# neeharperi/FutureDet

Hardware: AMD Instinct MI355X
Metric: sweeps/sec end-to-end (300k pts, 10-sweep voxel) (higher is better)
Workload: dtype f32

## Files before the change

### futuredet_amd/backbones.py

```python
import numpy as np
import torch
from torch import nn

from . import hip_ops, sparse as spconv
from .nn_utils import build_norm_layer
from .registry import BACKBONES
from .sparse import SparseConv3d, SubMConv3d


def conv3x3(in_planes, out_planes, stride=1, indice_key=None, bias=True):
    return spconv.SubMConv3d(in_planes, out_planes, kernel_size=3, stride=stride, padding=1, bias=bias,
                             indice_key=indice_key)


class SparseBasicBlock(spconv.SparseModule):
    expansion = 1

    def __init__(self, inplanes, planes, stride=1, norm_cfg=None, downsample=None, indice_key=None):
        super().__init__()
        if norm_cfg is None:
            norm_cfg = dict(type="BN1d", eps=1e-3, momentum=0.01)
        bias = norm_cfg is not None
        self.conv1 = conv3x3(inplanes, planes, stride, indice_key=indice_key, bias=bias)
        self.bn1 = build_norm_layer(norm_cfg, planes)[1]
        self.relu = nn.ReLU()
        self.conv2 = conv3x3(planes, planes, indice_key=indice_key, bias=bias)
        self.bn2 = build_norm_layer(norm_cfg, planes)[1]
        self.downsample = downsample
        self.stride = stride

    def forward(self, x):
        identity = x
        out = self.conv1(x)
        out.features = self.relu(self.bn1(out.features))
        out = self.conv2(out)
        out.features = self.bn2(out.features)
        if self.downsample is not None:
            identity = self.downsample(x)
        out.features = self.relu(out.features + identity.features)
        return out

    def forward_fused_bn(self, x, bn_act):
        out = self.conv1(x)
        out.features = bn_act(out.features, self.bn1, self.relu)
        out = self.conv2(out)
        identity = x if self.downsample is None else self.downsample(x)
        out.features = bn_act(out.features, self.bn2, self.relu, identity.features)
        return out


@BACKBONES.register_module
class SpMiddleResNetFHD(nn.Module):
    def __init__(self, num_input_features=128, norm_cfg=None, name="SpMiddleResNetFHD", **kwargs):
        super().__init__()
        self.name = name
        if norm_cfg is None:
            norm_cfg = dict(type="BN1d", eps=1e-3, momentum=0.01)
        S = spconv.SparseSequential
        self.conv_input = S(SubMConv3d(num_input_features, 16, 3, bias=False, indice_key="res0"),
                            build_norm_layer(norm_cfg, 16)[1], nn.ReLU(inplace=True))
        self.conv1 = S(SparseBasicBlock(16, 16, norm_cfg=norm_cfg, indice_key="res0"),
                       SparseBasicBlock(16, 16, norm_cfg=norm_cfg, indice_key="res0"))
        self.conv2 = S(SparseConv3d(16, 32, 3, 2, padding=1, bias=False), build_norm_layer(norm_cfg, 32)[1],
                       nn.ReLU(inplace=True), SparseBasicBlock(32, 32, norm_cfg=norm_cfg, indice_key="res1"),
                       SparseBasicBlock(32, 32, norm_cfg=norm_cfg, indice_key="res1"))
        self.conv3 = S(SparseConv3d(32, 64, 3, 2, padding=1, bias=False), build_norm_layer(norm_cfg, 64)[1],
                       nn.ReLU(inplace=True), SparseBasicBlock(64, 64, norm_cfg=norm_cfg, indice_key="res2"),
                       SparseBasicBlock(64, 64, norm_cfg=norm_cfg, indice_key="res2"))
        self.conv4 = S(SparseConv3d(64, 128, 3, 2, padding=[0, 1, 1], bias=False), build_norm_layer(norm_cfg, 128)[1],
                       nn.ReLU(inplace=True), SparseBasicBlock(128, 128, norm_cfg=norm_cfg, indice_key="res3"),
                       SparseBasicBlock(128, 128, norm_cfg=norm_cfg, indice_key="res3"))
        self.extra_conv = S(SparseConv3d(128, 128, (3, 1, 1), (2, 1, 1), bias=False), build_norm_layer(norm_cfg, 128)[1],
                            nn.ReLU())
        self.compute_dtype = torch.float32
        self.dense_channels_last = True
        self.dense_dtype = None
        self.profile_hook = None
        self.fused_bn = False
        self.train_dtype = torch.float32

    def _bn_act(self, features, bn, relu, residual=None):
        if self.fused_bn and spconv.batch_norm_fusable(features, bn):
            return spconv.batch_norm_act(features, bn, residual=residual, relu=True)
        if features.dtype == torch.bfloat16:
            out = bn(features.float())
            if residual is not None:
                out = out + residual.float()
            return spconv.relu_to_bf16(out)
        out = bn(features)
        if residual is not None:
            out = out + residual
        return relu(out)

    def _run_stage(self, seq, x):
        mods = list(seq._modules.values())
        i = 0
        while i < len(mods):
            m = mods[i]
            if isinstance(m, SparseBasicBlock):
                x = m.forward_fused_bn(x, self._bn_act)
            elif isinstance(m, spconv.SparseModule):
                x = m(x)
            elif x.features.shape[0] != 0:
                if isinstance(m, nn.BatchNorm1d) and i + 1 < len(mods) and isinstance(mods[i + 1], nn.ReLU):
                    x.features = self._bn_act(x.features, m, mods[i + 1])
                    i += 1
                else:
                    x.features = m(x.features)
            i += 1
        return x

    def forward_generic(self, voxel_features, coors, batch_size, input_shape):
        sparse_shape = np.array(input_shape[::-1]) + [1, 0, 0]
        ret = spconv.SparseConvTensor(voxel_features, coors.int(), sparse_shape, batch_size)
        stages = (self.conv_input, self.conv1, self.conv2, self.conv3, self.conv4, self.extra_conv)
        mixed = self.train_dtype == torch.bfloat16 and self.training and torch.is_grad_enabled()
        if mixed:
            ret.features = ret.features.to(torch.bfloat16)
        if mixed or (self.fused_bn and self.training and torch.is_grad_enabled()):
            run = [lambda x, seq=seq: self._run_stage(seq, x) for seq in stages]
        else:
            run = stages
        x = run[0](ret)
        x_conv1 = run[1](x)
        x_conv2 = run[2](x_conv1)
        x_conv3 = run[3](x_conv2)
        x_conv4 = run[4](x_conv3)
        ret = run[5](x_conv4).dense()
        if mixed:
            ret = ret.float()
        N, C, D, H, W = ret.shape
        ret = ret.view(N, C * D, H, W)
        return ret, {"conv1": x_conv1, "conv2": x_conv2, "conv3": x_conv3, "conv4": x_conv4}

    def _stages(self):
        return [(self.conv_input[0], self.conv_input[1], [self.conv1[0], self.conv1[1]], True),
                (self.conv2[0], self.conv2[1], [self.conv2[3], self.conv2[4]], False),
                (self.conv3[0], self.conv3[1], [self.conv3[3], self.conv3[4]], False),
                (self.conv4[0], self.conv4[1], [self.conv4[3], self.conv4[4]], False),
                (self.extra_conv[0], self.extra_conv[1], [], False)]

    def build_indexes(self, mark_fn, batch_size, input_shape, device, voxels=None, static=False, expected=None, row_caps=None):
        D, H, W = [int(v) for v in (np.array(input_shape[::-1]) + [1, 0, 0])]
        if voxels is not None:
            geoms = [self._stages()[lvl][0].geometry() for lvl in range(1, 5)]
            return hip_ops.build_pyramid(voxels[0], voxels[1], voxels[2], batch_size, (D, H, W), geoms, device, static=static,
                                         expected=expected, row_caps=row_caps)
        assert not static, "static indexes are built from the voxelizer's device output (voxels=...)"
        counts = torch.zeros((5,), dtype=torch.int32, device=device)
        idx = [hip_ops.SparseIndex(batch_size, D, H, W, device)]
        mark_fn(idx[0])
        idx[0].scan(counts[0:1])
        for lvl in range(1, 5):
            conv = self._stages()[lvl][0]
            ks, st, pd = conv.geometry()
            nxt = idx[-1].downsample(ks, st, pd)
            nxt.scan(counts[lvl:lvl + 1])
            idx.append(nxt)
        host = counts.cpu()
        for i, ix in enumerate(idx):
            ix.finalize(int(host[i]))
        return idx

    def run_fused(self, idx, feats0, dense_out=None, fork=False):
        dt = self.compute_dtype
        stages = self._stages()
        rb_cache = {}

        from_index = dt == torch.float32

        def rulebook(src, dst, conv):
            ks, st, pd = conv.geometry()
            key = (id(src), id(dst), tuple(ks), tuple(st), tuple(pd))
            if key not in rb_cache:
                layer = (spconv.pad_channels(conv.in_channels), spconv.pad_channels(conv.out_channels)) if from_index else None
                rb_cache[key] = src.rulebook(dst, ks, st, pd, fp32_layer=layer)
            return rb_cache[key]

        def run(conv, bn, x, src, dst, relu, residual=None):
            wpk, bias, cin_p, cout_p = conv.packed_weight(dt, bn)
            assert x.shape[1] == cin_p, (x.shape, cin_p)
            nbr = rulebook(src, dst, conv)
            fn = lambda: hip_ops.spconv_apply(x, wpk, bias, nbr, dst.n, cout_p, residual=residual, relu=relu)
            if self.profile_hook is not None:
                s = 4 if dt == torch.float32 else 2
                K = nbr.shape[0]
                table = lambda: nbr.table() if isinstance(nbr, hip_ops.IndexRulebook) else nbr
                pairs = lambda: int((table()[:, : dst.n] >= 0).sum().item())
                return self.profile_hook("spconv_%dx%d_K%d" % (cin_p, cout_p, K),
                                         dict(s=s, K=K, cin=cin_p, cout=cout_p, n_in=src.n, n_out=dst.n, pairs=pairs), fn)
            return fn()

        def index_plans():
            groups = ([], [])
            for lvl, (conv, bn, blocks, is_subm_in) in enumerate(stages):
                if lvl == 0:
                    continue
                src_l, dst_l = (idx[lvl] if is_subm_in else idx[lvl - 1]), idx[lvl]
                for s_l, cv in [(src_l, conv)] + [(dst_l, b.conv1) for b in blocks[:1]]:
                    nbr = rulebook(s_l, dst_l, cv)
                    if isinstance(nbr, hip_ops.IndexRulebook):
                        ci, co = spconv.pad_channels(cv.in_channels), spconv.pad_channels(cv.out_channels)
                        groups[int(ci == co and bool(hip_ops._lib.load().fd_spconv_wants_balanced_ranges(ci, co, 0)))].append((nbr, ci, co))
            made = []
            for group in groups:
                splits = [(rb,) + tuple(hip_ops.row_split(rb, rb.n_out, ci, co)) for rb, ci, co in group]
                made += [r for _, r, _ in splits if r is not None]
                made += hip_ops.plans_from_index(splits)
            return made

        main, side = None, None
        if fork and feats0.is_cuda:
            main = torch.cuda.current_stream(feats0.device)
            pool = self.__dict__.setdefault("_side_streams", {})
            side = pool.get(main.cuda_stream)
            if side is None:
                side = pool[main.cuda_stream] = torch.cuda.Stream(device=feats0.device)
            side.wait_stream(main)
            with torch.cuda.stream(side):
                made = []
                for lvl, (conv, bn, blocks, is_subm_in) in enumerate(stages):
                    if lvl == 0:
                        continue
                    src_l, dst_l = (idx[lvl] if is_subm_in else idx[lvl - 1]), idx[lvl]
                    nbr = rulebook(src_l, dst_l, conv)
                    if not isinstance(nbr, hip_ops.IndexRulebook):
                        made.append(nbr)
                    for blk in blocks:
                        nbr = rulebook(dst_l, dst_l, blk.conv1)
                        if isinstance(nbr, hip_ops.IndexRulebook):
                            continue
                        made.append(nbr)
                        cp = spconv.pad_channels(blk.conv1.out_channels)
                        if dt == torch.float32 and nbr.shape[0] == 27 and \
                                hip_ops._lib.load().fd_spconv_wants_balanced_ranges(cp, cp, 0):
                            r = hip_ops.ranges_for(nbr, cp, cp)
                            if r[0] is not None:
                                made.append(r[0])
                        if dt == torch.float32 and nbr.shape[0] == 27 and dst_l.n > 0 and \
                                hip_ops._lib.load().fd_spconv_plan_wanted(cp, cp, 0):
                            made.append(hip_ops.plan_for(nbr, dst_l.n, *hip_ops.row_split(nbr, dst_l.n, cp, cp))[0])
                made += index_plans()
                for t in made:
                    t.record_stream(main)
        elif from_index:
            index_plans()
        x = feats0
        levels = {}
        for lvl, (conv, bn, blocks, is_subm_in) in enumerate(stages):
            src = idx[lvl] if is_subm_in else idx[lvl - 1]
            dst = idx[lvl]
            if lvl == 1 and side is not None:
                main.wait_stream(side)
            x = run(conv, bn, x, src, dst, relu=True)
            for blk in blocks:
                y = run(blk.conv1, blk.bn1, x, dst, dst, relu=True)
                x = run(blk.conv2, blk.bn2, y, dst, dst, relu=True, residual=x)
            levels[lvl] = (x, dst)
        bev = hip_ops.densify(x, idx[4], out_dtype=self.dense_dtype or dt, channels_last=self.dense_channels_last, out=dense_out)
        return bev, levels

    def forward_static_train(self, feats0, idx):
        if not self.fused_bn:
            raise ValueError("SpMiddleResNetFHD.forward_static_train needs fused_bn = True: torch's BatchNorm1d cannot take its row count "
                             "from the device (set backbone.fused_bn = True)")
        if not (self.training and torch.is_grad_enabled()):
            raise RuntimeError("SpMiddleResNetFHD.forward_static_train is the training path: call .train() and enable gradients")
        if self.train_dtype not in (torch.float32, torch.bfloat16):
            raise ValueError("SpMiddleResNetFHD: train_dtype must be torch.float32 or torch.bfloat16 (got %s)" % (self.train_dtype,))
        B = idx[0].B
        feats = feats0.to(self.train_dtype)
        rulebooks = {}

        def conv(m, x, src, dst):
            ks, st, pd = m.geometry()
            key = (id(src), id(dst), tuple(ks), tuple(st), tuple(pd))
            if key not in rulebooks:
                rulebooks[key] = src.rulebook(dst, ks, st, pd)
            return m._forward_autograd(x, dst, rulebooks[key])

        def bn_act(x, bn, dst, residual=None):
            if dst.n < 2 or not spconv.batch_norm_fusable(x.features, bn):
                raise hip_ops.FutureDetHipError("forward_static_train: BatchNorm over %s %s rows cannot run on the fused kernels"
                                                % (tuple(x.features.shape), x.features.dtype))
            x.features = spconv.batch_norm_act(x.features, bn, residual=residual, relu=True, n_dev=dst.n_dev if dst.static else None)
            return x

        x = spconv.SparseConvTensor(feats, None, idx[0].spatial_shape, B, _index=idx[0])
        for lvl, (head, bn, blocks, is_subm_in) in enumerate(self._stages()):
            src, dst = (idx[lvl] if is_subm_in else idx[lvl - 1]), idx[lvl]
            x = bn_act(conv(head, x, src, dst), bn, dst)
            for blk in blocks:
                y = bn_act(conv(blk.conv1, x, dst, dst), blk.bn1, dst)
                x = bn_act(conv(blk.conv2, y, dst, dst), blk.bn2, dst, residual=x.features)
        ret = x.dense()
        if ret.dtype != torch.float32:
            ret = ret.float()
        N, C, D, H, W = ret.shape
        return ret.view(N, C * D, H, W)

    def forward(self, voxel_features, coors, batch_size, input_shape):
        if self.training:
            if self.train_dtype not in (torch.float32, torch.bfloat16):
                raise ValueError("SpMiddleResNetFHD: train_dtype must be torch.float32 or torch.bfloat16 (got %s)" % (self.train_dtype,))
            if self.train_dtype == torch.float32 and self.compute_dtype != torch.float32 and torch.is_grad_enabled():
                raise NotImplementedError("SpMiddleResNetFHD: with train_dtype = torch.float32 training runs the fp32 sparse convolution only; "
                                          "compute_dtype = %s selects the inference path (set train_dtype = torch.bfloat16 for mixed-precision "
                                          "training, or compute_dtype = torch.float32)" % self.compute_dtype)
            return self.forward_generic(voxel_features, coors, batch_size, input_shape)
        coors = coors.int().contiguous()
        dev = voxel_features.device
        idx = self.build_indexes(lambda i0: i0.mark(coors), batch_size, input_shape, dev)
        row_of = idx[0].lookup(coors)
        feats0 = hip_ops.rows_permute(voxel_features.float().contiguous(), row_of,
                                      spconv.pad_channels(voxel_features.shape[1]), self.compute_dtype, n_rows=idx[0].n)
        bev, levels = self.run_fused(idx, feats0)
        multi = {}
        for name, lvl, c in (("conv1", 0, 16), ("conv2", 1, 32), ("conv3", 2, 64), ("conv4", 3, 128)):
            f, ix = levels[lvl]
            multi[name] = spconv.SparseConvTensor(f[:, :c], None, ix.spatial_shape, batch_size, _index=ix)
        return bev, multi


@BACKBONES.register_module
class PointPillarsScatter(nn.Module):

    def __init__(self, num_input_features=64, norm_cfg=None, name="PointPillarsScatter", **kwargs):
        super().__init__()
        self.name = "PointPillarsScatter"
        self.nchannels = num_input_features
        self.dense_channels_last = True

    def forward(self, voxel_features, coords, batch_size, input_shape, n_dev=None):
        self.nx = int(input_shape[0])
        self.ny = int(input_shape[1])
        coords = coords.int().contiguous()
        if n_dev is None and torch.is_grad_enabled() and voxel_features.requires_grad:
            return _ScatterFn.apply(voxel_features, coords, batch_size, self.ny, self.nx, self.dense_channels_last)
        return hip_ops.pillar_scatter(voxel_features, coords, n_dev, batch_size, self.ny, self.nx,
                                      channels_last=self.dense_channels_last)


    def forward_static(self, voxel_features, coords, counts, batch_size, input_shape):
        self.nx = int(input_shape[0])
        self.ny = int(input_shape[1])
        return _ScatterSegFn.apply(voxel_features, coords.int().contiguous(), counts, batch_size, self.ny, self.nx, self.dense_channels_last)


class _ScatterSegFn(torch.autograd.Function):

    @staticmethod
    def forward(ctx, feats, coords, counts, batch_size, ny, nx, channels_last):
        B = counts.shape[0]
        cap = feats.shape[0] // B
        ctx.coords, ctx.counts, ctx.cap = coords, counts, cap
        canvas = None
        for b in range(B):
            sl = slice(b * cap, (b + 1) * cap)
            canvas = hip_ops.pillar_scatter(feats[sl], coords[sl], counts[b:b + 1], batch_size, ny, nx, channels_last=channels_last,
                                            out=canvas, zero_first=(b == 0))
        return canvas

    @staticmethod
    def backward(ctx, dcanvas):
        coords, counts, cap = ctx.coords, ctx.counts, ctx.cap
        dcanvas = dcanvas.float()
        d = torch.cat([hip_ops.pillar_scatter_backward(dcanvas, coords[b * cap:(b + 1) * cap], n_dev=counts[b:b + 1])
                       for b in range(counts.shape[0])])
        ctx.coords = ctx.counts = None
        return d, None, None, None, None, None, None


class _ScatterFn(torch.autograd.Function):

    @staticmethod
    def forward(ctx, feats, coords, batch_size, ny, nx, channels_last):
        ctx.coords = coords
        return hip_ops.pillar_scatter(feats, coords, None, batch_size, ny, nx, channels_last=channels_last)

    @staticmethod
    def backward(ctx, dcanvas):
        d = hip_ops.pillar_scatter_backward(dcanvas.float(), ctx.coords)
        ctx.coords = None
        return d, None, None, None, None, None
```

### futuredet_amd/csrc/fd_common.h

```cpp
#pragma once
#include <hip/hip_runtime.h>
#include <stdint.h>
#include <stdio.h>

#include <atomic>

#include "../../include/futuredet_hip.h"

namespace fd {

void set_error(const char *fmt, ...);

struct SpconvCall {
    const void *in;
    int64_t n_in;
    const void *wpacked;
    const float *bias;
    const void *residual;
    int relu;
    const int *nbr;
    int64_t nbr_stride;
    const int *ranges;
    int n_ranges;
    int K, n_out;
    const int *n_out_dev;
    int64_t n_expected;
    int cin, cout, dtype;
    void *out;
    hipStream_t stream;
    const int *plan;
    int64_t plan_stride;
};

constexpr int kSpconvMaxTaps = 27;

struct WeightSection {
    size_t offset, bytes;
};
struct SpconvWeightLayout {
    WeightSection base, c32, pair, win;
    size_t total;
};
inline SpconvWeightLayout spconv_weight_layout(int K, int cin, int cout, int dtype) {
    const size_t elem = dtype == 0 ? 4 : 2, main_bytes = (size_t)K * cin * cout * elem;
    SpconvWeightLayout l{};
    size_t end = 0;
    auto section = [&](bool present, size_t bytes) {
        const WeightSection s{end, present ? bytes : 0};
        end += s.bytes;
        return s;
    };
    l.base = section(true, main_bytes);
    l.c32 = section(dtype == 0 && cin == 32 && cout == 32, main_bytes);
    l.pair = section(dtype == 1 && cin == 16, (size_t)((K + 1) / 2) * 32 * cout * elem);
    l.win = section(dtype == 1 && ((cin == 64 && cout == 64) || (cin == 128 && cout == 128)), main_bytes);
    l.total = end;
    return l;
}
inline SpconvWeightLayout spconv_weight_layout(const SpconvCall &c) { return spconv_weight_layout(c.K, c.cin, c.cout, c.dtype); }

int spconv_f32_res16_dispatch(const SpconvCall &c);
int spconv_f32_c32_dispatch(const SpconvCall &c);
int spconv_f32_compact_dispatch(const SpconvCall &c);
int spconv_bf16_win_dispatch(const SpconvCall &c);
int spconv_bf16_ws_dispatch(const SpconvCall &c);

int wino_pc_launch(const float *x, const void *wp, const float *bias, float *y, int B, int H, int W, int cin, int cout, int relu, int cout_total,
                   int co_off, int wide_items, hipStream_t stream);

__device__ __forceinline__ int device_count(int capacity, const int *count_dev) {
    if (!count_dev) return capacity;
    const int n = *count_dev;
    return n < capacity ? (n > 0 ? n : 0) : capacity;
}

inline int check_launch(const char *what) {
    hipError_t e = hipGetLastError();
    if (e != hipSuccess) {
        set_error("%s: %s", what, hipGetErrorString(e));
        return FD_ELAUNCH;
    }
    return FD_OK;
}

#define FD_REQUIRE(cond, ...)           \
    do {                                \
        if (!(cond)) {                  \
            fd::set_error(__VA_ARGS__); \
            return FD_EINVAL;           \
        }                               \
    } while (0)

inline hipStream_t as_stream(fd_stream_t s) { return reinterpret_cast<hipStream_t>(s); }

int fill_words(void *p, uint32_t value, size_t n_words, hipStream_t stream);
int fill_words3(void *p0, uint32_t v0, size_t n0, void *p1, uint32_t v1, size_t n1, void *p2, uint32_t v2, size_t n2, hipStream_t stream);

constexpr int kMaxDevices = 64;
int current_device();
int device_cu_count();
bool ensure_dynamic_lds(const void *kernel, size_t bytes, std::atomic<uint64_t> &done);
#define FD_TUNE_KNOBS(X)                                                                                                       \
    X(kTuneSpconvRG, "spconv_rg") X(kTuneSpconvV1, "spconv_v1") X(kTuneConvNT, "conv_nt") X(kTuneV2RangesPerCU, "v2_ranges_per_cu") \
    X(kTuneSpconvC32, "spconv_c32") X(kTuneBf16GP, "bf16_gp") X(kTuneBf16RG, "bf16_rg") X(kTuneBf16Depth, "bf16_depth")        \
    X(kTuneBf16NW, "bf16_nw") X(kTuneBf16Win, "bf16_win") X(kTuneF32ResRG, "f32_res_rg") X(kTuneConvStrip, "conv_strip")       \
    X(kTuneF32ResNW, "f32_res_nw") X(kTuneSpconvPlan, "spconv_plan")
#define FD_TUNE_ENUM(key, name) key,
enum TuneKey { FD_TUNE_KNOBS(FD_TUNE_ENUM) kTuneCount };
#undef FD_TUNE_ENUM
int tuning(TuneKey key);

inline size_t align_up(size_t v, size_t a) { return (v + a - 1) / a * a; }

struct IndexGeom {
    int B, D, H, W, Ht, Wt;
    __host__ __device__ int64_t num_cols() const { return (int64_t)B * Ht * Wt * 64; }
};
__host__ __device__ inline IndexGeom make_geom(int B, int D, int H, int W) {
    IndexGeom g;
    g.B = B; g.D = D; g.H = H; g.W = W;
    g.Ht = (H + 7) >> 3; g.Wt = (W + 7) >> 3;
    return g;
}
__host__ __device__ inline int64_t col_of(const IndexGeom &g, int b, int y, int x) {
    return ((((int64_t)b * g.Ht + (y >> 3)) * g.Wt + (x >> 3)) << 6) + ((y & 7) << 3) + (x & 7);
}
__device__ inline void col_to_byx(const IndexGeom &g, int64_t col, int &b, int &y, int &x) {
    int in = (int)(col & 63);
    int64_t t = col >> 6;
    int tx = (int)(t % g.Wt);
    t /= g.Wt;
    int ty = (int)(t % g.Ht);
    b = (int)(t / g.Ht);
    y = ty * 8 + (in >> 3);
    x = tx * 8 + (in & 7);
}

__device__ inline unsigned xcd_swizzle(unsigned bid, unsigned nblocks) {
    const unsigned nx = 8;
    unsigned per = nblocks / nx, rem = nblocks % nx;
    unsigned xcd = bid % nx, loc = bid / nx;
    unsigned start = xcd * per + (xcd < rem ? xcd : rem);
    return start + loc;
}

}
```

### futuredet_amd/csrc/fd_spconv.hip

```cpp
#include "fd_spconv_pack.h"

namespace {

typedef float f32x4 __attribute__((ext_vector_type(4)));
typedef short s16x4 __attribute__((ext_vector_type(4)));
typedef __bf16 bf16x8 __attribute__((ext_vector_type(8)));

__device__ inline unsigned short f2bf(float v) {
    unsigned u = __float_as_uint(v);
    u += 0x7fffu + ((u >> 16) & 1u);
    return (unsigned short)(u >> 16);
}
__device__ inline float bf2f(unsigned short h) { return __uint_as_float(((unsigned)h) << 16); }


template <int CIN, int COUT, int RG>
__global__ void __launch_bounds__(256) spconv_f32(const float *__restrict__ in, const float4 *__restrict__ wp,
                                                  const float *__restrict__ bias, const float *__restrict__ residual, int relu,
                                                  const int *__restrict__ nbr, int64_t nbr_stride, int K, int n_out,
                                                  const int *__restrict__ n_out_dev, float *__restrict__ out) {
    constexpr int ROWS_B = 64 * RG;
    constexpr int NB = COUT / 16, NC = CIN / 16;
    __shared__ int s_nbr[fd::kSpconvMaxTaps * ROWS_B];
    const int tile = blockIdx.x;
    const int row0 = tile * ROWS_B;
    n_out = fd::device_count(n_out, n_out_dev);
    if (row0 >= n_out) return;
    for (int t = threadIdx.x; t < K * ROWS_B; t += 256) {
        int k = t / ROWS_B, r = t - k * ROWS_B;
        int64_t o = (int64_t)row0 + r;
        s_nbr[t] = (o < n_out) ? nbr[(int64_t)k * nbr_stride + o] : -1;
    }
    __syncthreads();
    const int lane = threadIdx.x & 63, wave = __builtin_amdgcn_readfirstlane(threadIdx.x >> 6);
    const int lrow = lane & 15, lq = lane >> 4;
    const int wrow = wave * 16 * RG;
    if (row0 + wrow >= n_out) return;

    f32x4 acc[RG][NB];
#pragma unroll
    for (int g = 0; g < RG; ++g)
#pragma unroll
        for (int nb = 0; nb < NB; ++nb) acc[g][nb] = (f32x4){0.f, 0.f, 0.f, 0.f};

    for (int k = 0; k < K; ++k) {
        int idx[RG];
        bool any[RG];
        bool any_all = false;
#pragma unroll
        for (int g = 0; g < RG; ++g) {
            idx[g] = s_nbr[k * ROWS_B + wrow + g * 16 + lrow];
            any[g] = __ballot(idx[g] >= 0) != 0ull;
            any_all = any_all || any[g];
        }
        if (!any_all) continue;
        const float4 *wk = wp + (int64_t)k * NC * NB * 64 + lane;
#pragma unroll
        for (int c = 0; c < NC; ++c) {
            float4 a[RG];
#pragma unroll
            for (int g = 0; g < RG; ++g) {
                a[g] = make_float4(0.f, 0.f, 0.f, 0.f);
                if (idx[g] >= 0) a[g] = *reinterpret_cast<const float4 *>(in + (int64_t)idx[g] * CIN + c * 16 + lq * 4);
            }
#pragma unroll
            for (int nb = 0; nb < NB; ++nb) {
                const float4 b = wk[(c * NB + nb) * 64];
#pragma unroll
                for (int g = 0; g < RG; ++g) {
                    if (any[g]) {
                        acc[g][nb] = __builtin_amdgcn_mfma_f32_16x16x4f32(a[g].x, b.x, acc[g][nb], 0, 0, 0);
                        acc[g][nb] = __builtin_amdgcn_mfma_f32_16x16x4f32(a[g].y, b.y, acc[g][nb], 0, 0, 0);
                        acc[g][nb] = __builtin_amdgcn_mfma_f32_16x16x4f32(a[g].z, b.z, acc[g][nb], 0, 0, 0);
                        acc[g][nb] = __builtin_amdgcn_mfma_f32_16x16x4f32(a[g].w, b.w, acc[g][nb], 0, 0, 0);
                    }
                }
            }
        }
    }
#pragma unroll
    for (int g = 0; g < RG; ++g) {
#pragma unroll
        for (int nb = 0; nb < NB; ++nb) {
            const int col = nb * 16 + lrow;
            const float bv = bias ? bias[col] : 0.0f;
#pragma unroll
            for (int r = 0; r < 4; ++r) {
                const int row = row0 + wrow + g * 16 + lq * 4 + r;
                if (row < n_out) {
                    float v = acc[g][nb][r] + bv;
                    if (residual) v += residual[(int64_t)row * COUT + col];
                    if (relu) v = fmaxf(v, 0.0f);
                    out[(int64_t)row * COUT + col] = v;
                }
            }
        }
    }
}

template <int CIN, int COUT, int RG>
__global__ void __launch_bounds__(256) spconv_bf16(const unsigned short *__restrict__ in, const void *__restrict__ wp_,
                                                   const float *__restrict__ bias, const unsigned short *__restrict__ residual,
                                                   int relu, const int *__restrict__ nbr, int64_t nbr_stride, int K, int n_out,
                                                   const int *__restrict__ n_out_dev, unsigned short *__restrict__ out) {
    constexpr int ROWS_B = 64 * RG;
    constexpr int NB = COUT / 16;
    constexpr bool WIDE = CIN >= 32;
    constexpr int NC = WIDE ? CIN / 32 : 1;
    __shared__ int s_nbr[fd::kSpconvMaxTaps * ROWS_B];
    const int tile = blockIdx.x;
    const int row0 = tile * ROWS_B;
    n_out = fd::device_count(n_out, n_out_dev);
    if (row0 >= n_out) return;
    for (int t = threadIdx.x; t < K * ROWS_B; t += 256) {
        int k = t / ROWS_B, r = t - k * ROWS_B;
        int64_t o = (int64_t)row0 + r;
        s_nbr[t] = (o < n_out) ? nbr[(int64_t)k * nbr_stride + o] : -1;
    }
    __syncthreads();
    const int lane = threadIdx.x & 63, wave = __builtin_amdgcn_readfirstlane(threadIdx.x >> 6);
    const int lrow = lane & 15, lq = lane >> 4;
    const int wrow = wave * 16 * RG;
    if (row0 + wrow >= n_out) return;

    f32x4 acc[RG][NB];
#pragma unroll
    for (int g = 0; g < RG; ++g)
#pragma unroll
        for (int nb = 0; nb < NB; ++nb) acc[g][nb] = (f32x4){0.f, 0.f, 0.f, 0.f};

    for (int k = 0; k < K; ++k) {
        int idx[RG];
        bool any[RG];
        bool any_all = false;
#pragma unroll
        for (int g = 0; g < RG; ++g) {
            idx[g] = s_nbr[k * ROWS_B + wrow + g * 16 + lrow];
            any[g] = __ballot(idx[g] >= 0) != 0ull;
            any_all = any_all || any[g];
        }
        if (!any_all) continue;
        if constexpr (WIDE) {
            const bf16x8 *wk = reinterpret_cast<const bf16x8 *>(wp_) + (int64_t)k * NC * NB * 64 + lane;
#pragma unroll
            for (int c = 0; c < NC; ++c) {
                bf16x8 a[RG];
#pragma unroll
                for (int g = 0; g < RG; ++g) {
                    uint4 raw = make_uint4(0u, 0u, 0u, 0u);
                    if (idx[g] >= 0) raw = *reinterpret_cast<const uint4 *>(in + (int64_t)idx[g] * CIN + c * 32 + lq * 8);
                    a[g] = __builtin_bit_cast(bf16x8, raw);
                }
#pragma unroll
                for (int nb = 0; nb < NB; ++nb) {
                    const bf16x8 b = wk[(c * NB + nb) * 64];
#pragma unroll
                    for (int g = 0; g < RG; ++g)
                        if (any[g]) acc[g][nb] = __builtin_amdgcn_mfma_f32_16x16x32_bf16(a[g], b, acc[g][nb], 0, 0, 0);
                }
            }
        } else {
            const s16x4 *wk = reinterpret_cast<const s16x4 *>(wp_) + (int64_t)k * NB * 64 + lane;
            s16x4 a[RG];
#pragma unroll
            for (int g = 0; g < RG; ++g) {
                uint2 raw = make_uint2(0u, 0u);
                if (idx[g] >= 0) raw = *reinterpret_cast<const uint2 *>(in + (int64_t)idx[g] * CIN + lq * 4);
                a[g] = __builtin_bit_cast(s16x4, raw);
            }
#pragma unroll
            for (int nb = 0; nb < NB; ++nb) {
                const s16x4 b = wk[nb * 64];
#pragma unroll
                for (int g = 0; g < RG; ++g)
                    if (any[g]) acc[g][nb] = __builtin_amdgcn_mfma_f32_16x16x16bf16_1k(a[g], b, acc[g][nb], 0, 0, 0);
            }
        }
    }
#pragma unroll
    for (int g = 0; g < RG; ++g) {
#pragma unroll
        for (int nb = 0; nb < NB; ++nb) {
            const int col = nb * 16 + lrow;
            const float bv = bias ? bias[col] : 0.0f;
#pragma unroll
            for (int r = 0; r < 4; ++r) {
                const int row = row0 + wrow + g * 16 + lq * 4 + r;
                if (row < n_out) {
                    float v = acc[g][nb][r] + bv;
                    if (residual) v += bf2f(residual[(int64_t)row * COUT + col]);
                    if (relu) v = fmaxf(v, 0.0f);
                    out[(int64_t)row * COUT + col] = f2bf(v);
                }
            }
        }
    }
}

template <int CIN, int COUT, int RG>
void launch(const fd::SpconvCall &a) {
    const int rows_b = 64 * RG;
    dim3 grid((unsigned)((a.n_out + rows_b - 1) / rows_b));
    const void *wp = (const char *)a.wpacked + fd::spconv_weight_layout(a).base.offset;
    if (a.dtype == 0)
        hipLaunchKernelGGL((spconv_f32<CIN, COUT, RG>), grid, dim3(256), 0, a.stream, (const float *)a.in, (const float4 *)wp, a.bias,
                           (const float *)a.residual, a.relu, a.nbr, a.nbr_stride, a.K, a.n_out, a.n_out_dev, (float *)a.out);
    else
        hipLaunchKernelGGL((spconv_bf16<CIN, COUT, RG>), grid, dim3(256), 0, a.stream, (const unsigned short *)a.in, wp, a.bias,
                           (const unsigned short *)a.residual, a.relu, a.nbr, a.nbr_stride, a.K, a.n_out, a.n_out_dev, (unsigned short *)a.out);
}

template <int CIN, int COUT>
void launch_rg(const fd::SpconvCall &a, int rg) {
    if (rg >= 4) launch<CIN, COUT, 4>(a);
    else if (rg == 2) launch<CIN, COUT, 2>(a);
    else launch<CIN, COUT, 1>(a);
}

int pick_rg(int64_t n_out, int cin, int cout) {
    const int forced = fd::tuning(fd::kTuneSpconvRG);
    if (forced > 0) return forced;
    const int64_t waves2 = (n_out + 31) / 32;
    int rg = (cin * cout >= 128 * 128) ? 1 : 2;
    if (rg == 2 && waves2 < 256 * 4 * 2) rg = 1;
    return rg;
}

}

extern "C" size_t fd_spconv_packed_weight_bytes(int K, int cin, int cout, int dtype) {
    if (K <= 0 || cin <= 0 || cout <= 0) return 0;
    return fd::spconv_weight_layout(K, cin, cout, dtype).total;
}

extern "C" int fd_spconv_pack_weight(const float *w, int K, int cin, int cout, int dtype, void *dst) {
    if (const int rc = fd::spconv_pack_check("fd_spconv_pack_weight", w, dst, K, cin, cout, dtype, 0)) return rc;
    fd::spconv_pack_weight_host(w, K, cin, cout, dtype, dst);
    return FD_OK;
}

namespace {
int spconv_apply(const void *in_feats, int64_t n_in, const void *wpacked, const float *bias, const void *residual, int relu, const int32_t *nbr,
                 int64_t nbr_stride, const int32_t *ranges, int n_ranges, int K, int64_t n_out, const int32_t *n_out_dev, int64_t n_expected, int cin,
                 int cout, int dtype, void *out_feats, fd_stream_t stream, const int32_t *plan, int64_t plan_stride) {
    FD_REQUIRE(K >= 1 && K <= fd::kSpconvMaxTaps, "fd_spconv_apply: K must be in [1,27]");
    FD_REQUIRE(dtype == 0 || dtype == 1, "fd_spconv_apply: dtype must be 0 (f32) or 1 (bf16)");
    FD_REQUIRE(n_out >= 0 && n_out <= nbr_stride && n_out < (1ll << 31), "fd_spconv_apply: n_out out of range");
    FD_REQUIRE(n_ranges >= 0 && (ranges == nullptr || n_ranges >= 1), "fd_spconv_apply: ranges needs n_ranges >= 1");
    if (n_expected <= 0 || n_expected > n_out) n_expected = n_out;
    if (n_out == 0) return FD_OK;
    FD_REQUIRE(in_feats && wpacked && (nbr || plan) && out_feats, "fd_spconv_apply: null argument");
    const fd::SpconvCall c{in_feats, n_in, wpacked, bias, residual, relu, nbr, nbr_stride, ranges, n_ranges, K, (int)n_out, n_out_dev, n_expected,
                           cin, cout, dtype, out_feats, fd::as_stream(stream), plan, plan_stride};
    if (dtype == 0 && !fd::tuning(fd::kTuneSpconvV1) && cin == 16 && fd::tuning(fd::kTuneF32ResRG) >= 0) {
        if (fd::spconv_f32_res16_dispatch(c)) return fd::check_launch("fd_spconv_apply(f32 resident)");
    }
    if (dtype == 0 && !fd::tuning(fd::kTuneSpconvV1) && fd::tuning(fd::kTuneSpconvC32) >= 0) {
        if (fd::spconv_f32_c32_dispatch(c)) return fd::check_launch("fd_spconv_apply(c32)");
    }
    if (dtype == 0 && !fd::tuning(fd::kTuneSpconvV1)) {
        if (fd::spconv_f32_compact_dispatch(c)) return fd::check_launch("fd_spconv_apply(compact)");
    }
    if (dtype == 1 && fd::tuning(fd::kTuneBf16GP) >= 0) {
        const bool subm_like = K == 27 && n_in == n_out;
        if (fd::tuning(fd::kTuneBf16Win) >= 0 && subm_like && fd::spconv_bf16_win_dispatch(c)) return fd::check_launch("fd_spconv_apply(bf16 window)");
        if (fd::spconv_bf16_ws_dispatch(c)) return fd::check_launch("fd_spconv_apply(bf16 ws)");
    }
    if (!nbr) {
        fd::set_error("fd_spconv_apply_plan: no kernel runs %d -> %d on %lld input rows from a chunk plan alone: pass the rulebook table", cin, cout,
                      (long long)n_in);
        return FD_EINVAL;
    }
    const int rg = pick_rg(n_expected, cin, cout);
    const int key = cin * 1000 + cout;
    switch (key) {
        case 16016: launch_rg<16, 16>(c, rg); break;
        case 16032: launch_rg<16, 32>(c, rg); break;
        case 32032: launch_rg<32, 32>(c, rg); break;
        case 32064: launch_rg<32, 64>(c, rg); break;
        case 64064: launch_rg<64, 64>(c, rg); break;
        case 64128: launch_rg<64, 128>(c, rg); break;
        case 128128: launch_rg<128, 128>(c, rg); break;
        default:
            fd::set_error("fd_spconv_apply: unsupported channels %d -> %d", cin, cout);
            return FD_EINVAL;
    }
    return fd::check_launch("fd_spconv_apply");
}
}

extern "C" int fd_spconv_apply(const void *in_feats, int64_t n_in, const void *wpacked, const float *bias, const void *residual, int relu,
                               const int32_t *nbr, int64_t nbr_stride, const int32_t *ranges, int n_ranges, int K, int64_t n_out,
                               const int32_t *n_out_dev, int64_t n_expected, int cin, int cout, int dtype, void *out_feats, fd_stream_t stream) {
    return spconv_apply(in_feats, n_in, wpacked, bias, residual, relu, nbr, nbr_stride, ranges, n_ranges, K, n_out, n_out_dev, n_expected, cin, cout,
                        dtype, out_feats, stream, nullptr, 0);
}

extern "C" int fd_spconv_apply_plan(const void *in_feats, int64_t n_in, const void *wpacked, const float *bias, const void *residual, int relu,
                                    const int32_t *nbr, int64_t nbr_stride, const int32_t *ranges, int n_ranges, int K, int64_t n_out,
                                    const int32_t *n_out_dev, int64_t n_expected, int cin, int cout, int dtype, void *out_feats,
                                    const int32_t *plan, int64_t plan_stride, fd_stream_t stream) {
    FD_REQUIRE(nbr || plan, "fd_spconv_apply_plan: nbr == NULL needs a chunk plan (fd_spconv_plan_from_index)");
    if (plan) {
        FD_REQUIRE(K == fd::kSpconvMaxTaps && dtype == 0, "fd_spconv_apply_plan: a chunk plan belongs to an fp32 layer of K = 27 taps");
        FD_REQUIRE(nbr == nullptr || cin == cout, "fd_spconv_apply_plan: next to a rulebook table a chunk plan belongs to an fp32 SubM layer (K = 27)");
        FD_REQUIRE(plan_stride >= fd_spconv_plan_stride(n_out), "fd_spconv_apply_plan: plan_stride below fd_spconv_plan_stride(n_out)");
        if (!nbr) {
            FD_REQUIRE(fd_spconv_index_plan_wanted(cin, cout, dtype),
                       "fd_spconv_apply_plan: nbr == NULL, but no kernel runs this layer shape from a chunk plan alone (fd_spconv_index_plan_wanted)");
        } else if (!fd_spconv_plan_wanted(cin, cout, dtype)) {
            plan = nullptr;
        }
    }
    return spconv_apply(in_feats, n_in, wpacked, bias, residual, relu, nbr, nbr_stride, ranges, n_ranges, K, n_out, n_out_dev, n_expected, cin, cout,
                        dtype, out_feats, stream, plan, plan_stride);
}
```

### futuredet_amd/csrc/fd_spconv_c32.hip

```cpp
#include "fd_spconv_chunk.h"

namespace {

namespace sk = fd::skeleton;
typedef float f32x16 __attribute__((ext_vector_type(16)));
typedef unsigned u32x4 __attribute__((ext_vector_type(4)));
constexpr int TM = 128, COUT = 32, TS = 4, WR = 1;
constexpr sk::Layout L = sk::layout(TM, COUT, TS, 32);
static_assert(((sk::kMaxTaps + TS - 1) / TS) * (TM / WR / 32) <= L.item_slot, "item list slot");

template <int CIN, int DEPTH, bool PLAN>
__global__ void __launch_bounds__(256) spconv_f32_c32(const float *__restrict__ in, const float4 *__restrict__ wp, const float *__restrict__ bias,
                                                      const float *__restrict__ residual, int relu, const int *__restrict__ nbr, int64_t nbr_stride,
                                                      int K, int n_out, const int *__restrict__ n_out_dev, float *__restrict__ out, unsigned in_bytes,
                                                      const int *__restrict__ ranges, int rows_per_range) {
    constexpr int NCH = CIN / 8;
    constexpr int kPad = sk::pad_entry(TM);
    extern __shared__ __attribute__((aligned(16))) unsigned char smem[];
    int *s_list = reinterpret_cast<int *>(smem + L.list);
    unsigned short *s_items = reinterpret_cast<unsigned short *>(smem + L.items);
    unsigned char *s_cnt = smem + L.cnt;
    int *s_pad = reinterpret_cast<int *>(smem + L.pad);
    float *s_acc = reinterpret_cast<float *>(smem + L.acc);

    const int tid = threadIdx.x, lane = tid & 63, wave = __builtin_amdgcn_readfirstlane(tid >> 6);
    int r_begin, r_end, n_chunks, chunk_rows;
    sk::resolve_range(n_out, n_out_dev, ranges, rows_per_range, r_begin, r_end);
    if (r_begin >= r_end) return;
    sk::cut_chunks<TM>(r_begin, r_end, n_chunks, chunk_rows);
    int pre[sk::kSliceRegs<TM>];
    const int k_fetch = PLAN ? sk::kPlanRows : K;
    sk::fetch_slice<TM>(pre, nbr, nbr_stride, k_fetch, r_begin);

    const int ln = lane & 31, lh = lane >> 5;
    const int ts = wave, wr = 0;
    unsigned char *acc_bytes = reinterpret_cast<unsigned char *>(s_acc + ts * L.acc_copy);
    const __amdgpu_buffer_rsrc_t rsrc = __builtin_amdgcn_make_buffer_rsrc(const_cast<float *>(in), 0, (int)in_bytes, 0x00020000);
    unsigned short *items = s_items + wave * L.item_slot;

    for (int chunk = 0; chunk < n_chunks; ++chunk) {
        int row0, n_rows;
        if (!sk::chunk_span(r_begin, r_end, chunk_rows, chunk, row0, n_rows)) break;
        if constexpr (PLAN) {
            sk::stage_plan_chunk<TM, COUT, TS, 32>(pre, s_list, s_cnt, s_pad, s_acc, bias, residual, row0, n_rows);
        } else {
            sk::stage_chunk<TM, COUT, TS, 32>(pre, s_list, s_pad, s_acc, bias, residual, K, row0, n_rows);
            __syncthreads();
            sk::compact_taps<TM, WR>(s_list, s_cnt, K);
        }
        __syncthreads();
        if (chunk + 1 < n_chunks) sk::fetch_slice<TM>(pre, nbr, nbr_stride, k_fetch, row0 + chunk_rows);
        const int n_items = sk::build_items<TS, 32>(s_cnt, items, K, ts, wr);

        int k_r[DEPTH], row_r[DEPTH];
        u32x4 a_r[DEPTH][NCH];
        auto stage_a0 = [&](int it) -> int { return sk::stage_a0(items, n_items, it); };
        auto stage_a1 = [&](int it, int code_v, int &kk, int &e) { sk::stage_a1<TM, WR, 32>(s_list, s_pad, n_items, wr, ln, it, code_v, kk, e); };
        auto gather_offset = [&](int e) -> unsigned { return sk::entry_row_bytes<CIN>(e) + (unsigned)(lh * 16); };
        auto gather_step = [&](unsigned voff, int c) { return __builtin_amdgcn_raw_buffer_load_b128(rsrc, voff + c * 32, 0, 0); };
        float4 b[NCH];
        auto load_b = [&](int k) {
            const float4 *wk = wp + (int64_t)k * NCH * 64 + lane;
#pragma unroll
            for (int c = 0; c < NCH; ++c) b[c] = wk[c * 64];
        };
        int k_s, e_s, code_s;
#pragma unroll
        for (int d = 0; d < DEPTH - 1; ++d) {
            stage_a1(d, stage_a0(d), k_s, e_s);
            const unsigned vo = gather_offset(e_s);
#pragma unroll
            for (int c = 0; c < NCH; ++c) a_r[d][c] = gather_step(vo, c);
            k_r[d] = k_s;
            row_r[d] = e_s;
        }
        k_r[DEPTH - 1] = -1;
        row_r[DEPTH - 1] = kPad;
        stage_a1(DEPTH - 1, stage_a0(DEPTH - 1), k_s, e_s);
        code_s = stage_a0(DEPTH);
        if (n_items > 0) load_b(k_r[0]);

        for (int i0 = 0; i0 < n_items; i0 += DEPTH) {
#pragma unroll
            for (int d = 0; d < DEPTH; ++d) {
                const unsigned arow = sk::entry_local_row(row_r[d]);
                unsigned aoff[4];
#pragma unroll
                for (int q = 0; q < 4; ++q) aoff[q] = sk::acc_slot_bytes<COUT>(arow, (unsigned)(2 * q + lh));
                f32x16 acc;
#pragma unroll
                for (int q = 0; q < 4; ++q) {
                    const float4 v = *reinterpret_cast<const float4 *>(acc_bytes + aoff[q]);
                    acc[4 * q + 0] = v.x; acc[4 * q + 1] = v.y; acc[4 * q + 2] = v.z; acc[4 * q + 3] = v.w;
                }
                const int dn = (d + DEPTH - 1) % DEPTH;
                {
                    const int it = i0 + d + DEPTH - 1;
                    const unsigned vo = gather_offset(e_s);
                    k_r[dn] = k_s;
                    row_r[dn] = e_s;
#pragma unroll
                    for (int c = 0; c < NCH; ++c) a_r[dn][c] = gather_step(vo, c);
                    stage_a1(it + 1, code_s, k_s, e_s);
                    code_s = stage_a0(it + 2);
                }
                const int knext = k_r[(d + 1) % DEPTH];
                const bool reload = knext >= 0 && knext != k_r[d];
                __builtin_amdgcn_sched_barrier(0);
#pragma unroll
                for (int c = 0; c < NCH; ++c) {
                    const float4 av = __builtin_bit_cast(float4, a_r[d][c]);
                    acc = __builtin_amdgcn_mfma_f32_32x32x2f32(b[c].x, av.x, acc, 0, 0, 0);
                    acc = __builtin_amdgcn_mfma_f32_32x32x2f32(b[c].y, av.y, acc, 0, 0, 0);
                    acc = __builtin_amdgcn_mfma_f32_32x32x2f32(b[c].z, av.z, acc, 0, 0, 0);
                    acc = __builtin_amdgcn_mfma_f32_32x32x2f32(b[c].w, av.w, acc, 0, 0, 0);
                    if (reload) b[c] = (wp + (int64_t)knext * NCH * 64 + lane)[c * 64];
                }
#pragma unroll
                for (int q = 0; q < 4; ++q)
                    *reinterpret_cast<float4 *>(acc_bytes + aoff[q]) = make_float4(acc[4 * q + 0], acc[4 * q + 1], acc[4 * q + 2], acc[4 * q + 3]);
                __builtin_amdgcn_sched_barrier(0);
            }
        }
        __syncthreads();
        sk::epilogue<TM, COUT, TS>(s_acc, bias, residual, relu, out, row0, n_rows);
        __syncthreads();
    }
}

template <int CIN, int DEPTH, bool PLAN>
int launch_c32(const fd::SpconvCall &c) {
    const unsigned in_bytes = (unsigned)(c.n_in * CIN * 4);
    int n_ranges = c.n_ranges, rows_per = 0;
    if (!c.ranges) sk::equal_rows_split(c.n_out, TM, c.n_out_dev != nullptr, n_ranges, rows_per);
    static std::atomic<uint64_t> lds_set{0};
    if (!fd::ensure_dynamic_lds(reinterpret_cast<const void *>(spconv_f32_c32<CIN, DEPTH, PLAN>), (size_t)L.bytes, lds_set)) return 0;
    const void *wp = (const char *)c.wpacked + fd::spconv_weight_layout(c).c32.offset;
    hipLaunchKernelGGL((spconv_f32_c32<CIN, DEPTH, PLAN>), dim3((unsigned)n_ranges), dim3(256), (size_t)L.bytes, c.stream, (const float *)c.in, (const float4 *)wp,
                       c.bias, (const float *)c.residual, c.relu, PLAN ? c.plan : c.nbr, PLAN ? c.plan_stride : c.nbr_stride, c.K, c.n_out, c.n_out_dev, (float *)c.out, in_bytes, c.ranges, rows_per);
    return 1;
}

}

namespace fd {
int spconv_f32_c32_dispatch(const SpconvCall &c) {
    if (c.cout != 32 || c.cin != 32) return 0;
    if (!sk::entries_fit(c.n_in, c.cin)) return 0;
    return c.plan ? launch_c32<32, 3, true>(c) : launch_c32<32, 3, false>(c);
}
}
```

### futuredet_amd/csrc/fd_spconv_chunk.h

```cpp
#pragma once
#include "fd_common.h"

namespace fd {
namespace skeleton {

constexpr int kMaxTaps = 27;

constexpr int pad_entry(int tm) { return (int)(0xffffff00u | (unsigned)tm); }
__device__ __forceinline__ int pack_entry(int in_row, int local_row) { return (in_row << 8) | local_row; }
__device__ __forceinline__ unsigned entry_local_row(int e) { return (unsigned)e & 255u; }
template <int CIN>
__device__ __forceinline__ unsigned entry_row_bytes(int e) {
    static_assert(CIN == 16 || CIN == 32 || CIN == 64 || CIN == 128, "shift per CIN");
    const unsigned hi = (unsigned)e & 0xffffff00u;
    return CIN >= 64 ? hi << (CIN == 128 ? 1 : 0) : hi >> (CIN == 32 ? 1 : 2);
}
inline bool entries_fit(int64_t n_in_bound, int cin) { return n_in_bound < (1ll << 23) && n_in_bound * cin * 4 < (1ll << 31); }

struct Layout {
    int list;
    int items;
    int item_slot;
    int cnt;
    int pad;
    int acc;
    int acc_copy;
    int bytes;
};
constexpr int acc_copy_floats(int tm, int cout) { return (tm + 1) * cout; }
constexpr Layout layout(int tm, int cout, int ts, int item) {
    Layout l{};
    l.list = 0;
    l.items = l.list + (int)sizeof(int) * kMaxTaps * tm;
    l.item_slot = item == 16 ? kMaxTaps * (tm / 16) : 32;
    l.cnt = l.items + (int)sizeof(unsigned short) * 4 * l.item_slot;
    l.pad = l.cnt + 112;
    l.acc = l.pad + (int)sizeof(int) * item;
    l.acc_copy = acc_copy_floats(tm, cout);
    l.bytes = l.acc + (int)sizeof(float) * ts * l.acc_copy;
    return l;
}

template <int COUT>
__device__ __forceinline__ unsigned acc_swizzle(unsigned row) {
    static_assert(COUT == 16 || COUT == 32 || COUT == 64 || COUT == 128, "whole bank rows");
    constexpr int kSwzShift = COUT >= 64 ? 0 : COUT == 32 ? 1 : 2;
    constexpr unsigned kSwzMask = COUT >= 64 ? 15u : COUT == 32 ? 7u : 3u;
    return (row >> kSwzShift) & kSwzMask;
}
template <int COUT>
__device__ __forceinline__ int acc_slot(int row, int col) {
    return row * (COUT / 4) + (col ^ (int)acc_swizzle<COUT>((unsigned)row));
}
template <int COUT>
__device__ __forceinline__ unsigned acc_slot_bytes(unsigned row, unsigned col) {
    return row * (COUT * 4) + ((col ^ acc_swizzle<COUT>(row)) << 4);
}

__device__ __forceinline__ void resolve_range_of(int block, int n_blocks, int n_out, const int *n_out_dev, const int *ranges, int rows_per_range,
                                                 int &r_begin, int &r_end) {
    if (n_out_dev) n_out = fd::device_count(n_out, n_out_dev);
    if (ranges) {
        r_begin = ranges[block];
        r_end = ranges[block + 1];
    } else {
        if (n_out_dev) rows_per_range = (((n_out + n_blocks - 1) / n_blocks) + 15) & ~15;
        const int64_t b = (int64_t)block * rows_per_range;
        r_begin = (int)(b < n_out ? b : n_out);
        r_end = (int)(b + rows_per_range < n_out ? b + rows_per_range : n_out);
    }
    if (r_end > n_out) r_end = n_out;
}
__device__ __forceinline__ void resolve_range(int n_out, const int *n_out_dev, const int *ranges, int rows_per_range,
                                              int &r_begin, int &r_end) {
    resolve_range_of((int)blockIdx.x, (int)gridDim.x, n_out, n_out_dev, ranges, rows_per_range, r_begin, r_end);
}
template <int TM>
__device__ __forceinline__ void cut_chunks(int r_begin, int r_end, int &n_chunks, int &chunk_rows) {
    n_chunks = (r_end - r_begin + TM - 1) / TM;
    chunk_rows = (((r_end - r_begin + n_chunks - 1) / n_chunks) + 15) & ~15;
}
__device__ __forceinline__ bool chunk_span(int r_begin, int r_end, int chunk_rows, int chunk, int &row0, int &n_rows) {
    row0 = r_begin + chunk * chunk_rows;
    n_rows = (r_end - row0) < chunk_rows ? (r_end - row0) : chunk_rows;
    return n_rows > 0;
}
inline void equal_rows_split(int n_out, int tm, bool device_count, int &n_ranges, int &rows_per) {
    if (n_ranges <= 0) n_ranges = (n_out + tm - 1) / tm;
    rows_per = (((n_out + n_ranges - 1) / n_ranges) + 15) & ~15;
    if (!device_count) n_ranges = (n_out + rows_per - 1) / rows_per;
}

template <int TM>
constexpr int kSliceRegs = (kMaxTaps * TM + 255) / 256;

template <int TM>
__device__ __forceinline__ void fetch_slice(int (&pre)[kSliceRegs<TM>], const int *nbr, int64_t nbr_stride, int K, int row0) {
    const int tid = threadIdx.x;
#pragma unroll
    for (int i = 0; i < kSliceRegs<TM>; ++i) {
        const int t = tid + i * 256;
        int k = t / TM;
        const int r = t - k * TM;
        k = k < K ? k : K - 1;
        int64_t o = (int64_t)row0 + r;
        o = o < nbr_stride ? o : nbr_stride - 1;
        pre[i] = nbr[(int64_t)k * nbr_stride + o];
    }
}

template <int COUT>
constexpr bool kInitAcc = COUT <= 64;

template <int TM, int COUT, int TS>
__device__ __forceinline__ void init_acc(float *s_acc, const float *bias, const float *residual, int row0, int n_rows) {
    const int tid = threadIdx.x;
    if constexpr (kInitAcc<COUT>) {
        constexpr int C4i = COUT / 4, NINIT = TM * C4i / 256;
        static_assert(TM * C4i % 256 == 0, "whole passes");
        float4 iv[NINIT];
#pragma unroll
        for (int i = 0; i < NINIT; ++i) {
            const int t = tid + i * 256, c4 = t % C4i;
            iv[i] = bias ? reinterpret_cast<const float4 *>(bias)[c4] : make_float4(0.f, 0.f, 0.f, 0.f);
        }
        if (residual) {
            float4 rv[NINIT];
#pragma unroll
            for (int i = 0; i < NINIT; ++i) {
                const int t = tid + i * 256, r = t / C4i, c4 = t - r * C4i;
                const int rr = r < n_rows ? r : n_rows - 1;
                rv[i] = reinterpret_cast<const float4 *>(residual + (int64_t)(row0 + rr) * COUT)[c4];
            }
#pragma unroll
            for (int i = 0; i < NINIT; ++i) { iv[i].x += rv[i].x; iv[i].y += rv[i].y; iv[i].z += rv[i].z; iv[i].w += rv[i].w; }
        }
#pragma unroll
        for (int i = 0; i < NINIT; ++i) {
            const int t = tid + i * 256, r = t / C4i, c4 = t - r * C4i;
            reinterpret_cast<float4 *>(s_acc)[acc_slot<COUT>(r, c4)] = r < n_rows ? iv[i] : make_float4(0.f, 0.f, 0.f, 0.f);
        }
        for (int t = TM * C4i + tid; t < TS * acc_copy_floats(TM, COUT) / 4; t += 256) reinterpret_cast<float4 *>(s_acc)[t] = make_float4(0.f, 0.f, 0.f, 0.f);
    } else {
        for (int t = tid; t < TS * acc_copy_floats(TM, COUT) / 4; t += 256) reinterpret_cast<float4 *>(s_acc)[t] = make_float4(0.f, 0.f, 0.f, 0.f);
    }
}

template <int TM, int COUT, int TS, int ITEM>
__device__ __forceinline__ void stage_chunk(const int (&pre)[kSliceRegs<TM>], int *s_list, int *s_pad, float *s_acc, const float *bias,
                                            const float *residual, int K, int row0, int n_rows) {
    const int tid = threadIdx.x;
    static_assert(256 % TM == 0, "a thread stages the same local row in every pass");
    const bool in_chunk = tid % TM < n_rows;
#pragma unroll
    for (int i = 0; i < kSliceRegs<TM>; ++i) {
        const int t = tid + i * 256;
        if (t < K * TM) s_list[t] = in_chunk ? pre[i] : -1;
    }
    init_acc<TM, COUT, TS>(s_acc, bias, residual, row0, n_rows);
    if (tid < ITEM) s_pad[tid] = pad_entry(TM);
}

constexpr int kPlanRows = kMaxTaps + 1;
constexpr int kPlanTM = 128;
constexpr int kPlanCountWords = (kMaxTaps + 3) / 4;
inline int64_t plan_stride_for(int64_t n_out) { return (n_out + 8 + 63) / 64 * 64; }

template <int TM, int COUT, int TS, int ITEM>
__device__ __forceinline__ void stage_plan_chunk(const int (&pre)[kSliceRegs<TM>], int *s_list, unsigned char *s_cnt, int *s_pad, float *s_acc,
                                                 const float *bias, const float *residual, int row0, int n_rows) {
    const int tid = threadIdx.x;
    static_assert(TM == kPlanTM && 256 % TM == 0, "the plan is cut for 128-row chunks");
    static_assert(kSliceRegs<TM> * 256 >= kMaxTaps * TM + kPlanCountWords, "the count words ride in the slice's last register");
    const bool in_chunk = tid % TM < n_rows;
#pragma unroll
    for (int i = 0; i < kSliceRegs<TM>; ++i) {
        const int t = tid + i * 256;
        if (t < kMaxTaps * TM) {
            s_list[t] = in_chunk ? pre[i] : pad_entry(TM);
        } else if (t < kMaxTaps * TM + kPlanCountWords) {
            const int k0 = (t - kMaxTaps * TM) * 4;
#pragma unroll
            for (int q = 0; q < 4; ++q)
                if (k0 + q < kMaxTaps) s_cnt[(k0 + q) * 4] = (unsigned char)((unsigned)pre[i] >> (8 * q));
        }
    }
    init_acc<TM, COUT, TS>(s_acc, bias, residual, row0, n_rows);
    if (tid < ITEM) s_pad[tid] = pad_entry(TM);
}

template <int TM, int WR>
__device__ __forceinline__ void compact_taps(int *s_list, unsigned char *s_cnt, int K) {
    const int lane = threadIdx.x & 63, wave = __builtin_amdgcn_readfirstlane(threadIdx.x >> 6);
    constexpr int RW = TM / WR, NH = (RW + 63) / 64;
    for (int k = wave; k < K; k += 4) {
#pragma unroll
        for (int wr = 0; wr < WR; ++wr) {
            const int base = k * TM + wr * RW;
            int count = 0;
            int v[NH];
#pragma unroll
            for (int h = 0; h < NH; ++h) {
                const int r = h * 64 + lane;
                v[h] = (r < RW) ? s_list[base + r] : -1;
            }
#pragma unroll
            for (int h = 0; h < NH; ++h) {
                const int r = h * 64 + lane;
                if (r < RW) s_list[base + r] = pad_entry(TM);
            }
#pragma unroll
            for (int h = 0; h < NH; ++h) {
                const int r = h * 64 + lane;
                const unsigned long long m = __ballot(v[h] >= 0);
                const int pos = count + __popcll(m & ((1ull << lane) - 1ull));
                if (v[h] >= 0) s_list[base + pos] = pack_entry(v[h], wr * RW + r);
                count += __popcll(m);
            }
            if (lane == 0) s_cnt[k * 4 + wr] = (unsigned char)count;
        }
    }
}

template <int TS, int ITEM>
__device__ __forceinline__ int build_items(const unsigned char *s_cnt, unsigned short *items, int K, int ts, int wr) {
    const int lane = threadIdx.x & 63;
    const int ng = (lane < K && (lane % TS) == ts) ? ((int)s_cnt[lane * 4 + wr] + ITEM - 1) / ITEM : 0;
    int inc = ng;
#pragma unroll
    for (int off = 1; off < 64; off <<= 1) {
        const int u = __shfl_up(inc, off);
        if (lane >= off) inc += u;
    }
    const int n_items = __builtin_amdgcn_readfirstlane(__shfl(inc, 63));
    for (int g = 0; g < ng; ++g) items[inc - ng + g] = (unsigned short)((lane << 3) | g);
    __builtin_amdgcn_fence(__ATOMIC_RELEASE, "workgroup");
    __builtin_amdgcn_wave_barrier();
    __builtin_amdgcn_fence(__ATOMIC_ACQUIRE, "workgroup");
    return n_items;
}

__device__ __forceinline__ int stage_a0(const unsigned short *items, int n_items, int it) { return (int)items[it < n_items ? it : 0]; }
template <int TM, int WR, int ITEM>
__device__ __forceinline__ void stage_a1(const int *s_list, const int *s_pad, int n_items, int wr, int lp, int it, int code_v, int &kk, int &e) {
    const bool v = it < n_items;
    const int code = __builtin_amdgcn_readfirstlane(code_v);
    const int ks = v ? (code >> 3) : 0;
    kk = v ? ks : -1;
    const int *lst = v ? s_list + ks * TM + wr * (TM / WR) + (code & 7) * ITEM : s_pad;
    e = lst[lp];
}

template <int TM, int COUT, int TS>
__device__ __forceinline__ void epilogue(float *s_acc, const float *bias, const float *residual, int relu,
                                         float *out, int row0, int n_rows) {
    const int tid = threadIdx.x;
    constexpr int C4 = COUT / 4;
    for (int t = tid; t < n_rows * C4; t += 256) {
        const int r = t / C4, c4 = t - r * C4;
        const int row = row0 + r;
        const int slot = acc_slot<COUT>(r, c4);
        float4 v = reinterpret_cast<const float4 *>(s_acc)[slot];
#pragma unroll
        for (int q = 1; q < TS; ++q) {
            const float4 v2 = reinterpret_cast<const float4 *>(s_acc + q * acc_copy_floats(TM, COUT))[slot];
            v.x += v2.x; v.y += v2.y; v.z += v2.z; v.w += v2.w;
        }
        if constexpr (!kInitAcc<COUT>) {
            if (bias) {
                const float4 bv = reinterpret_cast<const float4 *>(bias)[c4];
                v.x += bv.x; v.y += bv.y; v.z += bv.z; v.w += bv.w;
            }
            if (residual) {
                const float4 rv = reinterpret_cast<const float4 *>(residual + (int64_t)row * COUT)[c4];
                v.x += rv.x; v.y += rv.y; v.z += rv.z; v.w += rv.w;
            }
        }
        if (relu) { v.x = fmaxf(v.x, 0.f); v.y = fmaxf(v.y, 0.f); v.z = fmaxf(v.z, 0.f); v.w = fmaxf(v.w, 0.f); }
        reinterpret_cast<float4 *>(out + (int64_t)row * COUT)[c4] = v;
    }
}

}
}
```

### futuredet_amd/csrc/fd_spconv_v2.hip

```cpp
#include "fd_spconv_chunk.h"

namespace {

namespace sk = fd::skeleton;
typedef float f32x4 __attribute__((ext_vector_type(4)));
typedef unsigned u32x4 __attribute__((ext_vector_type(4)));
typedef int i32x4 __attribute__((ext_vector_type(4)));

#ifdef FD_V2_TRACE
__device__ unsigned long long *g_trace;
#define FD_T(i)                                                                                  \
    do {                                                                                         \
        if (threadIdx.x == 0 && g_trace) g_trace[(size_t)blockIdx.x * 16 + (i)] = __builtin_readcyclecounter(); \
    } while (0)
#define FD_TV(i, v)                                                                    \
    do {                                                                               \
        if (threadIdx.x == 0 && g_trace) g_trace[(size_t)blockIdx.x * 16 + (i)] = (v); \
    } while (0)
#else
#define FD_T(i)
#define FD_TV(i, v)
#endif


constexpr int tap_splits(int cout) { return (cout == 32 || cout == 64) ? 2 : 1; }

template <int CIN, int COUT, int TM, int DEPTH, bool PLAN>
__global__ void __launch_bounds__(256) spconv_f32_compact(const float *__restrict__ in, const float4 *__restrict__ wp,
                                                          const float *__restrict__ bias, const float *__restrict__ residual, int relu,
                                                          const int *__restrict__ nbr, int64_t nbr_stride, int K, int n_out,
                                                          const int *__restrict__ n_out_dev, float *__restrict__ out, unsigned in_bytes,
                                                          const int *__restrict__ ranges, int rows_per_range) {
    constexpr int NB = COUT / 16, NC = CIN / 16;
    constexpr int WC = NB == 8 ? 4 : (NB >= 2 ? 2 : 1);
    constexpr int NBW = NB / WC;
    constexpr int TS = tap_splits(COUT);
    constexpr int WR = 4 / (WC * TS);
    constexpr int NACC = NBW;
    static_assert((TM == 128 || TM == 64) && TM / WR >= 16, "local row uses 8 bits (0..TM, TM = scratch row)");
    static_assert(!PLAN || (TM == sk::kPlanTM && WR == 1), "the chunk plan holds the lists of 128-row chunks with one row set");
    constexpr int kPad = sk::pad_entry(TM);
    constexpr sk::Layout L = sk::layout(TM, COUT, TS, 16);
    extern __shared__ __attribute__((aligned(16))) unsigned char smem[];
    int *s_list = reinterpret_cast<int *>(smem + L.list);
    unsigned short *s_items = reinterpret_cast<unsigned short *>(smem + L.items);
    unsigned char *s_cnt = smem + L.cnt;
    int *s_pad = reinterpret_cast<int *>(smem + L.pad);
    float *s_acc = reinterpret_cast<float *>(smem + L.acc);

    const int tid = threadIdx.x, lane = tid & 63, wave = __builtin_amdgcn_readfirstlane(tid >> 6);
    int r_begin, r_end, n_chunks, chunk_rows;
    sk::resolve_range(n_out, n_out_dev, ranges, rows_per_range, r_begin, r_end);
    if (r_begin >= r_end) return;
    FD_T(0);
    sk::cut_chunks<TM>(r_begin, r_end, n_chunks, chunk_rows);
    int pre[sk::kSliceRegs<TM>];
    const int k_fetch = PLAN ? sk::kPlanRows : K;
    sk::fetch_slice<TM>(pre, nbr, nbr_stride, k_fetch, r_begin);

    const int lrow = lane & 15, lq = lane >> 4;
    const int wc = wave % WC, wr = TS == 1 ? wave / WC : 0, ts = TS == 1 ? 0 : wave / WC;
    const int cb = wc * NBW * 16;
    unsigned char *acc_bytes = reinterpret_cast<unsigned char *>(s_acc + ts * L.acc_copy);
    const unsigned slot0 = (unsigned)(cb >> 2) + (unsigned)lq;
    const __amdgpu_buffer_rsrc_t rsrc = __builtin_amdgcn_make_buffer_rsrc(const_cast<float *>(in), 0, (int)in_bytes, 0x00020000);
    unsigned short *items = s_items + wave * L.item_slot;

    for (int chunk = 0; chunk < n_chunks; ++chunk) {
    int row0, n_rows;
    if (!sk::chunk_span(r_begin, r_end, chunk_rows, chunk, row0, n_rows)) break;
    if constexpr (PLAN) {
        sk::stage_plan_chunk<TM, COUT, TS, 16>(pre, s_list, s_cnt, s_pad, s_acc, bias, residual, row0, n_rows);
    } else {
        sk::stage_chunk<TM, COUT, TS, 16>(pre, s_list, s_pad, s_acc, bias, residual, K, row0, n_rows);
        __syncthreads();
        if (chunk == 0) FD_T(1);
        sk::compact_taps<TM, WR>(s_list, s_cnt, K);
    }
    __syncthreads();
    if (chunk == 0) FD_T(2);
    if (chunk + 1 < n_chunks) sk::fetch_slice<TM>(pre, nbr, nbr_stride, k_fetch, row0 + chunk_rows);
    const int n_items = sk::build_items<TS, 16>(s_cnt, items, K, ts, wr);

    int k_r[DEPTH];
    int row_r[DEPTH];
    u32x4 a_r[DEPTH][NC];
    auto stage_a0 = [&](int it) -> int { return sk::stage_a0(items, n_items, it); };
    auto stage_a1 = [&](int it, int code_v, int &kk, int &e) { sk::stage_a1<TM, WR, 16>(s_list, s_pad, n_items, wr, lrow, it, code_v, kk, e); };
    auto gather_offset = [&](int e) -> unsigned { return sk::entry_row_bytes<CIN>(e) + (unsigned)(lq * 16); };
    auto gather_chunk = [&](unsigned voff, int c) { return __builtin_amdgcn_raw_buffer_load_b128(rsrc, voff + c * 64, 0, 0); };
    auto load_b = [&](int k, float4(&dst)[NC][NBW]) {
        const float4 *wk = wp + ((int64_t)k * NC * NB + wc * NBW) * 64 + lane;
#pragma unroll
        for (int c = 0; c < NC; ++c)
#pragma unroll
            for (int nw = 0; nw < NBW; ++nw) dst[c][nw] = wk[(c * NB + nw) * 64];
    };
    float4 b[NC][NBW];
    static_assert(DEPTH >= 2, "the slot freed by the previous item is refilled during the current item's MFMAs");
    int k_s, e_s, code_s;
#pragma unroll
    for (int d = 0; d < DEPTH - 1; ++d) {
        stage_a1(d, stage_a0(d), k_s, e_s);
        const unsigned vo = gather_offset(e_s);
#pragma unroll
        for (int c = 0; c < NC; ++c) a_r[d][c] = gather_chunk(vo, c);
        k_r[d] = k_s;
        row_r[d] = e_s;
    }
    k_r[DEPTH - 1] = -1;
    row_r[DEPTH - 1] = kPad;
    stage_a1(DEPTH - 1, stage_a0(DEPTH - 1), k_s, e_s);
    code_s = stage_a0(DEPTH);
    if (n_items > 0) load_b(k_r[0], b);
    if (chunk == 0) { FD_T(3); FD_TV(8, (unsigned long long)n_items); FD_TV(9, (unsigned long long)n_chunks); FD_TV(10, (unsigned long long)n_rows);
                      FD_TV(11, (unsigned long long)__builtin_amdgcn_s_getreg(4 | (31 << 11))); FD_TV(12, (unsigned long long)__builtin_amdgcn_s_getreg(20 | (31 << 11))); }
    FD_TV(13, (unsigned long long)(g_trace ? g_trace[(size_t)blockIdx.x * 16 + 13] : 0) + (unsigned long long)n_items);

    auto mfma_chunk = [&](const u32x4 &a4, const float4(&bc)[NBW], f32x4(&acc)[NACC]) {
        const float4 av = __builtin_bit_cast(float4, a4);
#pragma unroll
        for (int nw = 0; nw < NBW; ++nw) acc[nw] = __builtin_amdgcn_mfma_f32_16x16x4f32(bc[nw].x, av.x, acc[nw], 0, 0, 0);
#pragma unroll
        for (int nw = 0; nw < NBW; ++nw) acc[nw] = __builtin_amdgcn_mfma_f32_16x16x4f32(bc[nw].y, av.y, acc[nw], 0, 0, 0);
#pragma unroll
        for (int nw = 0; nw < NBW; ++nw) acc[nw] = __builtin_amdgcn_mfma_f32_16x16x4f32(bc[nw].z, av.z, acc[nw], 0, 0, 0);
#pragma unroll
        for (int nw = 0; nw < NBW; ++nw) acc[nw] = __builtin_amdgcn_mfma_f32_16x16x4f32(bc[nw].w, av.w, acc[nw], 0, 0, 0);
    };

    for (int i0 = 0; i0 < n_items; i0 += DEPTH) {
#pragma unroll
        for (int d = 0; d < DEPTH; ++d) {
            const unsigned arow = sk::entry_local_row(row_r[d]);
            unsigned aoff[NBW];
#pragma unroll
            for (int nw = 0; nw < NBW; ++nw) aoff[nw] = sk::acc_slot_bytes<COUT>(arow, slot0 + 4u * nw);
            f32x4 acc[NACC];
#pragma unroll
            for (int nw = 0; nw < NBW; ++nw) acc[nw] = *reinterpret_cast<const f32x4 *>(acc_bytes + aoff[nw]);
            const int dn = (d + DEPTH - 1) % DEPTH;
            unsigned vo;
            {
                const int it = i0 + d + DEPTH - 1;
                vo = gather_offset(e_s);
                k_r[dn] = k_s;
                row_r[dn] = e_s;
                stage_a1(it + 1, code_s, k_s, e_s);
                code_s = stage_a0(it + 2);
            }
            const int knext = k_r[(d + 1) % DEPTH];
            const bool reload = knext >= 0 && knext != k_r[d];
            constexpr bool kSpread = NC * 4 * NBW >= 16;
            if constexpr (!kSpread) {
#pragma unroll
                for (int c = 0; c < NC; ++c) a_r[dn][c] = gather_chunk(vo, c);
            }
            __builtin_amdgcn_sched_barrier(0);
            if (reload) {
                const float4 *wk = wp + ((int64_t)knext * NC * NB + wc * NBW) * 64 + lane;
#pragma unroll
                for (int c = 0; c < NC; ++c) {
                    mfma_chunk(a_r[d][c], b[c], acc);
                    if constexpr (kSpread) a_r[dn][c] = gather_chunk(vo, c);
#pragma unroll
                    for (int nw = 0; nw < NBW; ++nw) b[c][nw] = wk[(c * NB + nw) * 64];
                    __builtin_amdgcn_sched_group_barrier(0x008, 4 * NBW, 0);
                    __builtin_amdgcn_sched_group_barrier(0x020, (kSpread ? 1 : 0) + NBW, 0);
                }
            } else {
#pragma unroll
                for (int c = 0; c < NC; ++c) {
                    mfma_chunk(a_r[d][c], b[c], acc);
                    if constexpr (kSpread) {
                        a_r[dn][c] = gather_chunk(vo, c);
                        __builtin_amdgcn_sched_group_barrier(0x008, 4 * NBW, 0);
                        __builtin_amdgcn_sched_group_barrier(0x020, 1, 0);
                    }
                }
            }
#pragma unroll
            for (int nw = 0; nw < NBW; ++nw) *reinterpret_cast<f32x4 *>(acc_bytes + aoff[nw]) = acc[nw];
            __builtin_amdgcn_sched_barrier(0);
        }
    }
    if (chunk == 0) FD_T(4);
    __syncthreads();
    if (chunk == 0) FD_T(5);
    sk::epilogue<TM, COUT, TS>(s_acc, bias, residual, relu, out, row0, n_rows);
    __syncthreads();
    if (chunk == 0) FD_T(6);
    }
    FD_T(7);
}

inline size_t lds_request(int cin, int cout, int tm) {
    const size_t lds = (size_t)sk::layout(tm, cout, tap_splits(cout), 16).bytes;
    return (cin == 64 && cout == 64 && tm == 128 && lds < 56 * 1024) ? (size_t)56 * 1024 : lds;
}

template <int CIN, int COUT, int TM, int DEPTH, bool PLAN = false>
int launch_compact(const fd::SpconvCall &c) {
    if constexpr (!PLAN && ((CIN == COUT && COUT >= 32) || COUT == 2 * CIN) && TM == sk::kPlanTM) {
        if (c.plan) return launch_compact<CIN, COUT, TM, DEPTH, true>(c);
    }
    const size_t lds_req = lds_request(CIN, COUT, TM);
    static std::atomic<uint64_t> lds_set{0};
    auto kern = spconv_f32_compact<CIN, COUT, TM, DEPTH, PLAN>;
    if (!fd::ensure_dynamic_lds(reinterpret_cast<const void *>(kern), lds_req, lds_set)) return 0;
    const unsigned in_bytes = (unsigned)(c.n_in * CIN * 4);
    int n_ranges = c.n_ranges, rows_per = 0;
    if (!c.ranges) sk::equal_rows_split(c.n_out, TM, c.n_out_dev != nullptr, n_ranges, rows_per);
    const void *wp = (const char *)c.wpacked + fd::spconv_weight_layout(c).base.offset;
    hipLaunchKernelGGL(kern, dim3((unsigned)n_ranges), dim3(256), lds_req, c.stream, (const float *)c.in, (const float4 *)wp, c.bias,
                       (const float *)c.residual, c.relu, PLAN ? c.plan : c.nbr, PLAN ? c.plan_stride : c.nbr_stride, c.K, c.n_out, c.n_out_dev,
                       (float *)c.out, in_bytes, c.ranges, rows_per);
    return 1;
}

constexpr int kWorkRows = 8;
constexpr int kRowCost = 24;
__global__ void __launch_bounds__(256) block_work_kernel(const int *__restrict__ nbr, int64_t nbr_stride, int K, int n_out,
                                                         const int *__restrict__ n_out_dev, unsigned row_cost, unsigned *__restrict__ work) {
    n_out = fd::device_count(n_out, n_out_dev);
    const int n_blocks = (n_out + kWorkRows - 1) / kWorkRows;
    const int lane = threadIdx.x & 63;
    const int64_t wave = (int64_t)blockIdx.x * 4 + (threadIdx.x >> 6);
    const int64_t o = wave * 64 + lane;
    if (wave * 8 >= n_blocks) return;
    unsigned w = row_cost;
    for (int k = 0; k < K; ++k) {
        const bool v = o < n_out && nbr[(int64_t)k * nbr_stride + o] >= 0;
        const unsigned long long m = __ballot(v);
        const unsigned byte = (unsigned)(m >> (8 * (lane & 7))) & 0xffu;
        w += (unsigned)__popc(byte) * 2u + (byte ? 1u : 0u);
    }
    if (lane < 8 && wave * 8 + lane < n_blocks) work[wave * 8 + lane] = w;
}

__global__ void __launch_bounds__(1024) range_split_kernel(const unsigned *__restrict__ work, int n_out, const int *__restrict__ n_out_dev,
                                                           int n_ranges, int *__restrict__ ranges) {
    n_out = fd::device_count(n_out, n_out_dev);
    const int n_blocks = (n_out + kWorkRows - 1) / kWorkRows;
    __shared__ unsigned long long s_seg[16];
    __shared__ unsigned long long s_total;
    const int tid = threadIdx.x, lane = tid & 63, wave = tid >> 6;
    if (n_blocks == 0) {
        for (int j = tid; j <= n_ranges; j += 1024) ranges[j] = 0;
        return;
    }
    const int seg = (((n_blocks + 15) / 16) + 63) & ~63;
    const int b_lo = wave * seg, b_hi = min(n_blocks, b_lo + seg);
    constexpr int kU = 16;
    unsigned long long sum = 0;
    for (int c0 = b_lo; c0 < b_hi; c0 += 64 * kU) {
        unsigned wv[kU];
#pragma unroll
        for (int u = 0; u < kU; ++u) {
            const int bb = c0 + 64 * u + lane;
            wv[u] = work[bb < b_hi ? bb : b_hi - 1];
        }
#pragma unroll
        for (int u = 0; u < kU; ++u) sum += (c0 + 64 * u + lane < b_hi) ? wv[u] : 0u;
    }
#pragma unroll
    for (int o = 32; o > 0; o >>= 1) sum += __shfl_xor(sum, o);
    if (lane == 0) s_seg[wave] = sum;
    __syncthreads();
    if (tid == 0) {
        unsigned long long run = 0;
        for (int w = 0; w < 16; ++w) { const unsigned long long v = s_seg[w]; s_seg[w] = run; run += v; }
        s_total = run;
    }
    __syncthreads();
    const unsigned long long total = s_total > 0 ? s_total : 1ull;
    const double scale = (double)n_ranges / (2.0 * (double)total);
    auto range_of = [&](unsigned long long ex, unsigned w) -> int {
        const int r = (int)((double)(2ull * ex + w) * scale);
        return r < n_ranges ? r : n_ranges - 1;
    };
    unsigned long long run = s_seg[wave];
    int prev = -1;
    if (b_lo > 0 && b_lo < n_blocks) {
        const unsigned wp = work[b_lo - 1];
        prev = range_of(run - wp, wp);
    }
    constexpr int kB = 8;
    __shared__ unsigned s_buf[16][64 * (kB + 1)];
    unsigned *buf = s_buf[wave];
    for (int c0 = b_lo; c0 < b_hi; c0 += 64 * kB) {
#pragma unroll
        for (int u = 0; u < kB; ++u) {
            const int e = 64 * u + lane, bb = c0 + e;
            buf[(e / kB) * (kB + 1) + e % kB] = bb < b_hi ? work[bb] : 0u;
        }
        __builtin_amdgcn_fence(__ATOMIC_RELEASE, "workgroup");
        __builtin_amdgcn_wave_barrier();
        __builtin_amdgcn_fence(__ATOMIC_ACQUIRE, "workgroup");
        unsigned w[kB];
        unsigned tot = 0;
#pragma unroll
        for (int i = 0; i < kB; ++i) {
            w[i] = buf[lane * (kB + 1) + i];
            tot += w[i];
        }
        unsigned inc = tot;
#pragma unroll
        for (int o = 1; o < 64; o <<= 1) {
            const unsigned u = __shfl_up(inc, o);
            if (lane >= o) inc += u;
        }
        unsigned long long ex = run + (inc - tot);
        const int first = c0 + lane * kB;
        int last_rg = prev;
        {
            unsigned long long e2 = ex;
#pragma unroll
            for (int i = 0; i < kB; ++i) {
                if (first + i < b_hi) last_rg = range_of(e2, w[i]);
                e2 += w[i];
            }
        }
        int before = __shfl_up(last_rg, 1);
        if (lane == 0) before = prev;
        if (first >= b_hi) last_rg = before;
#pragma unroll
        for (int i = 0; i < kB; ++i) {
            const int bb = first + i;
            if (bb < b_hi) {
                const int rg = range_of(ex, w[i]);
                for (int j = before + 1; j <= rg; ++j) ranges[j] = bb * kWorkRows;
                before = rg;
                if (bb == n_blocks - 1)
                    for (int j = rg + 1; j <= n_ranges; ++j) ranges[j] = n_out;
            }
            ex += w[i];
        }
        const int n_valid = min(64 * kB, b_hi - c0);
        prev = __shfl(last_rg, (n_valid - 1) / kB);
        run += __shfl(inc, 63);
        __builtin_amdgcn_wave_barrier();
    }
}

constexpr int kPlanSplit = 4;
__global__ void __launch_bounds__(256) chunk_plan_kernel(const int *__restrict__ nbr, int64_t nbr_stride, int n_out, const int *__restrict__ n_out_dev,
                                                         const int *__restrict__ ranges, int rows_per_range, int *__restrict__ plan, int64_t plan_stride) {
    constexpr int TM = sk::kPlanTM, K = sk::kMaxTaps, NT = (K + 3) / 4, NH = TM / 64;
    constexpr int kPad = sk::pad_entry(TM);
    const int lane = threadIdx.x & 63, wave = __builtin_amdgcn_readfirstlane(threadIdx.x >> 6);
    int r_begin, r_end, n_chunks, chunk_rows;
    sk::resolve_range(n_out, n_out_dev, ranges, rows_per_range, r_begin, r_end);
    if (r_begin < 0 || r_begin >= r_end) return;
    sk::cut_chunks<TM>(r_begin, r_end, n_chunks, chunk_rows);
    for (int chunk = blockIdx.y; chunk < n_chunks; chunk += kPlanSplit) {
        int row0, n_rows;
        if (!sk::chunk_span(r_begin, r_end, chunk_rows, chunk, row0, n_rows)) break;
        int v[NT][NH];
#pragma unroll
        for (int j = 0; j < NT; ++j) {
            const int k = wave + 4 * j < K ? wave + 4 * j : K - 1;
#pragma unroll
            for (int h = 0; h < NH; ++h) {
                const int r = h * 64 + lane;
                const int rr = r < n_rows ? r : n_rows - 1;
                v[j][h] = nbr[(int64_t)k * nbr_stride + row0 + rr];
                if (r >= n_rows) v[j][h] = -1;
            }
        }
#pragma unroll
        for (int j = 0; j < NT; ++j) {
            const int k = wave + 4 * j;
            if (k >= K) break;
            int *list = plan + (int64_t)k * plan_stride + row0;
            int count = 0;
#pragma unroll
            for (int h = 0; h < NH; ++h) {
                const unsigned long long m = __ballot(v[j][h] >= 0);
                const int pos = count + __popcll(m & ((1ull << lane) - 1ull));
                if (v[j][h] >= 0) list[pos] = sk::pack_entry(v[j][h], h * 64 + lane);
                count += __popcll(m);
            }
#pragma unroll
            for (int h = 0; h < NH; ++h) {
                const int p = h * 64 + lane;
                if (p >= count && p < n_rows) list[p] = kPad;
            }
            if (lane == 0) reinterpret_cast<unsigned char *>(plan + (int64_t)K * plan_stride + row0)[k] = (unsigned char)count;
        }
    }
}

struct PlanSource {
    const unsigned long long *words;
    const int *prefix;
    const int *out_coords;
    const int *n_out_dev;
    const int *ranges;
    int *plan;
    int64_t plan_stride;
    fd::IndexGeom gi;
    int n_out, n_ranges, rows_per_range;
    int s[3], p[3];
};
constexpr int kMaxPlanSources = 8;
struct PlanSources {
    PlanSource t[kMaxPlanSources];
};

__device__ __forceinline__ int tap_row(unsigned long long w, int base, int iz, int D) {
    return (iz >= 0 && iz < D && ((w >> iz) & 1ull)) ? base + __popcll(w & ((1ull << iz) - 1ull)) : -1;
}

__global__ void __launch_bounds__(256) index_plan_kernel(const PlanSources S) {
    constexpr int TM = sk::kPlanTM, K = sk::kMaxTaps, NH = TM / 64, NCOL = 3;
    constexpr int kPad = sk::pad_entry(TM);
    const PlanSource &t = S.t[blockIdx.z];
    if ((int)blockIdx.x >= t.n_ranges) return;
    const int lane = threadIdx.x & 63, wave = __builtin_amdgcn_readfirstlane(threadIdx.x >> 6);
    int r_begin, r_end, n_chunks, chunk_rows;
    sk::resolve_range_of((int)blockIdx.x, t.n_ranges, t.n_out, t.n_out_dev, t.ranges, t.rows_per_range, r_begin, r_end);
    if (r_begin < 0 || r_begin >= r_end) return;
    sk::cut_chunks<TM>(r_begin, r_end, n_chunks, chunk_rows);
    const fd::IndexGeom gi = t.gi;
    for (int chunk = blockIdx.y; chunk < n_chunks; chunk += kPlanSplit) {
        int row0, n_rows;
        if (!sk::chunk_span(r_begin, r_end, chunk_rows, chunk, row0, n_rows)) break;
        int4 c[NH];
#pragma unroll
        for (int h = 0; h < NH; ++h) {
            const int r = h * 64 + lane;
            c[h] = reinterpret_cast<const int4 *>(t.out_coords)[row0 + (r < n_rows ? r : n_rows - 1)];
        }
        unsigned long long w[NCOL][NH];
        int base[NCOL][NH];
#pragma unroll
        for (int j = 0; j < NCOL; ++j) {
            const int c9 = wave + 4 * j, ky = c9 / 3, kx = c9 - 3 * ky;
#pragma unroll
            for (int h = 0; h < NH; ++h) {
                const int iy = c[h].z * t.s[1] - t.p[1] + ky;
                const int ix = c[h].w * t.s[2] - t.p[2] + kx;
                const bool ok = c9 < 9 && h * 64 + lane < n_rows && iy >= 0 && iy < gi.H && ix >= 0 && ix < gi.W;
                const int64_t col = ok ? fd::col_of(gi, c[h].x, iy, ix) : 0;
                const unsigned long long wv = t.words[col];
                base[j][h] = t.prefix[col];
                w[j][h] = ok ? wv : 0ull;
            }
        }
#pragma unroll
        for (int j = 0; j < NCOL; ++j) {
            const int c9 = wave + 4 * j;
            if (c9 >= 9) break;
            for (int kz = 0; kz < 3; ++kz) {
                const int k = kz * 9 + c9;
                int *list = t.plan + (int64_t)k * t.plan_stride + row0;
                int v[NH];
#pragma unroll
                for (int h = 0; h < NH; ++h) v[h] = tap_row(w[j][h], base[j][h], c[h].y * t.s[0] - t.p[0] + kz, gi.D);
                int count = 0;
#pragma unroll
                for (int h = 0; h < NH; ++h) {
                    const unsigned long long m = __ballot(v[h] >= 0);
                    const int pos = count + __popcll(m & ((1ull << lane) - 1ull));
                    if (v[h] >= 0) list[pos] = sk::pack_entry(v[h], h * 64 + lane);
                    count += __popcll(m);
                }
#pragma unroll
                for (int h = 0; h < NH; ++h) {
                    const int p = h * 64 + lane;
                    if (p >= count && p < n_rows) list[p] = kPad;
                }
                if (lane == 0) reinterpret_cast<unsigned char *>(t.plan + (int64_t)K * t.plan_stride + row0)[k] = (unsigned char)count;
            }
        }
    }
}

__global__ void __launch_bounds__(256) index_work_kernel(const unsigned long long *__restrict__ words, fd::IndexGeom g, const int *__restrict__ coords,
                                                         int n_out, const int *__restrict__ n_out_dev, unsigned row_cost, unsigned *__restrict__ work) {
    n_out = fd::device_count(n_out, n_out_dev);
    const int n_blocks = (n_out + kWorkRows - 1) / kWorkRows;
    const int lane = threadIdx.x & 63;
    const int64_t wave = (int64_t)blockIdx.x * 4 + (threadIdx.x >> 6);
    const int64_t o = wave * 64 + lane;
    if (wave * 8 >= n_blocks) return;
    const bool in = o < n_out;
    const int4 c = reinterpret_cast<const int4 *>(coords)[in ? o : n_out - 1];
    unsigned long long wv[9];
#pragma unroll
    for (int c9 = 0; c9 < 9; ++c9) {
        const int iy = c.z - 1 + c9 / 3, ix = c.w - 1 + c9 % 3;
        const bool ok = in && iy >= 0 && iy < g.H && ix >= 0 && ix < g.W;
        const unsigned long long x = words[ok ? fd::col_of(g, c.x, iy, ix) : 0];
        wv[c9] = ok ? x : 0ull;
    }
    unsigned w = row_cost;
#pragma unroll
    for (int c9 = 0; c9 < 9; ++c9) {
        for (int kz = 0; kz < 3; ++kz) {
            const int iz = c.y - 1 + kz;
            const bool v = iz >= 0 && iz < g.D && ((wv[c9] >> iz) & 1ull);
            const unsigned long long m = __ballot(v);
            const unsigned byte = (unsigned)(m >> (8 * (lane & 7))) & 0xffu;
            w += (unsigned)__popc(byte) * 2u + (byte ? 1u : 0u);
        }
    }
    if (lane < 8 && wave * 8 + lane < n_blocks) work[wave * 8 + lane] = w;
}

}

extern "C" int64_t fd_spconv_plan_stride(int64_t n_out) { return n_out < 0 ? 0 : sk::plan_stride_for(n_out); }
extern "C" size_t fd_spconv_plan_bytes(int64_t n_out) { return n_out < 0 ? 0 : sizeof(int32_t) * (size_t)sk::kPlanRows * (size_t)sk::plan_stride_for(n_out); }

extern "C" int fd_spconv_plan_wanted(int cin, int cout, int dtype) {
    if (dtype != 0 || cin != cout || fd::tuning(fd::kTuneSpconvV1) || fd::tuning(fd::kTuneSpconvPlan) < 0) return 0;
    return cin == 32 || cin == 64 || cin == 128;
// ... 135 lines not shown
```

### futuredet_amd/hip_ops.py

```python
import ctypes
import threading

import numpy as np
import torch

from . import lib as _lib
from .lib import DecodeCfg, FutureDetHipError, MapView, check


_raw_stream = getattr(torch._C, "_cuda_getCurrentRawStream", None)


def _stream():
    if _raw_stream is not None:
        return ctypes.c_void_p(_raw_stream(torch.cuda.current_device()))
    return ctypes.c_void_p(torch.cuda.current_stream().cuda_stream)


def _dev(t, name, dtype=None):
    if not isinstance(t, torch.Tensor) or not t.is_cuda:
        raise FutureDetHipError("%s must be a tensor on the HIP device (got %s); this path has no CPU implementation"
                                % (name, "cpu tensor" if isinstance(t, torch.Tensor) else type(t)))
    if dtype is not None and t.dtype != dtype:
        raise FutureDetHipError("%s must be %s, got %s" % (name, dtype, t.dtype))
    if not t.is_contiguous():
        raise FutureDetHipError("%s must be contiguous" % name)
    return t


def _p(t):
    return ctypes.c_void_p(t.data_ptr()) if t is not None else None


class _Workspace(object):

    def __init__(self):
        self._bufs = {}
        self._scope = threading.local()

    def scope(self, token):
        ws = self

        class _Scope(object):
            def __enter__(self_):
                self_.prev = getattr(ws._scope, "token", None)
                ws._scope.token = token

            def __exit__(self_, *exc):
                ws._scope.token = self_.prev

        return _Scope()

    def release(self, token):
        for key in [k for k in self._bufs if k[2] == ("scope", token)]:
            del self._bufs[key]

    def get(self, tag, nbytes, device):
        token = getattr(self._scope, "token", None)
        key = (tag, device.index, ("scope", token) if token is not None else _stream().value)
        buf = self._bufs.get(key)
        if buf is None or buf.numel() < nbytes:
            buf = torch.empty(max(int(nbytes), 256), dtype=torch.uint8, device=device)
            self._bufs[key] = buf
        return buf


workspace = _Workspace()
_DT = {torch.float32: 0, torch.bfloat16: 1}


def set_tuning(name, value):
    check(_lib.load().fd_tuning_set(name.encode(), int(value)), "fd_tuning_set")


def voxelize(points, voxel_size, coors_range, max_points, max_voxels, batch_idx=0, want_voxels=True, want_mean=False,
             mean_stride=None, coor_cols=3, out=None, n_points_dev=None):
    L = _lib.load()
    points = _dev(points, "points", torch.float32)
    n, ndim = points.shape
    dev = points.device
    rng = (ctypes.c_float * 6)(*[float(np.float32(v)) for v in coors_range])
    vs = (ctypes.c_float * 3)(*[float(np.float32(v)) for v in voxel_size])
    out = dict(out or {})
    if want_voxels and "voxels" not in out:
        out["voxels"] = torch.empty((max_voxels, max_points, ndim), dtype=torch.float32, device=dev)
    if want_mean and "mean" not in out:
        out["mean"] = torch.empty((max_voxels, mean_stride or ndim), dtype=torch.float32, device=dev)
    if "coors" not in out:
        out["coors"] = torch.empty((max_voxels, coor_cols), dtype=torch.int32, device=dev)
    if "num_points" not in out:
        out["num_points"] = torch.empty((max_voxels,), dtype=torch.int32, device=dev)
    if "num_voxels" not in out:
        out["num_voxels"] = torch.zeros((1,), dtype=torch.int32, device=dev)
    mean = out.get("mean") if want_mean else None
    voxels = out.get("voxels") if want_voxels else None
    ws_bytes = L.fd_voxelize_workspace_bytes(n, max_voxels)
    ws = workspace.get("voxelize", ws_bytes, dev)
    check(L.fd_voxelize(_p(points), n, _p(n_points_dev), ndim, rng, vs, int(max_points), int(max_voxels), int(batch_idx), _p(voxels), _p(mean),
                        int(mean.shape[1]) if mean is not None else 0, _p(out["coors"]), int(out["coors"].shape[1]),
                        _p(out["num_points"]), _p(out["num_voxels"]), _p(ws), ws.numel(), _stream()), "fd_voxelize")
    return out


class SparseIndex(object):

    def __init__(self, B, D, H, W, device, words=None, prefix=None):
        L = _lib.load()
        self.B, self.D, self.H, self.W = int(B), int(D), int(H), int(W)
        self.ncols = L.fd_index_num_cols(self.B, self.H, self.W)
        self.words = torch.zeros((self.ncols,), dtype=torch.int64, device=device) if words is None else words
        self.prefix = torch.empty((self.ncols,), dtype=torch.int32, device=device) if prefix is None else prefix
        self.n_dev = None
        self.n = None
        self.coords = None
        self.device = device
        self.static = False
        self.n_expected = 0

    @property
    def spatial_shape(self):
        return [self.D, self.H, self.W]

    def mark(self, coords, n_dev=None, n_max=None):
        L = _lib.load()
        coords = _dev(coords, "coords", torch.int32)
        n_max = coords.shape[0] if n_max is None else n_max
        check(L.fd_index_mark(_p(coords), _p(n_dev), n_max, self.B, self.D, self.H, self.W, _p(self.words), _stream()),
              "fd_index_mark")

    def scan(self, n_dev):
        L = _lib.load()
        ws = workspace.get("index_scan", L.fd_index_workspace_bytes(self.ncols), self.device)
        self.n_dev = n_dev
        check(L.fd_index_scan(_p(self.words), self.ncols, _p(self.prefix), _p(n_dev), _p(ws), ws.numel(), _stream()),
              "fd_index_scan")

    def downsample(self, ksize, stride, pad):
        L = _lib.load()
        od = [(i + 2 * p - (k - 1) - 1) // s + 1 for i, k, s, p in zip(self.spatial_shape, ksize, stride, pad)]
        out = SparseIndex(self.B, od[0], od[1], od[2], self.device)
        check(L.fd_index_downsample(_p(self.words), self.B, self.D, self.H, self.W, (ctypes.c_int * 3)(*ksize),
                                    (ctypes.c_int * 3)(*stride), (ctypes.c_int * 3)(*pad), _p(out.words), _stream()),
              "fd_index_downsample")
        return out

    def finalize(self, n):
        L = _lib.load()
        self.n = int(n)
        self.coords = torch.empty((max(self.n, 1), 4), dtype=torch.int32, device=self.device)[: self.n]
        if self.n:
            check(L.fd_index_coords(_p(self.words), _p(self.prefix), self.B, self.D, self.H, self.W, _p(self.coords),
                                    _stream()), "fd_index_coords")

    def lookup(self, coords, n_dev=None):
        L = _lib.load()
        coords = _dev(coords, "coords", torch.int32)
        row_of = torch.empty((coords.shape[0],), dtype=torch.int32, device=self.device)
        check(L.fd_index_lookup(_p(self.words), _p(self.prefix), self.B, self.D, self.H, self.W, _p(coords), _p(n_dev),
                                coords.shape[0], _p(row_of), _stream()), "fd_index_lookup")
        return row_of

    def rulebook(self, out_index, ksize, stride, pad, fp32_layer=None):
        L = _lib.load()
        assert out_index.n is not None
        if fp32_layer is not None and index_plan_wanted(self, out_index, ksize, *fp32_layer):
            return IndexRulebook(self, out_index, stride, pad)
        K = int(ksize[0] * ksize[1] * ksize[2])
        nstride = max(64, (out_index.n + 63) // 64 * 64)
        nbr = torch.empty((K, nstride), dtype=torch.int32, device=self.device)
        static = getattr(out_index, "static", False)
        if out_index.n == 0:
            nbr.fill_(-1)
            return nbr
        check(L.fd_rulebook(_p(self.words), _p(self.prefix), self.B, self.D, self.H, self.W, _p(out_index.coords), out_index.n,
                            _p(out_index.n_dev), nstride, 0 if static else 1, (ctypes.c_int * 3)(*ksize), (ctypes.c_int * 3)(*stride),
                            (ctypes.c_int * 3)(*pad), _p(nbr), _stream()), "fd_rulebook")
        nbr.n_out = out_index.n
        nbr.n_dev = out_index.n_dev if static else None
        nbr.n_expected = out_index.n_expected if static else 0
        src_static = getattr(self, "static", False)
        nbr.n_in_dev = self.n_dev if src_static else None
        nbr.n_in_expected = self.n_expected if src_static else 0
        return nbr


def index_plan_wanted(src, dst, ksize, cin, cout):
    return (tuple(int(k) for k in ksize) == (3, 3, 3) and bool(dst.n) and bool(src.n) and src.n < (1 << 23) and src.n * cin * 4 < (1 << 31)
            and bool(_lib.load().fd_spconv_index_plan_wanted(int(cin), int(cout), 0)))


class IndexRulebook(object):

    def __init__(self, src, dst, stride, pad):
        static = getattr(dst, "static", False)
        self.src, self.dst, self.stride, self.pad = src, dst, tuple(int(v) for v in stride), tuple(int(v) for v in pad)
        self.shape = (27, max(64, (dst.n + 63) // 64 * 64))
        self.device = src.device
        self.n_out = dst.n
        self.n_dev = dst.n_dev if static else None
        self.n_expected = dst.n_expected if static else 0
        self.ranges, self.plans, self._table = None, {}, None

    def table(self):
        if self._table is None:
            self._table = self.src.rulebook(self.dst, (3, 3, 3), self.stride, self.pad)
        return self._table


def plans_from_index(requests):
    L = _lib.load()
    todo = [(rb, r, int(n), (r.data_ptr() if r is not None else 0, int(n), int(rb.n_out))) for rb, r, n in requests]
    todo = [t for t in todo if t[3] not in t[0].plans]
    out = []
    for at in range(0, len(todo), 8):
        part = todo[at:at + 8]
        srcs = (_lib.PlanSource * len(part))()
        for s, (rb, ranges, n_ranges, key) in zip(srcs, part):
            pstride = int(L.fd_spconv_plan_stride(rb.n_out))
            plan = torch.empty((28, pstride), dtype=torch.int32, device=rb.device)
            s.in_words, s.in_prefix, s.out_coords = rb.src.words.data_ptr(), rb.src.prefix.data_ptr(), rb.dst.coords.data_ptr()
            s.n_out_dev = rb.n_dev.data_ptr() if rb.n_dev is not None else None
            s.ranges = ranges.data_ptr() if ranges is not None else None
            s.plan, s.n_out, s.plan_stride = plan.data_ptr(), rb.n_out, pstride
            s.Din, s.Hin, s.Win, s.n_ranges = rb.src.D, rb.src.H, rb.src.W, n_ranges
            s.stride[:], s.pad[:] = list(rb.stride), list(rb.pad)
            rb.plans[key] = (plan, pstride, ranges)
            out.append(plan)
        check(L.fd_spconv_plan_from_index(part[0][0].src.B, len(part), srcs, _stream()), "fd_spconv_plan_from_index")
    return out


class _PyramidPlan(object):

    def __init__(self, B, shape0, geoms, device):
        L = _lib.load()
        self.B, self.geoms, self.device = int(B), geoms, device
        self.shapes = [tuple(int(v) for v in shape0)]
        for ks, st, pd in geoms:
            self.shapes.append(tuple((i + 2 * p - (k - 1) - 1) // s + 1 for i, k, s, p in zip(self.shapes[-1], ks, st, pd)))
        self.ncols = [L.fd_index_num_cols(self.B, sh[1], sh[2]) for sh in self.shapes]
        self.ws_bytes = L.fd_index_workspace_bytes(sum(self.ncols) + 2048 * len(self.ncols))

    def row_caps(self, cap0):
        caps = [min(int(cap0), self.B * int(np.prod(self.shapes[0])))]
        for (ks, st, pd), sh in zip(self.geoms, self.shapes[1:]):
            fan = int(np.prod([-(-k // s) for k, s in zip(ks, st)]))
            caps.append(min(caps[-1] * fan, self.B * int(np.prod(sh))))
        return caps


_pyramid_plans = {}


def build_pyramid(coors, nvox, n_max, B, shape0, geoms, device, static=False, expected=None, row_caps=None):
    L = _lib.load()
    key = (int(B), tuple(int(v) for v in shape0), tuple((tuple(k), tuple(s), tuple(p)) for k, s, p in geoms), str(device))
    plan = _pyramid_plans.get(key)
    if plan is None:
        plan = _pyramid_plans[key] = _PyramidPlan(B, shape0, geoms, device)
    shapes, ncols = plan.shapes, plan.ncols
    words_all = torch.empty((sum(ncols),), dtype=torch.int64, device=device)
    prefix_all = torch.empty((sum(ncols),), dtype=torch.int32, device=device)
    counts = torch.empty((len(shapes),), dtype=torch.int32, device=device)
    idx, off = [], 0
    levels = (_lib.IndexLevel * len(shapes))()
    wp, pp = words_all.data_ptr(), prefix_all.data_ptr()
    for l, (sh, nc) in enumerate(zip(shapes, ncols)):
        ix = SparseIndex.__new__(SparseIndex)
        ix.B, ix.D, ix.H, ix.W, ix.ncols, ix.device = plan.B, sh[0], sh[1], sh[2], nc, device
        ix.words, ix.prefix = words_all[off:off + nc], prefix_all[off:off + nc]
        ix.n_dev, ix.n, ix.coords = counts[l:l + 1], None, None
        ix.level_counts = counts
        ix.static, ix.n_expected = False, 0
        lv = levels[l]
        lv.D, lv.H, lv.W = sh
        if l:
            ks, st, pd = geoms[l - 1]
            lv.ksize[:], lv.stride[:], lv.pad[:] = list(ks), list(st), list(pd)
        lv.words, lv.prefix, lv.coords = wp + 8 * off, pp + 4 * off, None
        idx.append(ix)
        off += nc
    ws = workspace.get("index_scan", plan.ws_bytes, device)

    def size_coords(host):
        total = sum(host)
        coords_all = torch.empty((max(total, 1), 4), dtype=torch.int32, device=device)
        o = 0
        for l, ix in enumerate(idx):
            ix.n = int(host[l])
            ix.coords = coords_all[o:o + ix.n]
            levels[l].coords = (coords_all.data_ptr() + 16 * o) if ix.n else None
            levels[l].coords_rows = ix.n
            o += ix.n

    if static:
        host = plan.row_caps(int(B) * int(n_max))
        if row_caps is not None:
            host = [min(int(a), int(b)) for a, b in zip(host, row_caps)]
        for l, ix in enumerate(idx):
            ix.static = True
            ix.n_expected = int(expected[l]) if expected is not None else 0
        size_coords(host)
        fused = all(int(h) > 0 for h in host)
        check(L.fd_index_pyramid(_p(coors), _p(nvox), int(n_max), plan.B, len(shapes), levels, _p(counts), _p(ws), ws.numel(), _stream()),
              "fd_index_pyramid")
        if not fused:
            check(L.fd_index_pyramid_coords(plan.B, len(shapes), levels, _stream()), "fd_index_pyramid_coords")
        return idx
    check(L.fd_index_pyramid(_p(coors), _p(nvox), int(n_max), plan.B, len(shapes), levels, _p(counts), _p(ws), ws.numel(), _stream()),
          "fd_index_pyramid")
    size_coords(counts.tolist())
    check(L.fd_index_pyramid_coords(plan.B, len(shapes), levels, _stream()), "fd_index_pyramid_coords")
    return idx


def ranges_for(nbr, cin, cout):
    cached = getattr(nbr, "ranges", None)
    if cached is not None:
        return cached
    L = _lib.load()
    n_out = getattr(nbr, "n_out", None)
    if not n_out:
        return None, 0
    K, nstride = nbr.shape
    n = int(L.fd_spconv_num_ranges(getattr(nbr, "n_expected", 0) or n_out, cin, cout, 0))
    if n <= 0:
        return None, 0
    ranges = torch.empty((n + 1,), dtype=torch.int32, device=nbr.device)
    ws = workspace.get("spconv_ranges", L.fd_spconv_ranges_workspace_bytes(n_out), nbr.device)
    if isinstance(nbr, IndexRulebook):
        ix = nbr.dst
        check(L.fd_spconv_ranges_from_index(_p(ix.words), ix.B, ix.D, ix.H, ix.W, _p(ix.coords), n_out, _p(nbr.n_dev), n, _p(ranges), _p(ws),
                                            ws.numel(), _stream()), "fd_spconv_ranges_from_index")
    else:
        check(L.fd_spconv_ranges(_p(nbr), nstride, K, n_out, _p(getattr(nbr, "n_dev", None)), n, _p(ranges), _p(ws), ws.numel(), _stream()),
              "fd_spconv_ranges")
    nbr.ranges = (ranges, n)
    return nbr.ranges


def row_split(nbr, n_out, cin, cout, balanced=None):
    L = _lib.load()
    if balanced is None:
        balanced = nbr.shape[0] == 27 and cin == cout and bool(L.fd_spconv_wants_balanced_ranges(cin, cout, 0))
    if balanced == "tiles":
        return None, 0
    if balanced:
        return ranges_for(nbr, cin, cout)
    return None, int(L.fd_spconv_num_ranges(getattr(nbr, "n_expected", 0) or n_out, cin, cout, 0))


def plan_for(nbr, n_out, ranges, n_ranges):
    key = (ranges.data_ptr() if ranges is not None else 0, int(n_ranges), int(n_out))
    if isinstance(nbr, IndexRulebook):
        assert int(n_out) == nbr.n_out
        plans_from_index([(nbr, ranges, n_ranges)])
        return nbr.plans[key][:2]
    plans = getattr(nbr, "plans", None)
    if plans is None:
        plans = nbr.plans = {}
    if key not in plans:
        L = _lib.load()
        K, nstride = nbr.shape
        pstride = int(L.fd_spconv_plan_stride(n_out))
        plan = torch.empty((28, pstride), dtype=torch.int32, device=nbr.device)
        check(L.fd_spconv_plan_build(_p(nbr), nstride, K, n_out, _p(getattr(nbr, "n_dev", None)), _p(ranges), int(n_ranges), _p(plan), pstride,
                                     _stream()), "fd_spconv_plan_build")
        plans[key] = (plan, pstride, ranges)
    return plans[key][:2]


def rows_permute(src, row_of, c_dst, dtype=torch.float32, n_rows=None, n_dev=None):
    L = _lib.load()
    src = _dev(src, "src", torch.float32)
    row_of = _dev(row_of, "row_of", torch.int32)
    n_rows = src.shape[0] if n_rows is None else n_rows
    dst = torch.zeros((max(n_rows, 1), c_dst), dtype=dtype, device=src.device)[:n_rows]
    if src.shape[0]:
        check(L.fd_rows_permute(_p(src), src.shape[1], _p(row_of), _p(n_dev), src.shape[0], _p(dst), c_dst,
                                _DT[dtype], _stream()), "fd_rows_permute")
    return dst


def rows_place(index, coords, src, c_dst, dtype=torch.float32, n_dev=None, out=None):
    L = _lib.load()
    coords = _dev(coords, "coords", torch.int32)
    src = _dev(src, "src", torch.float32)
    if out is None:
        out = torch.zeros((max(index.n, 1), c_dst), dtype=dtype, device=src.device)[: index.n]
    _dev(out, "out", dtype)
    if coords.dim() != 2 or coords.shape[1] != 4:
        raise FutureDetHipError("rows_place: coords must be [n, 4] (b, z, y, x), got %s" % (tuple(coords.shape),))
    if src.dim() != 2 or src.shape[0] < coords.shape[0]:
        raise FutureDetHipError("rows_place: src must be [n, c_src] with a row per coordinate")
    if out.dim() != 2 or out.shape[1] != c_dst or index.n is None or out.shape[0] < index.n:
        raise FutureDetHipError("rows_place: out must be [rows >= index.n, %d] (finalised index), got %s" % (c_dst, tuple(out.shape)))
    check(L.fd_rows_place(_p(index.words), _p(index.prefix), index.B, index.D, index.H, index.W, _p(coords), _p(n_dev),
                          coords.shape[0], _p(src), src.shape[1], _p(out), c_dst, _DT[dtype], _stream()), "fd_rows_place")
    return out


def pack_spconv_weight(w_kio, dtype=torch.float32):
    L = _lib.load()
    dev = w_kio.device
    w = w_kio.detach().to("cpu", torch.float32).contiguous()
    K, cin, cout = w.shape
    nbytes = L.fd_spconv_packed_weight_bytes(K, cin, cout, _DT[dtype])
    host = torch.empty((nbytes,), dtype=torch.uint8)
    check(L.fd_spconv_pack_weight(ctypes.c_void_p(w.data_ptr()), K, cin, cout, _DT[dtype], ctypes.c_void_p(host.data_ptr())),
          "fd_spconv_pack_weight")
    return host.to(dev)


PACK_PLAIN, PACK_TRANSPOSED, PACK_FLIPPED_TRANSPOSED = 0, 1, 2
_PACK_DEVICE = {torch.float32: "fd_spconv_pack_weight_device", torch.bfloat16: "fd_spconv_pack_weight_device_bf16"}
_WGRAD = {torch.float32: ("fd_spconv_wgrad", "fd_spconv_wgrad_workspace_bytes", "spconv_wgrad"),
          torch.bfloat16: ("fd_spconv_wgrad_bf16", "fd_spconv_wgrad_bf16_workspace_bytes", "spconv_wgrad_bf16")}


def pack_spconv_weight_device(w_kio, mode=PACK_PLAIN, dtype=torch.float32):
    L = _lib.load()
    if dtype not in _DT:
        raise FutureDetHipError("pack_spconv_weight_device: dtype must be float32 or bfloat16 (got %s)" % (dtype,))
    w = _dev(w_kio.detach(), "w_kio", torch.float32)
    K, cin, cout = w.shape
    ci, co = (cout, cin) if mode else (cin, cout)
    out = torch.empty((L.fd_spconv_packed_weight_bytes(K, ci, co, _DT[dtype]),), dtype=torch.uint8, device=w.device)
    name = _PACK_DEVICE[dtype]
    check(getattr(L, name)(_p(w), K, cin, cout, int(mode), _p(out), _stream()), name)
    return out


def spconv_wgrad(feats, dy, nbr, n_out):
    L = _lib.load()
    if feats.dtype != dy.dtype or feats.dtype not in _DT:
        raise FutureDetHipError("spconv_wgrad: feats and dy must both be float32 or both bfloat16 (got %s and %s)" % (feats.dtype, dy.dtype))
    feats = _dev(feats, "feats")
    dy = _dev(dy, "dy")
    K, nstride = nbr.shape
    cin, cout = feats.shape[1], dy.shape[1]
    assert dy.shape[0] >= n_out
    dw = torch.empty((K, cin, cout), dtype=torch.float32, device=feats.device)
    name, ws_bytes, tag = _WGRAD[feats.dtype]
    ws = workspace.get(tag, getattr(L, ws_bytes)(K, n_out, cin, cout), feats.device)
    check(getattr(L, name)(_p(feats), feats.shape[0], _p(dy), _p(_dev(nbr, "nbr", torch.int32)), nstride, K, n_out,
                           _p(getattr(nbr, "n_dev", None)), cin, cout, _p(dw), _p(ws), ws.numel(), _stream()), name)
    return dw


def assign_targets(boxes, counts, classes, trajectory, cfg, out):
    L = _lib.load()
    boxes = _dev(boxes, "boxes", torch.float32)
    B = boxes.shape[0]
    assert tuple(boxes.shape) == (B, cfg.T, cfg.n_max, 12), (tuple(boxes.shape), cfg.T, cfg.n_max)
    assert tuple(counts.shape) == (B, cfg.T) and tuple(classes.shape) == (B, cfg.T, cfg.n_max)
    assert (trajectory is None) == (cfg.n_sets == 1)
    if trajectory is not None:
        assert tuple(trajectory.shape) == (B, cfg.T, cfg.n_max)
        trajectory = _dev(trajectory, "trajectory", torch.int32)
    U = cfg.n_tasks + (2 if cfg.n_sets == 3 else 0)
    ws = workspace.get("targets", L.fd_targets_workspace_bytes(B, cfg.T, U, cfg.max_objs), boxes.device)
    check(L.fd_assign_targets(_p(boxes), _p(_dev(counts, "counts", torch.int32)), _p(_dev(classes, "classes", torch.int32)), _p(trajectory), B,
                              ctypes.byref(cfg), _p(_dev(out["hm"], "hm", torch.float32)), _p(_dev(out["ind"], "ind", torch.int64)),
                              _p(_dev(out["mask"], "mask", torch.uint8)), _p(_dev(out["cat"], "cat", torch.int64)),
                              _p(_dev(out["anno_box"], "anno_box", torch.float32)), _p(_dev(out["gt_boxes_and_cls"], "gt_boxes_and_cls", torch.float32)),
                              _p(_dev(out["status"], "status", torch.int32)), _p(ws), ws.numel(), _stream()), "fd_assign_targets")
    return out


def rulebook_transpose(nbr, n_out, n_in):
    L = _lib.load()
    K, nstride = nbr.shape
    istride = max(64, (n_in + 63) // 64 * 64)
    inv = torch.empty((K, istride), dtype=torch.int32, device=nbr.device)
    check(L.fd_rulebook_transpose(_p(_dev(nbr, "nbr", torch.int32)), nstride, K, n_out, _p(getattr(nbr, "n_dev", None)), n_in, _p(inv),
                                  istride, _stream()), "fd_rulebook_transpose")
    return inv


def dense_gather(grad, index, c):
    L = _lib.load()
    if not (isinstance(grad, torch.Tensor) and grad.is_cuda and grad.dtype == torch.float32):
        raise FutureDetHipError("dense_gather: grad must be a float32 tensor on the HIP device")
    n = int(index.n)
    feats = torch.empty((max(n, 1), c), dtype=torch.float32, device=grad.device)[:n]
    sb, sc, sy, sx = grad.stride()
    check(L.fd_dense_gather(_p(grad), sb, sc, sy, sx, index.D, _p(index.coords), n, _p(index.n_dev if index.static else None), c,
                            _p(feats), _stream()), "fd_dense_gather")
    return feats


def spconv_apply(feats, wpacked, bias, nbr, n_out, cout, residual=None, relu=False, out=None, balanced=None, plan=None):
    L = _lib.load()
    feats = _dev(feats, "feats")
    dt = _DT[feats.dtype]
    cin = feats.shape[1]
    out_dtype, out_cols = feats.dtype, cout
    from_index = isinstance(nbr, IndexRulebook)
    if from_index and (plan is False or dt != 0 or n_out != nbr.n_out or not index_plan_wanted(nbr.src, nbr.dst, (3, 3, 3), cin, cout)):
        nbr, from_index = nbr.table(), False
    K, nstride = nbr.shape
    if out is None:
        out = torch.empty((max(n_out, 1), out_cols), dtype=out_dtype, device=feats.device)[:n_out]
    if residual is not None:
        _dev(residual, "residual", out_dtype)
    n_dev, n_expected = getattr(nbr, "n_dev", None), getattr(nbr, "n_expected", 0)
    ranges, n_ranges = row_split(nbr, n_out, cin, cout, balanced) if dt == 0 and n_out > 0 else (None, 0)
    if plan is None:
        plan = from_index or (dt == 0 and n_out > 0 and K == 27 and cin == cout and bool(L.fd_spconv_plan_wanted(cin, cout, 0)))
    if plan:
        plan_t, pstride = plan_for(nbr if from_index else _dev(nbr, "nbr", torch.int32), n_out, ranges, n_ranges)
        check(L.fd_spconv_apply_plan(_p(feats), feats.shape[0], _p(_dev(wpacked, "wpacked")), _p(bias), _p(residual), int(bool(relu)),
                                     None if from_index else _p(nbr), nstride, _p(ranges), n_ranges, K, n_out, _p(n_dev), int(n_expected or 0),
                                     cin, cout, dt, _p(out), _p(plan_t), pstride, _stream()),
              "fd_spconv_apply_plan")
        return out
    check(L.fd_spconv_apply(_p(feats), feats.shape[0], _p(_dev(wpacked, "wpacked")), _p(bias), _p(residual), int(bool(relu)),
                            _p(_dev(nbr, "nbr", torch.int32)), nstride, _p(ranges), n_ranges, K, n_out, _p(n_dev), int(n_expected or 0),
                            cin, cout, dt, _p(out), _stream()),
          "fd_spconv_apply")
    return out


def densify(feats, index, out_dtype=None, channels_last=False, out=None):
    L = _lib.load()
    feats = _dev(feats, "feats")
    C = feats.shape[1]
    shape = (index.B, C * index.D, index.H, index.W)
    if out is None:
        out_dtype = out_dtype or feats.dtype
        out = torch.empty(shape, dtype=out_dtype, device=feats.device,
                          memory_format=torch.channels_last if channels_last else torch.contiguous_format)
    else:
        assert tuple(out.shape) == shape and out.is_cuda
        out_dtype = out.dtype
    sb, sc, sy, sx = out.stride()
    check(L.fd_densify(_p(feats), C, _DT[feats.dtype], _p(index.words), _p(index.prefix), index.B, index.D, index.H,
                       index.W, _p(out), _DT[out_dtype], sb, sc, sy, sx, int(feats.shape[0]), _stream()), "fd_densify")
    return out


def pack_conv2d_weight(w_oihw):
    L = _lib.load()
    dev = w_oihw.device
    w = w_oihw.detach().to("cpu", torch.float32).contiguous()
    cout, cin, ks, _ = w.shape
    nbytes = L.fd_conv2d_packed_weight_bytes(cout, cin, ks)
    if nbytes == 0:
        raise FutureDetHipError("fd_conv2d: unsupported weight shape %s" % (tuple(w.shape),))
    host = torch.empty((nbytes,), dtype=torch.uint8)
    check(L.fd_conv2d_pack_weight(ctypes.c_void_p(w.data_ptr()), cout, cin, ks, ctypes.c_void_p(host.data_ptr())),
          "fd_conv2d_pack_weight")
    return host.to(dev)


def conv2d_nhwc_bf16(x, wpk, bias, cout, ks, stride=1, relu=True, out=None, co_off=0, osy=1, osx=1, ooy=0, oox=0):
    L = _lib.load()
    x = _dev(x, "x", torch.bfloat16)
    B, H, W, cin = x.shape
    pad = 1 if ks == 3 else 0
    Ho, Wo = (H + 2 * pad - ks) // stride + 1, (W + 2 * pad - ks) // stride + 1
    if out is None:
        out = torch.empty((B, Ho * osy, Wo * osx, cout), dtype=torch.bfloat16, device=x.device)
    _dev(out, "out", torch.bfloat16)
    check(L.fd_conv2d_nhwc_bf16(_p(x), B, H, W, cin, _p(wpk), _p(bias), cout, ks, stride, pad, int(bool(relu)), _p(out),
                                out.shape[3], co_off, osy, osx, ooy, oox, _stream()), "fd_conv2d_nhwc_bf16")
    return out


def pack_conv2d_weight_device(w, transposed=False):
    L = _lib.load()
    w = _dev(w.detach(), "w", torch.float32)
    if w.dim() != 4 or w.shape[2] != w.shape[3]:
        raise FutureDetHipError("pack_conv2d_weight_device: need a [Cout, Cin, k, k] weight (got %s)" % (tuple(w.shape),))
    cout, cin, ks, _ = w.shape
    if transposed and cout % 32:
        raise FutureDetHipError("pack_conv2d_weight_device: the transposed weights need Cout %% 32 == 0 (got %s)" % (tuple(w.shape),))
    nbytes = L.fd_conv2d_packed_weight_bytes(cin, cout, ks) if transposed else L.fd_conv2d_packed_weight_bytes(cout, cin, ks)
    if nbytes == 0:
        raise FutureDetHipError("fd_conv2d: unsupported weight shape %s" % (tuple(w.shape),))
    out = torch.empty((nbytes,), dtype=torch.uint8, device=w.device)
    check(L.fd_conv2d_pack_weight_dev(_p(w), cout, cin, ks, int(bool(transposed)), _p(out), _stream()), "fd_conv2d_pack_weight_dev")
    return out


def conv2d_wgrad_bf16_chunk():
    return int(_lib.load().fd_conv2d_wgrad_bf16_chunk())


def conv2d_wgrad_bf16(x_nhwc, dy_nhwc, ks):
    L = _lib.load()
    x = _dev(x_nhwc, "x_nhwc", torch.bfloat16)
    dy = _dev(dy_nhwc, "dy_nhwc", torch.bfloat16)
    if x.dim() != 4 or dy.dim() != 4 or x.shape[:3] != dy.shape[:3]:
        raise FutureDetHipError("conv2d_wgrad_bf16: x [B,H,W,Cin] and dy [B,H,W,Cout] must cover the same pixels (got %s and %s)"
                                % (tuple(x.shape), tuple(dy.shape)))
    B, H, W, cin = x.shape
    cout = dy.shape[3]
    nbytes = L.fd_conv2d_wgrad_bf16_workspace_bytes(B, H, W, cin, cout, ks)
    if nbytes == 0:
        raise FutureDetHipError("conv2d_wgrad_bf16: unsupported problem %s -> %d channels, ks %s" % (tuple(x.shape), cout, ks))
    ws = torch.empty((nbytes,), dtype=torch.uint8, device=x.device)
    dw = torch.empty((cout, cin, ks, ks), dtype=torch.float32, device=x.device)
    check(L.fd_conv2d_wgrad_bf16(_p(x), _p(dy), B, H, W, cin, cout, ks, _p(ws), ws.numel(), _p(dw), _stream()), "fd_conv2d_wgrad_bf16")
    return dw


def _map4(t, name):
    t = _dev(t, name, torch.bfloat16)
    if t.dim() != 4:
        raise FutureDetHipError("%s must be a [B, H, W, C] map (got %s)" % (name, tuple(t.shape)))
    return t


def _out_map(out, shape, like, name):
    if out is None:
        return torch.empty(shape, dtype=torch.bfloat16, device=like.device)
    _dev(out, name, torch.bfloat16)
    if tuple(out.shape) != tuple(shape):
        raise FutureDetHipError("%s must be %s (got %s)" % (name, tuple(shape), tuple(out.shape)))
    return out


def conv2d_s2_dgrad_bf16(dy_nhwc, wpk_t, H, W, cin, out=None):
    L = _lib.load()
    dy = _map4(dy_nhwc, "dy_nhwc")
    B, Ho, Wo, cout = dy.shape
    if H < 1 or W < 1 or (Ho, Wo) != ((H - 1) // 2 + 1, (W - 1) // 2 + 1):
        raise FutureDetHipError("conv2d_s2_dgrad_bf16: dy %s is not the stride-2 map of %d x %d" % (tuple(dy.shape), H, W))
    _dev(wpk_t, "wpk_t", torch.uint8)
    if wpk_t.numel() != L.fd_conv2d_packed_weight_bytes(cin, cout, 3) or wpk_t.numel() == 0:
        raise FutureDetHipError("conv2d_s2_dgrad_bf16: wpk_t is not the transposed pack of a [%d, %d, 3, 3] weight" % (cout, cin))
    out = _out_map(out, (B, H, W, cin), dy, "out")
    check(L.fd_conv2d_s2_dgrad_bf16(_p(dy), B, H, W, cin, cout, _p(wpk_t), _p(out), _stream()), "fd_conv2d_s2_dgrad_bf16")
    return out


def conv2d_wgrad_s2_bf16(x_nhwc, dy_nhwc):
    L = _lib.load()
    x, dy = _map4(x_nhwc, "x_nhwc"), _map4(dy_nhwc, "dy_nhwc")
    B, H, W, cin = x.shape
    cout = dy.shape[3]
    if tuple(dy.shape[:3]) != (B, (H - 1) // 2 + 1, (W - 1) // 2 + 1):
        raise FutureDetHipError("conv2d_wgrad_s2_bf16: dy %s is not the stride-2 map of x %s" % (tuple(dy.shape), tuple(x.shape)))
    nbytes = L.fd_conv2d_wgrad_s2_bf16_workspace_bytes(B, H, W, cin, cout)
    if nbytes == 0:
        raise FutureDetHipError("conv2d_wgrad_s2_bf16: unsupported problem %s -> %d channels" % (tuple(x.shape), cout))
    ws = torch.empty((nbytes,), dtype=torch.uint8, device=x.device)
    dw = torch.empty((cout, cin, 3, 3), dtype=torch.float32, device=x.device)
    check(L.fd_conv2d_wgrad_s2_bf16(_p(x), _p(dy), B, H, W, cin, cout, _p(ws), ws.numel(), _p(dw), _stream()), "fd_conv2d_wgrad_s2_bf16")
    return dw


PACK_UP2, PACK_DOWN2 = 0, 1


def pack_conv2d_weight_2x2_device(w, kind, fine_major=False):
    L = _lib.load()
    w = _dev(w.detach(), "w", torch.float32)
    if w.dim() != 4 or tuple(w.shape[2:]) != (2, 2) or kind not in (PACK_UP2, PACK_DOWN2):
        raise FutureDetHipError("pack_conv2d_weight_2x2_device: need a [Ccoarse, Cfine, 2, 2] weight and kind PACK_UP2 or PACK_DOWN2 (got %s, %r)"
                                % (tuple(w.shape), kind))
    cc, cf = (w.shape[1], w.shape[0]) if fine_major else (w.shape[0], w.shape[1])
    nbytes = L.fd_conv2d_packed_weight_2x2_bytes(cc, cf, kind)
    if nbytes == 0:
        raise FutureDetHipError("pack_conv2d_weight_2x2_device: unsupported weight shape %s for kind %d" % (tuple(w.shape), kind))
    out = torch.empty((nbytes,), dtype=torch.uint8, device=w.device)
    check(L.fd_conv2d_pack_weight_2x2_dev(_p(w), cc, cf, kind, int(bool(fine_major)), _p(out), _stream()), "fd_conv2d_pack_weight_2x2_dev")
    return out


def conv2d_up2_bf16(x_nhwc, wpk4, c_fine, out=None):
    x = _map4(x_nhwc, "x_nhwc")
    B, H, W, cc = x.shape
    _dev(wpk4, "wpk4", torch.uint8)
    per = _lib.load().fd_conv2d_packed_weight_bytes(c_fine, cc, 1)
    if per == 0 or wpk4.numel() != 4 * per:
        raise FutureDetHipError("conv2d_up2_bf16: wpk4 is not the PACK_UP2 pack of a [%d, %d, 2, 2] weight" % (cc, c_fine))
    out = _out_map(out, (B, 2 * H, 2 * W, c_fine), x, "out")
    for tap in range(4):
        conv2d_nhwc_bf16(x, wpk4[tap * per:(tap + 1) * per], None, c_fine, 1, stride=1, relu=False, out=out, osy=2, osx=2, ooy=tap >> 1, oox=tap & 1)
    return out


def conv2d_down2_bf16(x_nhwc, wpk, c_coarse, out=None):
    L = _lib.load()
    x = _map4(x_nhwc, "x_nhwc")
    B, H, W, cf = x.shape
    _dev(wpk, "wpk", torch.uint8)
    if wpk.numel() != L.fd_conv2d_packed_weight_2x2_bytes(c_coarse, cf, PACK_DOWN2) or wpk.numel() == 0:
        raise FutureDetHipError("conv2d_down2_bf16: wpk is not the PACK_DOWN2 pack of a [%d, %d, 2, 2] weight" % (c_coarse, cf))
    out = _out_map(out, (B, H // 2, W // 2, c_coarse), x, "out")
    check(L.fd_conv2d_down2_bf16(_p(x), B, H, W, cf, _p(wpk), c_coarse, _p(out), _stream()), "fd_conv2d_down2_bf16")
    return out


def conv2d_wgrad_2x2_bf16(coarse_nhwc, fine_nhwc, fine_major=False):
    L = _lib.load()
    co, fi = _map4(coarse_nhwc, "coarse_nhwc"), _map4(fine_nhwc, "fine_nhwc")
    B, H, W, cf = fi.shape
    cc = co.shape[3]
    if tuple(co.shape[:3]) != (B, H // 2, W // 2):
        raise FutureDetHipError("conv2d_wgrad_2x2_bf16: coarse %s is not the 2 x 2 / stride 2 map of fine %s" % (tuple(co.shape), tuple(fi.shape)))
    nbytes = L.fd_conv2d_wgrad_2x2_bf16_workspace_bytes(B, H, W, cc, cf)
    if nbytes == 0:
        raise FutureDetHipError("conv2d_wgrad_2x2_bf16: unsupported problem %s, %s" % (tuple(co.shape), tuple(fi.shape)))
    ws = torch.empty((nbytes,), dtype=torch.uint8, device=fi.device)
    dw = torch.empty((cf, cc, 2, 2) if fine_major else (cc, cf, 2, 2), dtype=torch.float32, device=fi.device)
    check(L.fd_conv2d_wgrad_2x2_bf16(_p(co), _p(fi), B, H, W, cc, cf, int(bool(fine_major)), _p(ws), ws.numel(), _p(dw), _stream()),
          "fd_conv2d_wgrad_2x2_bf16")
    return dw


def head_tail_max_groups():
    return int(_lib.load().fd_head_tail_bf16_max_groups())


def head_tail_wgrad_chunk():
    return int(_lib.load().fd_head_tail_wgrad_bf16_chunk())


def _head_tail_group(what, x, c0, w, bias, y):
    x = _dev(x, what + ": x", torch.bfloat16)
    w = _dev(w, what + ": weight", torch.float32)
    y = _dev(y, what + ": y", torch.float32)
    if bias is not None:
        bias = _dev(bias, what + ": bias", torch.float32)
    if x.dim() != 4 or w.dim() != 4 or tuple(w.shape[2:]) != (3, 3) or y.dim() != 4:
        raise FutureDetHipError("%s: needs x [B, H, W, C], a [k, cin, 3, 3] weight and y [B, k, H, W] (got %s, %s, %s)"
                                % (what, tuple(x.shape), tuple(w.shape), tuple(y.shape)))
    k, cin = int(w.shape[0]), int(w.shape[1])
    B, H, W, C = x.shape
    if tuple(y.shape) != (B, k, H, W) or (bias is not None and tuple(bias.shape) != (k,)):
        raise FutureDetHipError("%s: y must be [%d, %d, %d, %d] and the bias [%d] (got %s, %s)"
                                % (what, B, k, H, W, k, tuple(y.shape), None if bias is None else tuple(bias.shape)))
    if c0 < 0 or c0 % 8 or c0 + cin > C:
        raise FutureDetHipError("%s: channels %d .. %d are no 16-byte aligned slice of the %d channels of x" % (what, c0, c0 + cin - 1, C))
    rec = _lib.HeadTailGroup(x.data_ptr() + 2 * c0, w.data_ptr(), bias.data_ptr() if bias is not None else None, y.data_ptr(), C, cin, k)
    return rec, (B, H, W)


def _head_tail_launch(what, entry, records, with_workspace=False):
    L = _lib.load()
    shapes = set(s for _, s in records)
    if len(shapes) != 1:
        raise FutureDetHipError("%s: needs at least one group, all over the same B x H x W pixels (got %s)" % (what, sorted(shapes)))
    B, H, W = shapes.pop()
    step = head_tail_max_groups()
    for i in range(0, len(records), step):
        part = [r for r, _ in records[i:i + step]]
        arr = (_lib.HeadTailGroup * len(part))(*part)
        if with_workspace:
            nbytes = L.fd_head_tail_wgrad_bf16_workspace_bytes(B, H, W, sum(r.cin for r in part))
            if nbytes == 0:
                raise FutureDetHipError("%s: unsupported problem %d x %d x %d, cin %s" % (what, B, H, W, [r.cin for r in part]))
            ws = workspace.get("head_tail_wgrad", nbytes, torch.device("cuda", torch.cuda.current_device()))
            check(getattr(L, entry)(arr, len(part), B, H, W, _p(ws), ws.numel(), _stream()), entry)
        else:
            check(getattr(L, entry)(arr, len(part), B, H, W, _stream()), entry)


def head_tail_forward(groups):
    recs, ys = [], []
    for x, c0, w, bias in groups:
        x = _dev(x, "head_tail_forward: x", torch.bfloat16)
        w = _dev(w, "head_tail_forward: weight", torch.float32)
        if x.dim() != 4 or w.dim() != 4:
            raise FutureDetHipError("head_tail_forward: needs x [B, H, W, C] and a [k, cin, 3, 3] weight (got %s, %s)" % (tuple(x.shape), tuple(w.shape)))
        if bias is None:
            raise FutureDetHipError("head_tail_forward: every group needs a bias")
        y = torch.empty((x.shape[0], w.shape[0], x.shape[1], x.shape[2]), dtype=torch.float32, device=x.device)
        recs.append(_head_tail_group("head_tail_forward", x, c0, w, bias, y))
        ys.append(y)
    _head_tail_launch("head_tail_forward", "fd_head_tail_forward_bf16", recs)
    return ys


def head_tail_dgrad(groups):
    recs = [_head_tail_group("head_tail_dgrad", dx, c0, w, None, dy) for dx, c0, w, dy in groups]
    _head_tail_launch("head_tail_dgrad", "fd_head_tail_dgrad_bf16", recs)


def head_tail_wgrad(groups):
    recs, out = [], []
    for x, c0, cin, dy in groups:
        dy = _dev(dy, "head_tail_wgrad: dy", torch.float32)
        if dy.dim() != 4:
            raise FutureDetHipError("head_tail_wgrad: dy must be [B, k, H, W] (got %s)" % (tuple(dy.shape),))
        dw = torch.empty((dy.shape[1], cin, 3, 3), dtype=torch.float32, device=dy.device)
        db = torch.empty((dy.shape[1],), dtype=torch.float32, device=dy.device)
        recs.append(_head_tail_group("head_tail_wgrad", x, c0, dw, db, dy))
        out.append((dw, db))
    _head_tail_launch("head_tail_wgrad", "fd_head_tail_wgrad_bf16", recs, with_workspace=True)
    return out


def pack_conv2d_weight_f32(w_oihw):
    L = _lib.load()
    dev = w_oihw.device
    w = w_oihw.detach().to("cpu", torch.float32).contiguous()
    cout, cin, ks, _ = w.shape
    nbytes = L.fd_conv2d_f32_packed_weight_bytes(cout, cin, ks)
    if nbytes == 0:
        raise FutureDetHipError("fd_conv2d_f32: unsupported weight shape %s" % (tuple(w.shape),))
    host = torch.empty((nbytes,), dtype=torch.uint8)
    check(L.fd_conv2d_f32_pack_weight(ctypes.c_void_p(w.data_ptr()), cout, cin, ks, ctypes.c_void_p(host.data_ptr())),
          "fd_conv2d_f32_pack_weight")
    return host.to(dev)


def conv2d_nhwc_f32(x, wpk, bias, cout, ks, stride=1, relu=True, out=None, co_off=0, osy=1, osx=1, ooy=0, oox=0, tile=0):
    L = _lib.load()
# ... 1146 lines not shown
```

### futuredet_amd/lib.py

```python
import ctypes
import os

_HERE = os.path.dirname(os.path.abspath(__file__))
LIB_PATH = os.environ.get("FD_LIB_PATH") or os.path.join(_HERE, "libfuturedet_hip.so")
_lib = None

c_void_p = ctypes.c_void_p
c_int = ctypes.c_int
c_i64 = ctypes.c_int64
c_size_t = ctypes.c_size_t
c_float = ctypes.c_float


class MapView(ctypes.Structure):
    _fields_ = [("data", ctypes.c_void_p), ("group_stride", ctypes.c_int64), ("channel_stride", ctypes.c_int64), ("cell_stride", ctypes.c_int64),
                ("dtype", ctypes.c_int)]


ABI_VERSION = 8


class DecodeCfg(ctypes.Structure):
    _fields_ = [("H", c_int), ("W", c_int), ("out_size_factor", c_float), ("voxel_x", c_float), ("voxel_y", c_float),
                ("pc_x", c_float), ("pc_y", c_float), ("score_threshold", c_float), ("center_range", c_float * 6),
                ("nms_iou_threshold", c_float), ("nms_pre_max", c_int), ("nms_post_max", c_int), ("hm_channels", c_int),
                ("nms_kind", c_int), ("n_radius", c_int), ("circle_radius", c_float * 16)]


class IndexLevel(ctypes.Structure):
    _fields_ = [("D", ctypes.c_int32), ("H", ctypes.c_int32), ("W", ctypes.c_int32), ("ksize", ctypes.c_int32 * 3),
                ("stride", ctypes.c_int32 * 3), ("pad", ctypes.c_int32 * 3), ("words", c_void_p), ("prefix", c_void_p),
                ("coords", c_void_p), ("coords_rows", ctypes.c_int64)]


class PlanSource(ctypes.Structure):
    _fields_ = [("in_words", c_void_p), ("in_prefix", c_void_p), ("out_coords", c_void_p), ("n_out_dev", c_void_p), ("ranges", c_void_p),
                ("plan", c_void_p), ("n_out", ctypes.c_int64), ("plan_stride", ctypes.c_int64), ("Din", ctypes.c_int32), ("Hin", ctypes.c_int32),
                ("Win", ctypes.c_int32), ("n_ranges", ctypes.c_int32), ("stride", ctypes.c_int32 * 3), ("pad", ctypes.c_int32 * 3)]


class ForecastBuffers(ctypes.Structure):
    _fields_ = [(n, c_void_p) for n in ("center", "quat", "velocity", "size", "fwd_idx", "fwd_ok", "bwd_idx", "bwd_ok", "match_idx", "cv_centers",
                                        "status", "traj_kind", "traj_src", "traj_first", "traj_group", "n_traj")]


class TargetsCfg(ctypes.Structure):
    _fields_ = [("H", c_int), ("W", c_int), ("T", c_int), ("n_max", c_int), ("max_objs", c_int), ("n_sets", c_int), ("n_tasks", c_int),
                ("task_classes", c_int * 16), ("radius_mult", c_int), ("min_radius", c_int), ("out_size_factor", c_float), ("voxel_x", c_float),
                ("voxel_y", c_float), ("pc_x", c_float), ("pc_y", c_float), ("gaussian_overlap", ctypes.c_double)]


class OptimTable(ctypes.Structure):
    _fields_ = [(n, c_void_p) for n in ("params", "numel", "offset", "flags", "step", "coef", "chunks", "partials", "norm", "grad", "exp_avg",
                                        "exp_avg_sq")] + [("total", c_i64), ("n_tensors", ctypes.c_int32), ("n_chunks", ctypes.c_int32),
                                                          ("chunk", ctypes.c_int32)]


class LossCfg(ctypes.Structure):
    _fields_ = [(n, ctypes.c_int32) for n in ("B", "H", "W", "M", "n_tasks", "dense", "T", "D", "row_stride")] + [
        ("col", ctypes.c_int32 * 14), ("code_weights", ctypes.c_double * 14), ("code_weights_forecast", ctypes.c_double * 14),
        ("weight", ctypes.c_double)]


class LossTask(ctypes.Structure):
    _fields_ = [("hm", c_void_p), ("hm_target", c_void_p), ("ind", c_void_p), ("cat", c_void_p), ("mask", c_void_p * 7), ("maps", c_void_p * 7),
                ("anno_box", c_void_p * 7), ("C", ctypes.c_int32), ("sig", c_void_p), ("d_hm", c_void_p), ("d_maps", c_void_p * 7)]


class HeadTailGroup(ctypes.Structure):
    _fields_ = [("x", c_void_p), ("w", c_void_p), ("bias", c_void_p), ("y", c_void_p), ("x_stride", c_i64), ("cin", c_int), ("k", c_int)]


class DenseBnNhwcGroup(ctypes.Structure):
    _fields_ = [("gamma", c_void_p), ("beta", c_void_p), ("running_mean", c_void_p), ("running_var", c_void_p), ("num_batches_tracked", c_void_p),
                ("c", c_int), ("eps", c_float), ("momentum", ctypes.c_double)]


class AugmentRecord(ctypes.Structure):
    _fields_ = [("flip_a", ctypes.c_int32), ("flip_b", ctypes.c_int32), ("c", c_float), ("s", c_float), ("rot", c_float), ("scale", c_float),
                ("tx", ctypes.c_double), ("ty", ctypes.c_double), ("tz", ctypes.c_double)]


class AugmentMaskRecord(ctypes.Structure):
    _fields_ = [("flip_a", ctypes.c_int32), ("flip_b", ctypes.c_int32), ("m1", ctypes.c_double * 6), ("m2", ctypes.c_double * 6)]


SIGNATURES = {
    "fd_abi_version": (c_int, []),
    "fd_last_error": (ctypes.c_char_p, []),
    "fd_tuning_set": (c_int, [ctypes.c_char_p, c_int]),
    "fd_voxelize_workspace_bytes": (c_size_t, [c_i64, c_i64]),
    "fd_voxelize": (c_int, [c_void_p, c_i64, c_void_p, c_int, c_void_p, c_void_p, c_int, c_i64, c_int, c_void_p, c_void_p, c_int,
                            c_void_p, c_int, c_void_p, c_void_p, c_void_p, c_size_t, c_void_p]),
    "fd_index_num_cols": (c_i64, [c_int, c_int, c_int]),
    "fd_index_workspace_bytes": (c_size_t, [c_i64]),
    "fd_index_mark": (c_int, [c_void_p, c_void_p, c_i64, c_int, c_int, c_int, c_int, c_void_p, c_void_p]),
    "fd_index_downsample": (c_int, [c_void_p, c_int, c_int, c_int, c_int, c_void_p, c_void_p, c_void_p, c_void_p, c_void_p]),
    "fd_index_scan": (c_int, [c_void_p, c_i64, c_void_p, c_void_p, c_void_p, c_size_t, c_void_p]),
    "fd_index_coords": (c_int, [c_void_p, c_void_p, c_int, c_int, c_int, c_int, c_void_p, c_void_p]),
    "fd_index_lookup": (c_int, [c_void_p, c_void_p, c_int, c_int, c_int, c_int, c_void_p, c_void_p, c_i64, c_void_p, c_void_p]),
    "fd_rows_permute": (c_int, [c_void_p, c_int, c_void_p, c_void_p, c_i64, c_void_p, c_int, c_int, c_void_p]),
    "fd_rulebook": (c_int, [c_void_p, c_void_p, c_int, c_int, c_int, c_int, c_void_p, c_i64, c_void_p, c_i64, c_int, c_void_p, c_void_p,
                            c_void_p, c_void_p, c_void_p]),
    "fd_spconv_packed_weight_bytes": (c_size_t, [c_int, c_int, c_int, c_int]),
    "fd_spconv_pack_weight": (c_int, [c_void_p, c_int, c_int, c_int, c_int, c_void_p]),
    "fd_spconv_apply": (c_int, [c_void_p, c_i64, c_void_p, c_void_p, c_void_p, c_int, c_void_p, c_i64, c_void_p, c_int, c_int, c_i64,
                                c_void_p, c_i64, c_int, c_int, c_int, c_void_p, c_void_p]),
    "fd_spconv_num_ranges": (c_int, [c_i64, c_int, c_int, c_int]),
    "fd_spconv_wants_balanced_ranges": (c_int, [c_int, c_int, c_int]),
    "fd_spconv_ranges_workspace_bytes": (c_size_t, [c_i64]),
    "fd_spconv_ranges": (c_int, [c_void_p, c_i64, c_int, c_i64, c_void_p, c_int, c_void_p, c_void_p, c_size_t, c_void_p]),
    "fd_spconv_plan_stride": (c_i64, [c_i64]),
    "fd_spconv_plan_bytes": (c_size_t, [c_i64]),
    "fd_spconv_plan_wanted": (c_int, [c_int, c_int, c_int]),
    "fd_spconv_plan_build": (c_int, [c_void_p, c_i64, c_int, c_i64, c_void_p, c_void_p, c_int, c_void_p, c_i64, c_void_p]),
    "fd_spconv_apply_plan": (c_int, [c_void_p, c_i64, c_void_p, c_void_p, c_void_p, c_int, c_void_p, c_i64, c_void_p, c_int, c_int, c_i64,
                                     c_void_p, c_i64, c_int, c_int, c_int, c_void_p, c_void_p, c_i64, c_void_p]),
    "fd_spconv_index_plan_wanted": (c_int, [c_int, c_int, c_int]),
    "fd_spconv_plan_from_index": (c_int, [c_int, c_int, ctypes.POINTER(PlanSource), c_void_p]),
    "fd_spconv_ranges_from_index": (c_int, [c_void_p, c_int, c_int, c_int, c_int, c_void_p, c_i64, c_void_p, c_int, c_void_p, c_void_p, c_size_t,
                                            c_void_p]),
    "fd_densify": (c_int, [c_void_p, c_int, c_int, c_void_p, c_void_p, c_int, c_int, c_int, c_int, c_void_p, c_int, c_i64,
                           c_i64, c_i64, c_i64, c_i64, c_void_p]),
    "fd_conv2d_packed_weight_bytes": (c_size_t, [c_int, c_int, c_int]),
    "fd_conv2d_pack_weight": (c_int, [c_void_p, c_int, c_int, c_int, c_void_p]),
    "fd_conv2d_nhwc_bf16": (c_int, [c_void_p, c_int, c_int, c_int, c_int, c_void_p, c_void_p, c_int, c_int, c_int, c_int, c_int,
                                    c_void_p, c_int, c_int, c_int, c_int, c_int, c_int, c_void_p]),
    "fd_conv2d_f32_packed_weight_bytes": (c_size_t, [c_int, c_int, c_int]),
    "fd_conv2d_f32_pack_weight": (c_int, [c_void_p, c_int, c_int, c_int, c_void_p]),
    "fd_conv2d_f32_num_tiles": (c_int, []),
    "fd_conv2d_nhwc_f32": (c_int, [c_void_p, c_int, c_int, c_int, c_int, c_void_p, c_void_p, c_int, c_int, c_int, c_int, c_int,
                                   c_void_p, c_int, c_int, c_int, c_int, c_int, c_int, c_int, c_void_p]),
    "fd_conv2d_shuffle_nhwc_f32": (c_int, [c_void_p, c_int, c_int, c_int, c_int, c_void_p, c_void_p, c_int, c_int, c_int, c_void_p, c_int, c_int, c_int,
                                           c_void_p]),
    "fd_conv2d_grouped_nhwc_f32": (c_int, [c_void_p, c_int, c_int, c_int, c_int, c_int, c_void_p, c_void_p, c_void_p, c_int, c_void_p, c_int, c_int,
                                           c_int, c_void_p]),
    "fd_conv2d_wino_f32_num_tiles": (c_int, []),
    "fd_conv2d_wino_f32_packed_weight_bytes": (c_size_t, [c_int, c_int]),
    "fd_conv2d_wino_f32_pack_weight": (c_int, [c_void_p, c_int, c_int, c_void_p]),
    "fd_conv2d_wino_nhwc_f32": (c_int, [c_void_p, c_int, c_int, c_int, c_int, c_void_p, c_void_p, c_int, c_int, c_void_p, c_int, c_int, c_int,
                                        c_void_p]),
    "fd_decode_workspace_bytes": (c_size_t, [c_int, ctypes.POINTER(DecodeCfg)]),
    "fd_centerpoint_decode": (c_int, [c_void_p, c_i64, c_void_p, c_i64, c_void_p, c_i64, c_void_p, c_i64, c_void_p, c_i64,
                                      c_int, ctypes.POINTER(DecodeCfg), c_void_p, c_void_p, c_void_p, c_void_p, c_void_p,
                                      c_size_t, c_void_p]),
    "fd_centerpoint_decode_maps": (c_int, [ctypes.POINTER(MapView)] * 5 + [c_int, ctypes.POINTER(DecodeCfg), c_void_p, c_void_p, c_void_p, c_void_p,
                                           c_void_p, c_size_t, c_void_p]),
    "fd_centerpoint_decode_packed": (c_int, [ctypes.POINTER(MapView)] * 6 + [c_int, c_int, ctypes.POINTER(DecodeCfg), c_int, c_void_p, c_void_p, c_void_p,
                                             c_void_p, c_void_p, c_void_p, c_void_p, c_void_p, c_void_p, c_void_p, c_size_t, c_void_p]),
    "fd_assemble_detections": (c_int, [c_void_p, c_void_p, c_void_p, c_void_p, ctypes.POINTER(MapView), c_int, c_int, c_int, c_void_p, c_void_p,
                                       c_void_p, c_void_p, c_void_p, c_void_p]),
    "fd_nms_workspace_bytes": (c_size_t, [c_int]),
    "fd_rotated_nms": (c_int, [c_void_p, c_int, c_float, c_void_p, c_void_p, c_void_p, c_size_t, c_void_p]),
    "fd_boxes_iou_bev": (c_int, [c_void_p, c_int, c_void_p, c_int, c_void_p, c_void_p]),
    "fd_pillar_encode": (c_int, [c_void_p, c_void_p, c_void_p, c_void_p, c_i64, c_int, c_int, c_int, c_float, c_float, c_float,
                                 c_float, c_void_p, c_void_p, c_void_p, c_int, c_void_p, c_void_p, c_void_p, c_int, c_int,
                                 c_void_p, c_int, c_void_p]),
    "fd_pillar_scatter": (c_int, [c_void_p, c_int, c_int, c_int, c_void_p, c_void_p, c_i64, c_int, c_int, c_int, c_void_p, c_int,
                                  c_i64, c_i64, c_i64, c_i64, c_int, c_void_p]),
    "fd_forecast_chains": (c_int, [c_void_p, c_void_p, c_void_p, c_void_p, c_int, c_int, ctypes.c_double, c_void_p, c_void_p,
                                   c_void_p, c_void_p, c_void_p, c_void_p, c_void_p, c_void_p]),
    "fd_det_to_global_boxes": (c_int, [c_void_p, c_int, c_void_p, c_void_p, c_void_p, c_void_p, c_void_p, c_void_p, c_void_p, c_void_p, c_void_p]),
    "fd_forecast_groups": (c_int, [c_void_p, c_int, ctypes.c_double, c_void_p, c_void_p]),
    "fd_forecast_from_detections": (c_int, [c_void_p, c_void_p, c_int, c_int, c_int, c_int, c_void_p, c_void_p, ctypes.c_double, ctypes.c_double,
                                            ctypes.POINTER(ForecastBuffers), c_void_p]),
    "fd_nearest_rows": (c_int, [c_void_p, c_int, c_void_p, c_int, c_int, c_void_p, c_void_p]),
    "fd_index_pyramid": (c_int, [c_void_p, c_void_p, c_i64, c_int, c_int, ctypes.POINTER(IndexLevel), c_void_p, c_void_p, c_size_t,
                                 c_void_p]),
    "fd_index_pyramid_coords": (c_int, [c_int, c_int, ctypes.POINTER(IndexLevel), c_void_p]),
    "fd_rows_place": (c_int, [c_void_p, c_void_p, c_int, c_int, c_int, c_int, c_void_p, c_void_p, c_i64, c_void_p, c_int, c_void_p,
                              c_int, c_int, c_void_p]),
    "fd_sweep_assemble_workspace_bytes": (c_size_t, [c_i64]),
    "fd_sweep_assemble": (c_int, [c_void_p, c_int, c_int, c_i64, c_void_p, c_int, c_float, c_void_p, c_void_p, c_void_p,
                                  c_size_t, c_void_p]),
    "fd_deform_adapt_packed_weight_bytes": (c_size_t, [c_int]),
    "fd_deform_adapt_pack_weight": (c_int, [c_void_p, c_void_p, c_int, c_void_p]),
    "fd_deform_adapt_nhwc": (c_int, [c_void_p, c_int, c_int, c_int, c_int, c_int, c_void_p, c_void_p, c_void_p, c_void_p, c_void_p, c_void_p]),
    "fd_deform_adapt_backward_workspace_bytes": (c_size_t, [c_int, c_int, c_int]),
    "fd_deform_adapt_backward": (c_int, [c_void_p, c_void_p, c_void_p, c_void_p, c_void_p, c_void_p, c_int, c_int, c_int, c_int, c_void_p, c_void_p,
                                         c_void_p, c_void_p, c_size_t, c_void_p]),
    "fd_deform_adapt_pack_weight_device": (c_int, [c_void_p, c_void_p, c_void_p, c_void_p]),
    "fd_spconv_wgrad_workspace_bytes": (c_size_t, [c_int, c_i64, c_int, c_int]),
    "fd_spconv_wgrad": (c_int, [c_void_p, c_i64, c_void_p, c_void_p, c_i64, c_int, c_i64, c_void_p, c_int, c_int, c_void_p, c_void_p, c_size_t,
                                c_void_p]),
    "fd_rulebook_transpose": (c_int, [c_void_p, c_i64, c_int, c_i64, c_void_p, c_i64, c_void_p, c_i64, c_void_p]),
    "fd_spconv_pack_weight_device": (c_int, [c_void_p, c_int, c_int, c_int, c_int, c_void_p, c_void_p]),
    "fd_spconv_wgrad_bf16_workspace_bytes": (c_size_t, [c_int, c_i64, c_int, c_int]),
    "fd_spconv_wgrad_bf16": (c_int, [c_void_p, c_i64, c_void_p, c_void_p, c_i64, c_int, c_i64, c_void_p, c_int, c_int, c_void_p, c_void_p, c_size_t,
                                     c_void_p]),
    "fd_spconv_pack_weight_device_bf16": (c_int, [c_void_p, c_int, c_int, c_int, c_int, c_void_p, c_void_p]),
    "fd_conv2d_pack_weight_dev": (c_int, [c_void_p, c_int, c_int, c_int, c_int, c_void_p, c_void_p]),
    "fd_conv2d_wgrad_bf16_chunk": (c_int, []),
    "fd_conv2d_wgrad_bf16_workspace_bytes": (c_size_t, [c_int, c_int, c_int, c_int, c_int, c_int]),
    "fd_conv2d_wgrad_bf16": (c_int, [c_void_p, c_void_p, c_int, c_int, c_int, c_int, c_int, c_int, c_void_p, c_size_t, c_void_p, c_void_p]),
    "fd_conv2d_s2_dgrad_bf16": (c_int, [c_void_p, c_int, c_int, c_int, c_int, c_int, c_void_p, c_void_p, c_void_p]),
    "fd_conv2d_wgrad_s2_bf16_workspace_bytes": (c_size_t, [c_int, c_int, c_int, c_int, c_int]),
    "fd_conv2d_wgrad_s2_bf16": (c_int, [c_void_p, c_void_p, c_int, c_int, c_int, c_int, c_int, c_void_p, c_size_t, c_void_p, c_void_p]),
    "fd_conv2d_down2_bf16": (c_int, [c_void_p, c_int, c_int, c_int, c_int, c_void_p, c_int, c_void_p, c_void_p]),
    "fd_conv2d_packed_weight_2x2_bytes": (c_size_t, [c_int, c_int, c_int]),
    "fd_conv2d_pack_weight_2x2_dev": (c_int, [c_void_p, c_int, c_int, c_int, c_int, c_void_p, c_void_p]),
    "fd_conv2d_wgrad_2x2_bf16_workspace_bytes": (c_size_t, [c_int, c_int, c_int, c_int, c_int]),
    "fd_conv2d_wgrad_2x2_bf16": (c_int, [c_void_p, c_void_p, c_int, c_int, c_int, c_int, c_int, c_int, c_void_p, c_size_t, c_void_p, c_void_p]),
    "fd_head_tail_bf16_max_groups": (c_int, []),
    "fd_head_tail_wgrad_bf16_chunk": (c_int, []),
    "fd_head_tail_wgrad_bf16_workspace_bytes": (c_size_t, [c_int, c_int, c_int, c_int]),
    "fd_head_tail_forward_bf16": (c_int, [ctypes.POINTER(HeadTailGroup), c_int, c_int, c_int, c_int, c_void_p]),
    "fd_head_tail_dgrad_bf16": (c_int, [ctypes.POINTER(HeadTailGroup), c_int, c_int, c_int, c_int, c_void_p]),
    "fd_head_tail_wgrad_bf16": (c_int, [ctypes.POINTER(HeadTailGroup), c_int, c_int, c_int, c_int, c_void_p, c_size_t, c_void_p]),
    "fd_dense_gather": (c_int, [c_void_p, c_i64, c_i64, c_i64, c_i64, c_int, c_void_p, c_i64, c_void_p, c_int, c_void_p, c_void_p]),
    "fd_pillar_train_workspace_bytes": (c_size_t, [c_i64, c_int]),
    "fd_pillar_train_forward": (c_int, [c_void_p, c_void_p, c_void_p, c_i64, c_int, c_int, c_int, c_float, c_float, c_float, c_float,
                                        c_void_p, c_void_p, c_void_p, c_int, c_float, c_void_p, c_void_p, c_void_p, c_int, c_float,
                                        c_void_p, c_void_p, c_void_p, c_void_p, c_void_p, c_void_p, c_size_t, c_void_p]),
    "fd_pillar_train_backward": (c_int, [c_void_p, c_void_p, c_void_p, c_i64, c_int, c_int, c_int, c_float, c_float, c_float, c_float,
                                         c_void_p, c_void_p, c_void_p, c_int, c_void_p, c_void_p, c_void_p, c_int, c_void_p,
                                         c_void_p, c_void_p, c_void_p, c_void_p, c_void_p, c_void_p, c_void_p, c_size_t, c_void_p]),
    "fd_pillar_train_forward_dev": (c_int, [c_void_p, c_void_p, c_void_p, c_void_p, c_int, c_i64, c_int, c_int, c_int, c_float, c_float,
                                            c_float, c_float, c_void_p, c_void_p, c_void_p, c_int, c_float, c_void_p, c_void_p, c_void_p,
                                            c_int, c_float, c_void_p, c_void_p, c_void_p, c_void_p, c_void_p, c_void_p, c_size_t, c_void_p]),
    "fd_pillar_train_backward_dev": (c_int, [c_void_p, c_void_p, c_void_p, c_void_p, c_int, c_i64, c_int, c_int, c_int, c_float, c_float,
                                             c_float, c_float, c_void_p, c_void_p, c_void_p, c_int, c_void_p, c_void_p, c_void_p, c_int,
                                             c_void_p, c_void_p, c_void_p, c_void_p, c_void_p, c_void_p, c_void_p, c_void_p, c_size_t,
                                             c_void_p]),
    "fd_pillar_train_running_stats_dev": (c_int, [c_void_p, c_void_p, c_int, ctypes.c_double, c_void_p, c_int, c_i64, c_int, c_void_p,
                                                  c_void_p, c_void_p, c_void_p]),
    "fd_targets_workspace_bytes": (c_size_t, [c_int, c_int, c_int, c_int]),
    "fd_assign_targets": (c_int, [c_void_p, c_void_p, c_void_p, c_void_p, c_int, ctypes.POINTER(TargetsCfg), c_void_p, c_void_p, c_void_p, c_void_p,
                                  c_void_p, c_void_p, c_void_p, c_void_p, c_size_t, c_void_p]),
    "fd_optim_chunk": (c_int, []),
    "fd_optim_zero_grad": (c_int, [ctypes.POINTER(OptimTable), c_void_p]),
    "fd_optim_adam_step": (c_int, [ctypes.POINTER(OptimTable)] + [ctypes.c_double] * 6 + [c_void_p]),
    "fd_optim_adam_step_dev": (c_int, [ctypes.POINTER(OptimTable), c_void_p, c_int, c_void_p, c_void_p]),
    "fd_rows_colsum_chunk": (c_int, []),
    "fd_rows_colsum_workspace_bytes": (c_size_t, [c_i64, c_int]),
    "fd_rows_colsum": (c_int, [c_void_p, c_i64, c_void_p, c_int, c_int, c_void_p, c_void_p, c_size_t, c_void_p]),
    "fd_levels_overflow": (c_int, [c_void_p, c_void_p, c_int, c_void_p, c_void_p]),
    "fd_augment_points": (c_int, [c_void_p, c_i64, c_int, c_void_p, c_void_p, c_void_p, c_void_p]),
    "fd_augment_boxes": (c_int, [c_void_p, c_void_p, c_void_p, c_void_p, c_int, c_int, c_int, c_void_p]),
    "fd_gt_range_filter": (c_int, [c_void_p, c_void_p, c_void_p, c_void_p, c_float, c_float, c_float, c_float, c_void_p, c_void_p, c_void_p,
                                   c_void_p, c_void_p, c_int, c_int, c_int, c_void_p]),
    "fd_augment_mask": (c_int, [c_void_p, c_void_p, c_void_p, c_int, c_int, c_int, c_int, c_void_p]),
    "fd_augment_mask_check": (c_int, [c_void_p, c_int, c_int, c_int]),
    "fd_loss_chunk": (c_int, []),
    "fd_centerhead_loss_terms": (c_size_t, [ctypes.POINTER(LossCfg)]),
    "fd_centerhead_loss_workspace_bytes": (c_size_t, [ctypes.POINTER(LossCfg), c_int]),
    "fd_centerhead_loss_forward": (c_int, [ctypes.POINTER(LossCfg), ctypes.POINTER(LossTask), c_void_p, c_void_p, c_size_t, c_void_p]),
    "fd_centerhead_loss_backward": (c_int, [ctypes.POINTER(LossCfg), ctypes.POINTER(LossTask), c_void_p, c_void_p, c_void_p, c_size_t, c_void_p]),
    "fd_sparse_bn_chunk": (c_int, []),
    "fd_sparse_bn_workspace_bytes": (c_size_t, [c_i64, c_int]),
    "fd_sparse_bn_train_forward": (c_int, [c_void_p, c_void_p, c_void_p, c_void_p, c_i64, c_void_p, c_int, c_int, c_float, ctypes.c_double,
                                           c_void_p, c_void_p, c_void_p, c_void_p, c_void_p, c_void_p, c_size_t, c_void_p]),
    "fd_sparse_bn_train_backward": (c_int, [c_void_p, c_void_p, c_void_p, c_void_p, c_void_p, c_i64, c_void_p, c_int, c_int,
                                            c_void_p, c_void_p, c_void_p, c_void_p, c_void_p, c_size_t, c_void_p]),
    "fd_dense_bn_chunk": (c_int, []),
    "fd_dense_bn_workspace_bytes": (c_size_t, [c_i64, c_int, c_i64]),
    "fd_dense_bn_train_forward": (c_int, [c_void_p, c_void_p, c_void_p, c_i64, c_int, c_i64, c_int, c_float, ctypes.c_double,
                                          c_void_p, c_void_p, c_void_p, c_void_p, c_void_p, c_void_p, c_size_t, c_void_p]),
    "fd_dense_bn_train_backward": (c_int, [c_void_p, c_void_p, c_void_p, c_void_p, c_void_p, c_i64, c_int, c_i64, c_int,
                                           c_void_p, c_void_p, c_void_p, c_void_p, c_size_t, c_void_p]),
    "fd_dense_bn_nhwc_chunk": (c_int, []),
    "fd_dense_bn_nhwc_stat_groups": (c_int, []),
    "fd_dense_bn_nhwc_apply_blocks": (c_int, []),
    "fd_dense_bn_nhwc_workspace_bytes": (c_size_t, [c_i64, c_int]),
    "fd_dense_bn_nhwc_train_forward_bf16": (c_int, [c_void_p, ctypes.POINTER(DenseBnNhwcGroup), c_int, c_i64, c_int, c_int, c_void_p, c_void_p,
                                                    c_void_p, c_size_t, c_void_p]),
    "fd_dense_bn_nhwc_train_backward_bf16": (c_int, [c_void_p, c_void_p, c_void_p, c_void_p, ctypes.POINTER(DenseBnNhwcGroup), c_int, c_i64, c_int,
                                                     c_int, c_void_p, c_void_p, c_void_p, c_void_p, c_size_t, c_void_p]),
}
for _name in ("fd_sparse_bn_train_forward", "fd_sparse_bn_train_backward"):
    SIGNATURES[_name + "_bf16"] = SIGNATURES[_name]



class FutureDetHipError(RuntimeError):
    pass


def load():
    global _lib
    if _lib is None:
        if not os.path.isfile(LIB_PATH):
            raise FutureDetHipError(
                "libfuturedet_hip.so is not built (%s). Run `python -c 'import __graft_entry__ as g; g.build()'` "
                "or `python futuredet_amd/build.py`; there is no CPU fallback for this path." % LIB_PATH)
        L = ctypes.CDLL(LIB_PATH)
        for name, (res, args) in SIGNATURES.items():
            fn = getattr(L, name)
            fn.restype = res
            fn.argtypes = args
        if L.fd_abi_version() != ABI_VERSION:
            raise FutureDetHipError("%s reports ABI %d, these bindings are written for %d: rebuild it (python futuredet_amd/build.py --force)"
                                    % (LIB_PATH, L.fd_abi_version(), ABI_VERSION))
        _lib = L
    return _lib


def check(status, what):
    if status != 0:
        msg = load().fd_last_error()
        raise FutureDetHipError("%s failed (%d): %s" % (what, status, msg.decode() if msg else "?"))
```

### include/futuredet_hip.h

```cpp
#ifndef FUTUREDET_HIP_H
#define FUTUREDET_HIP_H

#include <stddef.h>
#include <stdint.h>

#ifdef __cplusplus
extern "C" {
#endif

#define FD_OK 0
#define FD_EINVAL (-1)
#define FD_EWORKSPACE (-2)
#define FD_ELAUNCH (-3)

typedef void *fd_stream_t;

int fd_abi_version(void);
const char *fd_last_error(void);
int fd_tuning_set(const char *name, int value);

size_t fd_voxelize_workspace_bytes(int64_t n_points, int64_t max_voxels);
int fd_voxelize(const float *points, int64_t n_points, const int32_t *n_points_dev, int ndim, const float *range6_host,
                const float *voxel_size3_host, int max_points, int64_t max_voxels, int batch_idx,
                float *out_voxels, float *out_mean, int mean_stride, int32_t *out_coors, int coor_cols,
                int32_t *out_num_points, int32_t *out_num_voxels, void *workspace, size_t workspace_bytes,
                fd_stream_t stream);

int64_t fd_index_num_cols(int B, int H, int W);
size_t fd_index_workspace_bytes(int64_t num_cols);
int fd_index_mark(const int32_t *coords , const int32_t *n_dev ,
                  int64_t n_max, int B, int D, int H, int W, uint64_t *words, fd_stream_t stream);
int fd_index_downsample(const uint64_t *in_words, int B, int D, int H, int W, const int *ksize3,
                        const int *stride3, const int *pad3, uint64_t *out_words, fd_stream_t stream);
int fd_index_scan(const uint64_t *words, int64_t num_cols, int32_t *prefix, int32_t *n_active_dev,
                  void *workspace, size_t workspace_bytes, fd_stream_t stream);
int fd_index_coords(const uint64_t *words, const int32_t *prefix, int B, int D, int H, int W,
                    int32_t *coords , fd_stream_t stream);
int fd_index_lookup(const uint64_t *words, const int32_t *prefix, int B, int D, int H, int W,
                    const int32_t *coords_in, const int32_t *n_dev, int64_t n_max, int32_t *row_of,
                    fd_stream_t stream);
int fd_rows_permute(const float *src, int c_src, const int32_t *row_of, const int32_t *n_dev, int64_t n_max,
                    void *dst, int c_dst, int dst_bf16, fd_stream_t stream);
int fd_rulebook(const uint64_t *in_words, const int32_t *in_prefix, int B, int Din, int Hin, int Win,
                const int32_t *out_coords, int64_t out_rows, const int32_t *n_out_dev, int64_t nbr_stride, int fill_tail, const int *ksize3,
                const int *stride3, const int *pad3, int32_t *nbr, fd_stream_t stream);

size_t fd_spconv_packed_weight_bytes(int K, int cin, int cout, int dtype);
int fd_spconv_pack_weight(const float *w_kio_host, int K, int cin, int cout, int dtype, void *wpacked_host);
int fd_spconv_apply(const void *in_feats, int64_t n_in, const void *wpacked, const float *bias, const void *residual,
                    int relu, const int32_t *nbr, int64_t nbr_stride, const int32_t *ranges ,
                    int n_ranges, int K, int64_t n_out, const int32_t *n_out_dev ,
                    int64_t n_expected ,
                    int cin, int cout, int dtype, void *out_feats, fd_stream_t stream);
int fd_spconv_num_ranges(int64_t n_out, int cin, int cout, int dtype);
int fd_spconv_wants_balanced_ranges(int cin, int cout, int dtype);
size_t fd_spconv_ranges_workspace_bytes(int64_t n_out);
int fd_spconv_ranges(const int32_t *nbr, int64_t nbr_stride, int K, int64_t n_out, const int32_t *n_out_dev, int n_ranges,
                     int32_t *ranges , void *workspace, size_t workspace_bytes, fd_stream_t stream);
int64_t fd_spconv_plan_stride(int64_t n_out);
size_t fd_spconv_plan_bytes(int64_t n_out);
int fd_spconv_plan_wanted(int cin, int cout, int dtype);
int fd_spconv_plan_build(const int32_t *nbr, int64_t nbr_stride, int K, int64_t n_out, const int32_t *n_out_dev, const int32_t *ranges,
                         int n_ranges, int32_t *plan, int64_t plan_stride, fd_stream_t stream);
int fd_spconv_apply_plan(const void *in_feats, int64_t n_in, const void *wpacked, const float *bias, const void *residual, int relu,
                         const int32_t *nbr, int64_t nbr_stride, const int32_t *ranges, int n_ranges, int K, int64_t n_out,
                         const int32_t *n_out_dev, int64_t n_expected, int cin, int cout, int dtype, void *out_feats, const int32_t *plan,
                         int64_t plan_stride, fd_stream_t stream);
typedef struct fd_plan_source {
    const uint64_t *in_words;
    const int32_t *in_prefix;
    const int32_t *out_coords;
    const int32_t *n_out_dev;
    const int32_t *ranges;
    int32_t *plan;
    int64_t n_out, plan_stride;
    int32_t Din, Hin, Win, n_ranges;
    int32_t stride[3], pad[3];
} fd_plan_source;
int fd_spconv_index_plan_wanted(int cin, int cout, int dtype);
int fd_spconv_plan_from_index(int B, int n_sources, const fd_plan_source *sources_host, fd_stream_t stream);
int fd_spconv_ranges_from_index(const uint64_t *words, int B, int D, int H, int W, const int32_t *coords, int64_t n_out,
                                const int32_t *n_out_dev, int n_ranges, int32_t *ranges , void *workspace,
                                size_t workspace_bytes, fd_stream_t stream);

int fd_densify(const void *feats, int c, int dtype, const uint64_t *words, const int32_t *prefix, int B, int D,
               int H, int W, void *out, int out_dtype, int64_t stride_b, int64_t stride_c, int64_t stride_y,
               int64_t stride_x, int64_t n_rows ,
               fd_stream_t stream);

size_t fd_conv2d_packed_weight_bytes(int cout, int cin, int ks);
int fd_conv2d_pack_weight(const float *w_oihw_host, int cout, int cin, int ks, void *wpacked_host);
int fd_conv2d_nhwc_bf16(const void *x, int B, int H, int W, int cin, const void *wpacked, const float *bias, int cout,
                        int ks, int stride, int pad, int relu, void *y, int cout_total, int co_off, int osy, int osx,
                        int ooy, int oox, fd_stream_t stream);
size_t fd_conv2d_f32_packed_weight_bytes(int cout, int cin, int ks);
int fd_conv2d_f32_pack_weight(const float *w_oihw_host, int cout, int cin, int ks, void *wpacked_host);
int fd_conv2d_f32_num_tiles(void);
int fd_conv2d_nhwc_f32(const float *x, int B, int H, int W, int cin, const void *wpacked, const float *bias, int cout, int ks,
                       int stride, int pad, int relu, float *y, int cout_total, int co_off, int osy, int osx, int ooy, int oox,
                       int tile , fd_stream_t stream);
int fd_conv2d_shuffle_nhwc_f32(const float *x, int B, int H, int W, int cin, const void *wpacked, const float *bias, int cout_sub, int k,
                               int relu, float *y, int cout_total, int co_off, int tile, fd_stream_t stream);
int fd_conv2d_grouped_nhwc_f32(const float *x, int B, int H, int W, int groups, int cin_g, const void *wpacked, const float *bias,
                               const int *counts_host, int relu, float *y, int cout_total, int co_off, int tile, fd_stream_t stream);
int fd_conv2d_wino_f32_num_tiles(void);
size_t fd_conv2d_wino_f32_packed_weight_bytes(int cout, int cin);
int fd_conv2d_wino_f32_pack_weight(const float *w_oihw_host, int cout, int cin, void *wpacked_host);
int fd_conv2d_wino_nhwc_f32(const float *x, int B, int H, int W, int cin, const void *wpacked, const float *bias, int cout, int relu,
                            float *y, int cout_total, int co_off, int tile , fd_stream_t stream);

typedef struct fd_decode_cfg {
    int H, W;
    float out_size_factor, voxel_x, voxel_y, pc_x, pc_y;
    float score_threshold;
    float center_range[6];
    float nms_iou_threshold;
    int nms_pre_max, nms_post_max;
    int hm_channels;
    int nms_kind;
    int n_radius;
    float circle_radius[16];
} fd_decode_cfg;

typedef struct fd_map_view {
    const void *data;
    int64_t group_stride, channel_stride, cell_stride;
    int dtype;
} fd_map_view;

size_t fd_decode_workspace_bytes(int G, const fd_decode_cfg *cfg);
int fd_centerpoint_decode_maps(const fd_map_view *hm, const fd_map_view *reg, const fd_map_view *height, const fd_map_view *dim,
                               const fd_map_view *rot, int G, const fd_decode_cfg *cfg_host, float *out_boxes7, float *out_scores,
                               int32_t *out_cell, int32_t *out_count, void *workspace, size_t workspace_bytes, fd_stream_t stream);
int fd_assemble_detections(const float *boxes7, const float *scores, const int32_t *cell, const int32_t *count, const fd_map_view *vel,
                           int B, int post_max, int S, const int32_t *step_group, const int32_t *step_vel_channel,
                           const int32_t *step_label, float *packed, int32_t *counts_out, fd_stream_t stream);
int fd_centerpoint_decode_packed(const fd_map_view *hm, const fd_map_view *reg, const fd_map_view *height, const fd_map_view *dim,
                                 const fd_map_view *rot, const fd_map_view *vel, int G, int B, const fd_decode_cfg *cfg_host, int S,
                                 const int32_t *step_group, const int32_t *step_vel_channel, const int32_t *step_label, float *out_boxes7,
                                 float *out_scores, int32_t *out_cell, int32_t *out_count, float *packed, int32_t *counts_out, void *workspace,
                                 size_t workspace_bytes, fd_stream_t stream);
int fd_centerpoint_decode(const float *hm, int64_t hm_gstride, const float *reg, int64_t reg_gstride,
                          const float *height, int64_t height_gstride, const float *dim, int64_t dim_gstride,
                          const float *rot, int64_t rot_gstride, int G, const fd_decode_cfg *cfg_host,
                          float *out_boxes7, float *out_scores, int32_t *out_cell, int32_t *out_count,
                          void *workspace, size_t workspace_bytes, fd_stream_t stream);

size_t fd_nms_workspace_bytes(int n);
int fd_rotated_nms(const float *boxes7, int n, float thresh, int64_t *keep, int32_t *out_count,
                   void *workspace, size_t workspace_bytes, fd_stream_t stream);
int fd_boxes_iou_bev(const float *a7, int na, const float *b7, int nb, float *out, fd_stream_t stream);

#define FD_SWEEP_HAS_TRANSFORM 1
#define FD_SWEEP_REMOVE_CLOSE 2
typedef struct fd_sweep_desc {
    double m[16];
    int64_t row_begin, row_end;
    float time;
    int32_t flags;
} fd_sweep_desc;
size_t fd_sweep_assemble_workspace_bytes(int64_t n_rows);
int fd_sweep_assemble(const float *raw, int raw_cols, int keep_cols, int64_t n_rows, const fd_sweep_desc *sweeps_dev,
                      int n_sweeps, float min_distance, float *out_points, int32_t *out_count, void *workspace,
                      size_t workspace_bytes, fd_stream_t stream);

int fd_pillar_encode(const float *voxels, const int32_t *num_points, const int32_t *coors4, const int32_t *n_dev,
                     int64_t m_max, int max_points, int ndim, int with_distance, float vx, float vy, float x_offset,
                     float y_offset, const float *w1, const float *scale1, const float *shift1, int units1,
                     const float *w2, const float *scale2, const float *shift2, int units2, int out_dtype, void *out,
                     int out_stride, fd_stream_t stream);

int fd_pillar_scatter(const void *feats, int c, int feat_stride, int dtype, const int32_t *coors4, const int32_t *n_dev,
                      int64_t m_max, int B, int H, int W, void *out, int out_dtype, int64_t stride_b, int64_t stride_c,
                      int64_t stride_y, int64_t stride_x, int zero_first, fd_stream_t stream);


int fd_forecast_chains(const double *centers, const double *velocity, const int32_t *counts, const double *time_dev, int T,
                       int n_max, double reject_thresh, int32_t *fwd_idx, int32_t *fwd_ok, int32_t *bwd_idx, int32_t *bwd_ok,
                       int32_t *match_idx, double *cv_centers, int32_t *status, fd_stream_t stream);

int fd_det_to_global_boxes(const float *box3d9, int n, const double *cs_rotation4_host, const double *cs_translation3_host,
                           const double *pose_rotation4_host, const double *pose_translation3_host, double *center,
                           double *quat, double *velocity, float *size, fd_stream_t stream);
int fd_forecast_groups(const double *centers3, int n, double match_thresh, int32_t *ids, fd_stream_t stream);

typedef struct fd_forecast_buffers {
    double *center, *quat, *velocity;
    float *size;
    int32_t *fwd_idx, *fwd_ok, *bwd_idx, *bwd_ok, *match_idx;
    double *cv_centers;
    int32_t *status;
    int32_t *traj_kind, *traj_src, *traj_first, *traj_group, *n_traj;
} fd_forecast_buffers;
int fd_forecast_from_detections(const float *packed, const int32_t *counts, int B, int T, int post, int row_floats,
                                const double *records_dev, const double *time_dev, double reject_thresh, double match_thresh,
                                const fd_forecast_buffers *out, fd_stream_t stream);

int fd_nearest_rows(const double *library, int n_library, const double *queries, int n_queries, int dim, int32_t *idx, fd_stream_t stream);

typedef struct fd_index_level {
    int32_t D, H, W;
    int32_t ksize[3], stride[3], pad[3];
    uint64_t *words;
    int32_t *prefix;
    int32_t *coords;
    int64_t coords_rows;
} fd_index_level;
int fd_index_pyramid(const int32_t *coords, const int32_t *n_dev, int64_t n_max_per_sample, int B, int n_levels,
                     const fd_index_level *levels_host, int32_t *counts_dev, void *workspace, size_t workspace_bytes,
                     fd_stream_t stream);
int fd_index_pyramid_coords(int B, int n_levels, const fd_index_level *levels_host, fd_stream_t stream);

int fd_rows_place(const uint64_t *words, const int32_t *prefix, int B, int D, int H, int W, const int32_t *coords_in,
                  const int32_t *n_dev, int64_t n_max, const float *src, int c_src, void *dst, int c_dst, int dst_bf16,
                  fd_stream_t stream);

size_t fd_deform_adapt_packed_weight_bytes(int bf16);
int fd_deform_adapt_pack_weight(const float *w_cls_oihw_host, const float *w_reg_oihw_host, int bf16, void *wpacked_host);
int fd_deform_adapt_nhwc(const void *x, int B, int H, int W, int C, int bf16, const float *off_w, const float *off_b, const float *offsets,
                         const void *wpacked, void *y, fd_stream_t stream);

size_t fd_deform_adapt_backward_workspace_bytes(int B, int H, int W);
int fd_deform_adapt_backward(const float *x, const float *offsets, const float *w_cls_oihw, const float *w_reg_oihw, const float *y, const float *dy,
                             int B, int H, int W, int C, float *dx, float *doffsets, float *dw, void *workspace, size_t workspace_bytes,
                             fd_stream_t stream);
int fd_deform_adapt_pack_weight_device(const float *w_cls_oihw, const float *w_reg_oihw, void *wpacked, fd_stream_t stream);

size_t fd_spconv_wgrad_workspace_bytes(int K, int64_t n_out, int cin, int cout);
int fd_spconv_wgrad(const float *in_feats, int64_t n_in, const float *dy, const int32_t *nbr, int64_t nbr_stride, int K, int64_t n_out,
                    const int32_t *n_out_dev, int cin, int cout, float *dw, void *workspace, size_t workspace_bytes, fd_stream_t stream);
int fd_rulebook_transpose(const int32_t *nbr, int64_t nbr_stride, int K, int64_t n_out, const int32_t *n_out_dev, int64_t n_in, int32_t *inv,
                          int64_t inv_stride, fd_stream_t stream);
int fd_spconv_pack_weight_device(const float *w_kio, int K, int cin, int cout, int mode, void *wpacked, fd_stream_t stream);
int fd_dense_gather(const float *dense, int64_t stride_b, int64_t stride_c, int64_t stride_y, int64_t stride_x, int D, const int32_t *coords,
                    int64_t n_rows, const int32_t *n_dev, int c, float *feats, fd_stream_t stream);

size_t fd_spconv_wgrad_bf16_workspace_bytes(int K, int64_t n_out, int cin, int cout);
int fd_spconv_wgrad_bf16(const void *in_feats, int64_t n_in, const void *dy, const int32_t *nbr, int64_t nbr_stride, int K, int64_t n_out,
                         const int32_t *n_out_dev, int cin, int cout, float *dw, void *workspace, size_t workspace_bytes, fd_stream_t stream);
int fd_spconv_pack_weight_device_bf16(const float *w_kio, int K, int cin, int cout, int mode, void *wpacked, fd_stream_t stream);

int fd_conv2d_pack_weight_dev(const float *w_oihw, int cout, int cin, int ks, int mode, void *wpacked, fd_stream_t stream);
int fd_conv2d_wgrad_bf16_chunk(void);
size_t fd_conv2d_wgrad_bf16_workspace_bytes(int B, int H, int W, int cin, int cout, int ks);
int fd_conv2d_wgrad_bf16(const void *x, const void *dy, int B, int H, int W, int cin, int cout, int ks, void *workspace,
                         size_t workspace_bytes, float *dw, fd_stream_t stream);

typedef struct fd_head_tail_group {
    void *x;
    float *w;
    float *bias;
    void *y;
    int64_t x_stride;
    int cin;
    int k;
} fd_head_tail_group;
int fd_head_tail_bf16_max_groups(void);
int fd_head_tail_wgrad_bf16_chunk(void);
size_t fd_head_tail_wgrad_bf16_workspace_bytes(int B, int H, int W, int cin_sum);
int fd_head_tail_forward_bf16(const fd_head_tail_group *groups, int n_groups, int B, int H, int W, fd_stream_t stream);
int fd_head_tail_dgrad_bf16(const fd_head_tail_group *groups, int n_groups, int B, int H, int W, fd_stream_t stream);
int fd_head_tail_wgrad_bf16(const fd_head_tail_group *groups, int n_groups, int B, int H, int W, void *workspace, size_t workspace_bytes,
                            fd_stream_t stream);

#define FD_TARGETS_MAX_TASKS 16
typedef struct fd_targets_cfg {
    int H, W;
    int T, n_max, max_objs;
    int n_sets;
    int n_tasks;
    int task_classes[FD_TARGETS_MAX_TASKS];
    int radius_mult;
    int min_radius;
    float out_size_factor, voxel_x, voxel_y, pc_x, pc_y;
    double gaussian_overlap;
} fd_targets_cfg;
size_t fd_targets_workspace_bytes(int B, int T, int maps_per_step, int max_objs);
int fd_assign_targets(const float *boxes, const int32_t *counts, const int32_t *classes, const int32_t *trajectory, int B,
                      const fd_targets_cfg *cfg, float *hm, int64_t *ind, uint8_t *mask, int64_t *cat, float *anno_box,
                      float *gt_boxes_and_cls, int32_t *status, void *workspace, size_t workspace_bytes, fd_stream_t stream);

size_t fd_pillar_train_workspace_bytes(int64_t m, int max_points);
int fd_pillar_train_forward(const float *voxels, const int32_t *num_points, const int32_t *coors4, int64_t m, int max_points, int ndim,
                            int with_distance, float vx, float vy, float x_offset, float y_offset, const float *w1, const float *gamma1,
                            const float *beta1, int units1, float eps1, const float *w2, const float *gamma2, const float *beta2, int units2,
                            float eps2, float *out, float *mean1, float *var1, float *mean2, float *var2, void *workspace,
                            size_t workspace_bytes, fd_stream_t stream);
int fd_pillar_train_backward(const float *voxels, const int32_t *num_points, const int32_t *coors4, int64_t m, int max_points, int ndim,
                             int with_distance, float vx, float vy, float x_offset, float y_offset, const float *w1, const float *gamma1,
                             const float *beta1, int units1, const float *w2, const float *gamma2, const float *beta2, int units2,
                             const float *dout, float *dw1, float *dgamma1, float *dbeta1, float *dw2, float *dgamma2, float *dbeta2,
                             void *workspace, size_t workspace_bytes, fd_stream_t stream);

int fd_pillar_train_forward_dev(const float *voxels, const int32_t *num_points, const int32_t *coors4, const int32_t *seg_counts, int n_seg,
                                int64_t seg_stride, int max_points, int ndim, int with_distance, float vx, float vy, float x_offset,
                                float y_offset, const float *w1, const float *gamma1, const float *beta1, int units1, float eps1,
                                const float *w2, const float *gamma2, const float *beta2, int units2, float eps2, float *out, float *mean1,
                                float *var1, float *mean2, float *var2, void *workspace, size_t workspace_bytes, fd_stream_t stream);
int fd_pillar_train_backward_dev(const float *voxels, const int32_t *num_points, const int32_t *coors4, const int32_t *seg_counts, int n_seg,
                                 int64_t seg_stride, int max_points, int ndim, int with_distance, float vx, float vy, float x_offset,
                                 float y_offset, const float *w1, const float *gamma1, const float *beta1, int units1, const float *w2,
                                 const float *gamma2, const float *beta2, int units2, const float *dout, float *dw1, float *dgamma1,
                                 float *dbeta1, float *dw2, float *dgamma2, float *dbeta2, void *workspace, size_t workspace_bytes,
                                 fd_stream_t stream);
int fd_pillar_train_running_stats_dev(const float *mean, const float *var, int channels, double momentum, const int32_t *seg_counts, int n_seg,
                                      int64_t seg_stride, int max_points, float *running_mean, float *running_var,
                                      int64_t *num_batches_tracked, fd_stream_t stream);

#define FD_OPTIM_CHUNK 4096
#define FD_OPTIM_DECAY 1
#define FD_OPTIM_HAS_GRAD 2
typedef struct fd_optim_table {
    const void *params;
    const void *numel, *offset;
    const void *flags;
    void *step;
    void *coef;
    const void *chunks;
    void *partials;
    void *norm;
    float *grad, *exp_avg, *exp_avg_sq;
    int64_t total;
    int32_t n_tensors, n_chunks, chunk;
} fd_optim_table;
int fd_optim_chunk(void);
int fd_optim_zero_grad(const fd_optim_table *table, fd_stream_t stream);
int fd_optim_adam_step(const fd_optim_table *table, double lr, double beta1, double beta2, double eps, double wd, double max_norm,
                       fd_stream_t stream);
int fd_optim_adam_step_dev(const fd_optim_table *table, const double *hyper, int clip, const int32_t *skip, fd_stream_t stream);

#define FD_ROWS_COLSUM_CHUNK 512
int fd_rows_colsum_chunk(void);
size_t fd_rows_colsum_workspace_bytes(int64_t n, int C);
int fd_rows_colsum(const void *x, int64_t n, const int32_t *n_dev, int C, int dtype, float *out, void *workspace, size_t workspace_bytes,
                   fd_stream_t stream);
int fd_levels_overflow(const int32_t *counts, const int32_t *caps, int n_levels, int32_t *flag, fd_stream_t stream);

#define FD_AUGMENT_MAX_ROWS (1 << 28)
typedef struct fd_augment_record {
    int32_t flip_a, flip_b;
    float c, s, rot, scale;
    double tx, ty, tz;
} fd_augment_record;
int fd_augment_points(const float *src, int64_t n_rows, int ndim, const int32_t *perm, const fd_augment_record *rec, float *dst,
                      fd_stream_t stream);
int fd_augment_boxes(const float *boxes, const int32_t *counts, const fd_augment_record *recs, float *out, int B, int T, int n_max,
                     fd_stream_t stream);

#define FD_RANGE_FILTER_MAX_N 4096
#define FD_AUGMENT_MASK_MAX_PIXELS 40960
#define FD_AUGMENT_MASK_MAX_COORD 32000.0
typedef struct fd_augment_mask_record {
    int32_t flip_a, flip_b;
    double m1[6], m2[6];
} fd_augment_mask_record;
int fd_gt_range_filter(const float *boxes, const int32_t *counts, const int32_t *classes, const int32_t *trajectory, float xmin, float ymin,
                       float xmax, float ymax, float *boxes_out, int32_t *counts_out, int32_t *classes_out, int32_t *trajectory_out,
                       int32_t *status, int B, int T, int n_max, fd_stream_t stream);
int fd_augment_mask(const float *src, const fd_augment_mask_record *recs, float *dst, int B, int C, int H, int W, fd_stream_t stream);
int fd_augment_mask_check(const fd_augment_mask_record *recs_host, int B, int H, int W);

#define FD_LOSS_CHUNK 2048
#define FD_LOSS_MAX_TASKS 16
#define FD_LOSS_MAX_STEPS 7
#define FD_LOSS_MAX_OBJS 2048
typedef struct fd_loss_cfg {
    int32_t B;
    int32_t H;
    int32_t W;
    int32_t M;
    int32_t n_tasks;
    int32_t dense;
    int32_t T;
    int32_t D;
    int32_t row_stride;
    int32_t col[14];
    double code_weights[14];
    double code_weights_forecast[14];
    double weight;
} fd_loss_cfg;
typedef struct fd_loss_task {
    const float *hm;
// ... 84 lines not shown
```

Before: 288.6.

## Store sparse-conv level activations in XOR-swizzled row layout to spread LDS/cache banks

Adds a per-row XOR swizzle of 16-byte column pieces for fp32 sparse-conv activations within a residual level. The first conv writes swizzled output, the block convs gather swizzled inputs and residuals, and the last conv un-swizzles its output. By default only the 32-channel level is enabled through a new tuning knob. The swizzle is meant to cut bank or channel conflicts in row gathers, at the cost of extra template variants and index arithmetic in the kernels.

Result: faster. 291.7 (median of 6 runs) (+1.1%).

```diff
diff --git a/futuredet_amd/backbones.py b/futuredet_amd/backbones.py
--- a/futuredet_amd/backbones.py
+++ b/futuredet_amd/backbones.py
@@ -177,11 +177,11 @@
                 rb_cache[key] = src.rulebook(dst, ks, st, pd, fp32_layer=layer)
             return rb_cache[key]
 
-        def run(conv, bn, x, src, dst, relu, residual=None):
+        def run(conv, bn, x, src, dst, relu, residual=None, layout=0):
             wpk, bias, cin_p, cout_p = conv.packed_weight(dt, bn)
             assert x.shape[1] == cin_p, (x.shape, cin_p)
             nbr = rulebook(src, dst, conv)
-            fn = lambda: hip_ops.spconv_apply(x, wpk, bias, nbr, dst.n, cout_p, residual=residual, relu=relu)
+            fn = lambda: hip_ops.spconv_apply(x, wpk, bias, nbr, dst.n, cout_p, residual=residual, relu=relu, layout=layout)
             if self.profile_hook is not None:
                 s = 4 if dt == torch.float32 else 2
                 K = nbr.shape[0]
@@ -252,10 +252,13 @@
             dst = idx[lvl]
             if lvl == 1 and side is not None:
                 main.wait_stream(side)
-            x = run(conv, bn, x, src, dst, relu=True)
-            for blk in blocks:
-                y = run(blk.conv1, blk.bn1, x, dst, dst, relu=True)
-                x = run(blk.conv2, blk.bn2, y, dst, dst, relu=True, residual=x)
+            swz = from_index and lvl >= 1 and len(blocks) > 0 and hip_ops.level_layout(
+                spconv.pad_channels(conv.in_channels), spconv.pad_channels(conv.out_channels), src.n, dst.n)
+            x = run(conv, bn, x, src, dst, relu=True, layout=4 if swz else 0)
+            for i, blk in enumerate(blocks):
+                y = run(blk.conv1, blk.bn1, x, dst, dst, relu=True, layout=5 if swz else 0)
+                last = i + 1 == len(blocks)
+                x = run(blk.conv2, blk.bn2, y, dst, dst, relu=True, residual=x, layout=(3 if last else 7) if swz else 0)
             levels[lvl] = (x, dst)
         bev = hip_ops.densify(x, idx[4], out_dtype=self.dense_dtype or dt, channels_last=self.dense_channels_last, out=dense_out)
         return bev, levels
diff --git a/futuredet_amd/csrc/fd_common.h b/futuredet_amd/csrc/fd_common.h
--- a/futuredet_amd/csrc/fd_common.h
+++ b/futuredet_amd/csrc/fd_common.h
@@ -30,6 +30,7 @@
     hipStream_t stream;
     const int *plan;
     int64_t plan_stride;
+    int layout;
 };
 
 constexpr int kSpconvMaxTaps = 27;
@@ -104,7 +105,7 @@
     X(kTuneSpconvRG, "spconv_rg") X(kTuneSpconvV1, "spconv_v1") X(kTuneConvNT, "conv_nt") X(kTuneV2RangesPerCU, "v2_ranges_per_cu") \
     X(kTuneSpconvC32, "spconv_c32") X(kTuneBf16GP, "bf16_gp") X(kTuneBf16RG, "bf16_rg") X(kTuneBf16Depth, "bf16_depth")        \
     X(kTuneBf16NW, "bf16_nw") X(kTuneBf16Win, "bf16_win") X(kTuneF32ResRG, "f32_res_rg") X(kTuneConvStrip, "conv_strip")       \
-    X(kTuneF32ResNW, "f32_res_nw") X(kTuneSpconvPlan, "spconv_plan")
+    X(kTuneF32ResNW, "f32_res_nw") X(kTuneSpconvPlan, "spconv_plan") X(kTuneSpconvSwz, "spconv_swz")
 #define FD_TUNE_ENUM(key, name) key,
 enum TuneKey { FD_TUNE_KNOBS(FD_TUNE_ENUM) kTuneCount };
 #undef FD_TUNE_ENUM
diff --git a/futuredet_amd/csrc/fd_spconv.hip b/futuredet_amd/csrc/fd_spconv.hip
--- a/futuredet_amd/csrc/fd_spconv.hip
+++ b/futuredet_amd/csrc/fd_spconv.hip
@@ -242,7 +242,7 @@
 namespace {
 int spconv_apply(const void *in_feats, int64_t n_in, const void *wpacked, const float *bias, const void *residual, int relu, const int32_t *nbr,
                  int64_t nbr_stride, const int32_t *ranges, int n_ranges, int K, int64_t n_out, const int32_t *n_out_dev, int64_t n_expected, int cin,
-                 int cout, int dtype, void *out_feats, fd_stream_t stream, const int32_t *plan, int64_t plan_stride) {
+                 int cout, int dtype, void *out_feats, fd_stream_t stream, const int32_t *plan, int64_t plan_stride, int layout = 0) {
     FD_REQUIRE(K >= 1 && K <= fd::kSpconvMaxTaps, "fd_spconv_apply: K must be in [1,27]");
     FD_REQUIRE(dtype == 0 || dtype == 1, "fd_spconv_apply: dtype must be 0 (f32) or 1 (bf16)");
     FD_REQUIRE(n_out >= 0 && n_out <= nbr_stride && n_out < (1ll << 31), "fd_spconv_apply: n_out out of range");
@@ -251,7 +251,19 @@
     if (n_out == 0) return FD_OK;
     FD_REQUIRE(in_feats && wpacked && (nbr || plan) && out_feats, "fd_spconv_apply: null argument");
     const fd::SpconvCall c{in_feats, n_in, wpacked, bias, residual, relu, nbr, nbr_stride, ranges, n_ranges, K, (int)n_out, n_out_dev, n_expected,
-                           cin, cout, dtype, out_feats, fd::as_stream(stream), plan, plan_stride};
+                           cin, cout, dtype, out_feats, fd::as_stream(stream), plan, plan_stride, layout};
+    if (layout) {
+        FD_REQUIRE((layout & ~7) == 0, "fd_spconv_apply_layout: layout has bits 0 (input), 1 (residual), 2 (output)");
+        int launched = 0;
+        if (dtype == 0 && !fd::tuning(fd::kTuneSpconvV1)) {
+            if (fd::tuning(fd::kTuneSpconvC32) >= 0) launched = fd::spconv_f32_c32_dispatch(c);
+            if (!launched) launched = fd::spconv_f32_compact_dispatch(c);
+        }
+        if (launched) return fd::check_launch("fd_spconv_apply_layout");
+        fd::set_error("fd_spconv_apply_layout: no kernel runs %d -> %d (dtype %d) with layout %d: bank-spread rows are for the fp32 32 -> 32, 64 -> 64 and "
+                      "128 -> 128 layers (all bits) and the outputs of 16 -> 32, 32 -> 64 and 64 -> 128 (bit 2)", cin, cout, dtype, layout);
+        return FD_EINVAL;
+    }
     if (dtype == 0 && !fd::tuning(fd::kTuneSpconvV1) && cin == 16 && fd::tuning(fd::kTuneF32ResRG) >= 0) {
         if (fd::spconv_f32_res16_dispatch(c)) return fd::check_launch("fd_spconv_apply(f32 resident)");
     }
@@ -315,3 +327,37 @@
     return spconv_apply(in_feats, n_in, wpacked, bias, residual, relu, nbr, nbr_stride, ranges, n_ranges, K, n_out, n_out_dev, n_expected, cin, cout,
                         dtype, out_feats, stream, plan, plan_stride);
 }
+
+constexpr int kSwzDefaultLevels = 1;
+extern "C" int fd_spconv_layout_wanted(int cin, int cout, int dtype) {
+    const int knob = fd::tuning(fd::kTuneSpconvSwz);
+    if (dtype != 0 || knob < 0 || fd::tuning(fd::kTuneSpconvV1)) return 0;
+    const int levels = knob == 0 ? kSwzDefaultLevels : knob;
+    const int level = cout == 32 ? 1 : cout == 64 ? 2 : cout == 128 ? 4 : 0;
+    if (!(levels & level)) return 0;
+    if (cin == cout) return (cout == 32 && fd::tuning(fd::kTuneSpconvC32) < 0) ? 0 : 7;
+    return 2 * cin == cout ? 4 : 0;
+}
+
+extern "C" int fd_spconv_apply_layout(const void *in_feats, int64_t n_in, const void *wpacked, const float *bias, const void *residual, int relu,
+                                      const int32_t *nbr, int64_t nbr_stride, const int32_t *ranges, int n_ranges, int K, int64_t n_out,
+                                      const int32_t *n_out_dev, int64_t n_expected, int cin, int cout, int dtype, void *out_feats,
+                                      const int32_t *plan, int64_t plan_stride, int layout, fd_stream_t stream) {
+    if (layout == 0)
+        return fd_spconv_apply_plan(in_feats, n_in, wpacked, bias, residual, relu, nbr, nbr_stride, ranges, n_ranges, K, n_out, n_out_dev, n_expected,
+                                    cin, cout, dtype, out_feats, plan, plan_stride, stream);
+    FD_REQUIRE(nbr || plan, "fd_spconv_apply_layout: nbr == NULL needs a chunk plan (fd_spconv_plan_from_index)");
+    if (plan) {
+        FD_REQUIRE(K == fd::kSpconvMaxTaps, "fd_spconv_apply_layout: a chunk plan belongs to an fp32 layer of K = 27 taps");
+        FD_REQUIRE(nbr == nullptr || cin == cout, "fd_spconv_apply_layout: next to a rulebook table a chunk plan belongs to an fp32 SubM layer (K = 27)");
+        FD_REQUIRE(plan_stride >= fd_spconv_plan_stride(n_out), "fd_spconv_apply_layout: plan_stride below fd_spconv_plan_stride(n_out)");
+        if (!nbr) {
+            FD_REQUIRE(fd_spconv_index_plan_wanted(cin, cout, dtype),
+                       "fd_spconv_apply_layout: nbr == NULL, but no kernel runs this layer shape from a chunk plan alone (fd_spconv_index_plan_wanted)");
+        } else if (!fd_spconv_plan_wanted(cin, cout, dtype)) {
+            plan = nullptr;
+        }
+    }
+    return spconv_apply(in_feats, n_in, wpacked, bias, residual, relu, nbr, nbr_stride, ranges, n_ranges, K, n_out, n_out_dev, n_expected, cin, cout,
+                        dtype, out_feats, stream, plan, plan_stride, layout);
+}
diff --git a/futuredet_amd/csrc/fd_spconv_c32.hip b/futuredet_amd/csrc/fd_spconv_c32.hip
--- a/futuredet_amd/csrc/fd_spconv_c32.hip
+++ b/futuredet_amd/csrc/fd_spconv_c32.hip
@@ -9,7 +9,7 @@
 constexpr sk::Layout L = sk::layout(TM, COUT, TS, 32);
 static_assert(((sk::kMaxTaps + TS - 1) / TS) * (TM / WR / 32) <= L.item_slot, "item list slot");
 
-template <int CIN, int DEPTH, bool PLAN>
+template <int CIN, int DEPTH, bool PLAN, bool SWZ>
 __global__ void __launch_bounds__(256) spconv_f32_c32(const float *__restrict__ in, const float4 *__restrict__ wp, const float *__restrict__ bias,
                                                       const float *__restrict__ residual, int relu, const int *__restrict__ nbr, int64_t nbr_stride,
                                                       int K, int n_out, const int *__restrict__ n_out_dev, float *__restrict__ out, unsigned in_bytes,
@@ -42,9 +42,9 @@
         int row0, n_rows;
         if (!sk::chunk_span(r_begin, r_end, chunk_rows, chunk, row0, n_rows)) break;
         if constexpr (PLAN) {
-            sk::stage_plan_chunk<TM, COUT, TS, 32>(pre, s_list, s_cnt, s_pad, s_acc, bias, residual, row0, n_rows);
+            sk::stage_plan_chunk<TM, COUT, TS, 32>(pre, s_list, s_cnt, s_pad, s_acc, bias, residual, relu, row0, n_rows);
         } else {
-            sk::stage_chunk<TM, COUT, TS, 32>(pre, s_list, s_pad, s_acc, bias, residual, K, row0, n_rows);
+            sk::stage_chunk<TM, COUT, TS, 32>(pre, s_list, s_pad, s_acc, bias, residual, relu, K, row0, n_rows);
             __syncthreads();
             sk::compact_taps<TM, WR>(s_list, s_cnt, K);
         }
@@ -56,8 +56,13 @@
         u32x4 a_r[DEPTH][NCH];
         auto stage_a0 = [&](int it) -> int { return sk::stage_a0(items, n_items, it); };
         auto stage_a1 = [&](int it, int code_v, int &kk, int &e) { sk::stage_a1<TM, WR, 32>(s_list, s_pad, n_items, wr, ln, it, code_v, kk, e); };
-        auto gather_offset = [&](int e) -> unsigned { return sk::entry_row_bytes<CIN>(e) + (unsigned)(lh * 16); };
-        auto gather_step = [&](unsigned voff, int c) { return __builtin_amdgcn_raw_buffer_load_b128(rsrc, voff + c * 32, 0, 0); };
+        auto gather_offset = [&](int e) -> unsigned {
+            const unsigned o = sk::entry_row_bytes<CIN>(e) + (unsigned)(lh * 16);
+            return SWZ ? o ^ sk::entry_swz_bits(e) : o;
+        };
+        auto gather_step = [&](unsigned voff, int c) {
+            return SWZ ? __builtin_amdgcn_raw_buffer_load_b128(rsrc, voff ^ (unsigned)(c * 32), 0, 0) : __builtin_amdgcn_raw_buffer_load_b128(rsrc, voff + c * 32, 0, 0);
+        };
         float4 b[NCH];
         auto load_b = [&](int k) {
             const float4 *wk = wp + (int64_t)k * NCH * 64 + lane;
@@ -128,16 +133,16 @@
     }
 }
 
-template <int CIN, int DEPTH, bool PLAN>
+template <int CIN, int DEPTH, bool PLAN, bool SWZ>
 int launch_c32(const fd::SpconvCall &c) {
     const unsigned in_bytes = (unsigned)(c.n_in * CIN * 4);
     int n_ranges = c.n_ranges, rows_per = 0;
     if (!c.ranges) sk::equal_rows_split(c.n_out, TM, c.n_out_dev != nullptr, n_ranges, rows_per);
     static std::atomic<uint64_t> lds_set{0};
-    if (!fd::ensure_dynamic_lds(reinterpret_cast<const void *>(spconv_f32_c32<CIN, DEPTH, PLAN>), (size_t)L.bytes, lds_set)) return 0;
+    if (!fd::ensure_dynamic_lds(reinterpret_cast<const void *>(spconv_f32_c32<CIN, DEPTH, PLAN, SWZ>), (size_t)L.bytes, lds_set)) return 0;
     const void *wp = (const char *)c.wpacked + fd::spconv_weight_layout(c).c32.offset;
-    hipLaunchKernelGGL((spconv_f32_c32<CIN, DEPTH, PLAN>), dim3((unsigned)n_ranges), dim3(256), (size_t)L.bytes, c.stream, (const float *)c.in, (const float4 *)wp,
-                       c.bias, (const float *)c.residual, c.relu, PLAN ? c.plan : c.nbr, PLAN ? c.plan_stride : c.nbr_stride, c.K, c.n_out, c.n_out_dev, (float *)c.out, in_bytes, c.ranges, rows_per);
+    hipLaunchKernelGGL((spconv_f32_c32<CIN, DEPTH, PLAN, SWZ>), dim3((unsigned)n_ranges), dim3(256), (size_t)L.bytes, c.stream, (const float *)c.in, (const float4 *)wp,
+                       c.bias, (const float *)c.residual, sk::kernel_flags(c.relu, c.layout), PLAN ? c.plan : c.nbr, PLAN ? c.plan_stride : c.nbr_stride, c.K, c.n_out, c.n_out_dev, (float *)c.out, in_bytes, c.ranges, rows_per);
     return 1;
 }
 
@@ -147,6 +152,7 @@
 int spconv_f32_c32_dispatch(const SpconvCall &c) {
     if (c.cout != 32 || c.cin != 32) return 0;
     if (!sk::entries_fit(c.n_in, c.cin)) return 0;
-    return c.plan ? launch_c32<32, 3, true>(c) : launch_c32<32, 3, false>(c);
+    if (c.layout & sk::kLayoutIn) return c.plan ? launch_c32<32, 3, true, true>(c) : launch_c32<32, 3, false, true>(c);
+    return c.plan ? launch_c32<32, 3, true, false>(c) : launch_c32<32, 3, false, false>(c);
 }
 }
diff --git a/futuredet_amd/csrc/fd_spconv_chunk.h b/futuredet_amd/csrc/fd_spconv_chunk.h
--- a/futuredet_amd/csrc/fd_spconv_chunk.h
+++ b/futuredet_amd/csrc/fd_spconv_chunk.h
@@ -15,6 +15,18 @@
     const unsigned hi = (unsigned)e & 0xffffff00u;
     return CIN >= 64 ? hi << (CIN == 128 ? 1 : 0) : hi >> (CIN == 32 ? 1 : 2);
 }
+
+constexpr int kLayoutIn = 1, kLayoutResidual = 2, kLayoutOut = 4;
+constexpr int kFlagRelu = 1, kFlagResidualSwz = kLayoutResidual, kFlagOutSwz = kLayoutOut;
+constexpr int kernel_flags(int relu, int layout) { return (relu ? kFlagRelu : 0) | (layout & (kLayoutResidual | kLayoutOut)); }
+__host__ __device__ constexpr unsigned swz_piece_bytes(unsigned s, unsigned r) { return (s ^ (r & 7u)) << 4; }
+template <int COLS>
+__device__ __forceinline__ int swz_col4(int c4, int row, bool on) {
+    if constexpr (COLS < 32) return c4;
+    return c4 ^ (row & (on ? 7 : 0));
+}
+__device__ __forceinline__ unsigned entry_swz_bits(int e) { return ((unsigned)e >> 4) & 0x70u; }
+
 inline bool entries_fit(int64_t n_in_bound, int cin) { return n_in_bound < (1ll << 23) && n_in_bound * cin * 4 < (1ll << 31); }
 
 struct Layout {
@@ -113,7 +125,7 @@
 constexpr bool kInitAcc = COUT <= 64;
 
 template <int TM, int COUT, int TS>
-__device__ __forceinline__ void init_acc(float *s_acc, const float *bias, const float *residual, int row0, int n_rows) {
+__device__ __forceinline__ void init_acc(float *s_acc, const float *bias, const float *residual, int flags, int row0, int n_rows) {
     const int tid = threadIdx.x;
     if constexpr (kInitAcc<COUT>) {
         constexpr int C4i = COUT / 4, NINIT = TM * C4i / 256;
@@ -130,7 +142,7 @@
             for (int i = 0; i < NINIT; ++i) {
                 const int t = tid + i * 256, r = t / C4i, c4 = t - r * C4i;
                 const int rr = r < n_rows ? r : n_rows - 1;
-                rv[i] = reinterpret_cast<const float4 *>(residual + (int64_t)(row0 + rr) * COUT)[c4];
+                rv[i] = reinterpret_cast<const float4 *>(residual + (int64_t)(row0 + rr) * COUT)[swz_col4<COUT>(c4, row0 + rr, flags & kFlagResidualSwz)];
             }
 #pragma unroll
             for (int i = 0; i < NINIT; ++i) { iv[i].x += rv[i].x; iv[i].y += rv[i].y; iv[i].z += rv[i].z; iv[i].w += rv[i].w; }
@@ -148,7 +160,7 @@
 
 template <int TM, int COUT, int TS, int ITEM>
 __device__ __forceinline__ void stage_chunk(const int (&pre)[kSliceRegs<TM>], int *s_list, int *s_pad, float *s_acc, const float *bias,
-                                            const float *residual, int K, int row0, int n_rows) {
+                                            const float *residual, int flags, int K, int row0, int n_rows) {
     const int tid = threadIdx.x;
     static_assert(256 % TM == 0, "a thread stages the same local row in every pass");
     const bool in_chunk = tid % TM < n_rows;
@@ -157,7 +169,7 @@
         const int t = tid + i * 256;
         if (t < K * TM) s_list[t] = in_chunk ? pre[i] : -1;
     }
-    init_acc<TM, COUT, TS>(s_acc, bias, residual, row0, n_rows);
+    init_acc<TM, COUT, TS>(s_acc, bias, residual, flags, row0, n_rows);
     if (tid < ITEM) s_pad[tid] = pad_entry(TM);
 }
 
@@ -168,7 +180,7 @@
 
 template <int TM, int COUT, int TS, int ITEM>
 __device__ __forceinline__ void stage_plan_chunk(const int (&pre)[kSliceRegs<TM>], int *s_list, unsigned char *s_cnt, int *s_pad, float *s_acc,
-                                                 const float *bias, const float *residual, int row0, int n_rows) {
+                                                 const float *bias, const float *residual, int flags, int row0, int n_rows) {
     const int tid = threadIdx.x;
     static_assert(TM == kPlanTM && 256 % TM == 0, "the plan is cut for 128-row chunks");
     static_assert(kSliceRegs<TM> * 256 >= kMaxTaps * TM + kPlanCountWords, "the count words ride in the slice's last register");
@@ -185,7 +197,7 @@
                 if (k0 + q < kMaxTaps) s_cnt[(k0 + q) * 4] = (unsigned char)((unsigned)pre[i] >> (8 * q));
         }
     }
-    init_acc<TM, COUT, TS>(s_acc, bias, residual, row0, n_rows);
+    init_acc<TM, COUT, TS>(s_acc, bias, residual, flags, row0, n_rows);
     if (tid < ITEM) s_pad[tid] = pad_entry(TM);
 }
 
@@ -252,7 +264,7 @@
 }
 
 template <int TM, int COUT, int TS>
-__device__ __forceinline__ void epilogue(float *s_acc, const float *bias, const float *residual, int relu,
+__device__ __forceinline__ void epilogue(float *s_acc, const float *bias, const float *residual, int flags,
                                          float *out, int row0, int n_rows) {
     const int tid = threadIdx.x;
     constexpr int C4 = COUT / 4;
@@ -272,14 +284,14 @@
                 v.x += bv.x; v.y += bv.y; v.z += bv.z; v.w += bv.w;
             }
             if (residual) {
-                const float4 rv = reinterpret_cast<const float4 *>(residual + (int64_t)row * COUT)[c4];
+                const float4 rv = reinterpret_cast<const float4 *>(residual + (int64_t)row * COUT)[swz_col4<COUT>(c4, row, flags & kFlagResidualSwz)];
                 v.x += rv.x; v.y += rv.y; v.z += rv.z; v.w += rv.w;
             }
         }
-        if (relu) { v.x = fmaxf(v.x, 0.f); v.y = fmaxf(v.y, 0.f); v.z = fmaxf(v.z, 0.f); v.w = fmaxf(v.w, 0.f); }
-        reinterpret_cast<float4 *>(out + (int64_t)row * COUT)[c4] = v;
-    }
-}
-
-}
-}
+        if (flags & kFlagRelu) { v.x = fmaxf(v.x, 0.f); v.y = fmaxf(v.y, 0.f); v.z = fmaxf(v.z, 0.f); v.w = fmaxf(v.w, 0.f); }
+        reinterpret_cast<float4 *>(out + (int64_t)row * COUT)[swz_col4<COUT>(c4, row, flags & kFlagOutSwz)] = v;
+    }
+}
+
+}
+}
diff --git a/futuredet_amd/csrc/fd_spconv_v2.hip b/futuredet_amd/csrc/fd_spconv_v2.hip
--- a/futuredet_amd/csrc/fd_spconv_v2.hip
+++ b/futuredet_amd/csrc/fd_spconv_v2.hip
@@ -25,7 +25,7 @@
 
 constexpr int tap_splits(int cout) { return (cout == 32 || cout == 64) ? 2 : 1; }
 
-template <int CIN, int COUT, int TM, int DEPTH, bool PLAN>
+template <int CIN, int COUT, int TM, int DEPTH, bool PLAN, bool SWZ>
 __global__ void __launch_bounds__(256) spconv_f32_compact(const float *__restrict__ in, const float4 *__restrict__ wp,
                                                           const float *__restrict__ bias, const float *__restrict__ residual, int relu,
                                                           const int *__restrict__ nbr, int64_t nbr_stride, int K, int n_out,
@@ -39,6 +39,7 @@
     constexpr int NACC = NBW;
     static_assert((TM == 128 || TM == 64) && TM / WR >= 16, "local row uses 8 bits (0..TM, TM = scratch row)");
     static_assert(!PLAN || (TM == sk::kPlanTM && WR == 1), "the chunk plan holds the lists of 128-row chunks with one row set");
+    static_assert(!SWZ || CIN >= 32, "rows of fewer than 128 bytes are never bank-spread");
     constexpr int kPad = sk::pad_entry(TM);
     constexpr sk::Layout L = sk::layout(TM, COUT, TS, 16);
     extern __shared__ __attribute__((aligned(16))) unsigned char smem[];
@@ -70,9 +71,9 @@
     int row0, n_rows;
     if (!sk::chunk_span(r_begin, r_end, chunk_rows, chunk, row0, n_rows)) break;
     if constexpr (PLAN) {
-        sk::stage_plan_chunk<TM, COUT, TS, 16>(pre, s_list, s_cnt, s_pad, s_acc, bias, residual, row0, n_rows);
+        sk::stage_plan_chunk<TM, COUT, TS, 16>(pre, s_list, s_cnt, s_pad, s_acc, bias, residual, relu, row0, n_rows);
     } else {
-        sk::stage_chunk<TM, COUT, TS, 16>(pre, s_list, s_pad, s_acc, bias, residual, K, row0, n_rows);
+        sk::stage_chunk<TM, COUT, TS, 16>(pre, s_list, s_pad, s_acc, bias, residual, relu, K, row0, n_rows);
         __syncthreads();
         if (chunk == 0) FD_T(1);
         sk::compact_taps<TM, WR>(s_list, s_cnt, K);
@@ -87,8 +88,14 @@
     u32x4 a_r[DEPTH][NC];
     auto stage_a0 = [&](int it) -> int { return sk::stage_a0(items, n_items, it); };
     auto stage_a1 = [&](int it, int code_v, int &kk, int &e) { sk::stage_a1<TM, WR, 16>(s_list, s_pad, n_items, wr, lrow, it, code_v, kk, e); };
-    auto gather_offset = [&](int e) -> unsigned { return sk::entry_row_bytes<CIN>(e) + (unsigned)(lq * 16); };
-    auto gather_chunk = [&](unsigned voff, int c) { return __builtin_amdgcn_raw_buffer_load_b128(rsrc, voff + c * 64, 0, 0); };
+    auto gather_offset = [&](int e) -> unsigned {
+        const unsigned o = sk::entry_row_bytes<CIN>(e) + (unsigned)(lq * 16);
+        return SWZ ? o ^ sk::entry_swz_bits(e) : o;
+    };
+    auto gather_chunk = [&](unsigned voff, int c) {
+        return SWZ ? __builtin_amdgcn_raw_buffer_load_b128(rsrc, (voff ^ (unsigned)((c & 1) * 64)) + (c >> 1) * 128, 0, 0)
+                   : __builtin_amdgcn_raw_buffer_load_b128(rsrc, voff + c * 64, 0, 0);
+    };
     auto load_b = [&](int k, float4(&dst)[NC][NBW]) {
         const float4 *wk = wp + ((int64_t)k * NC * NB + wc * NBW) * 64 + lane;
 #pragma unroll
@@ -199,21 +206,30 @@
     return (cin == 64 && cout == 64 && tm == 128 && lds < 56 * 1024) ? (size_t)56 * 1024 : lds;
 }
 
-template <int CIN, int COUT, int TM, int DEPTH, bool PLAN = false>
+constexpr bool has_swz_gather(int cin, int cout, int tm) { return cin == cout && (cin == 64 || cin == 128) && tm == sk::kPlanTM; }
+
+template <int CIN, int COUT, int TM, int DEPTH, bool PLAN = false, bool SWZ = false>
 int launch_compact(const fd::SpconvCall &c) {
+    if constexpr (!PLAN && !SWZ) {
+        if ((c.layout & sk::kLayoutIn) && !has_swz_gather(CIN, COUT, TM)) return 0;
+        if ((c.layout & (sk::kLayoutResidual | sk::kLayoutOut)) && COUT < 32) return 0;
+        if constexpr (has_swz_gather(CIN, COUT, TM)) {
+            if (c.layout & sk::kLayoutIn) return launch_compact<CIN, COUT, TM, DEPTH, false, true>(c);
+        }
+    }
     if constexpr (!PLAN && ((CIN == COUT && COUT >= 32) || COUT == 2 * CIN) && TM == sk::kPlanTM) {
-        if (c.plan) return launch_compact<CIN, COUT, TM, DEPTH, true>(c);
+        if (c.plan) return launch_compact<CIN, COUT, TM, DEPTH, true, SWZ>(c);
     }
     const size_t lds_req = lds_request(CIN, COUT, TM);
     static std::atomic<uint64_t> lds_set{0};
-    auto kern = spconv_f32_compact<CIN, COUT, TM, DEPTH, PLAN>;
+    auto kern = spconv_f32_compact<CIN, COUT, TM, DEPTH, PLAN, SWZ>;
     if (!fd::ensure_dynamic_lds(reinterpret_cast<const void *>(kern), lds_req, lds_set)) return 0;
     const unsigned in_bytes = (unsigned)(c.n_in * CIN * 4);
     int n_ranges = c.n_ranges, rows_per = 0;
     if (!c.ranges) sk::equal_rows_split(c.n_out, TM, c.n_out_dev != nullptr, n_ranges, rows_per);
     const void *wp = (const char *)c.wpacked + fd::spconv_weight_layout(c).base.offset;
     hipLaunchKernelGGL(kern, dim3((unsigned)n_ranges), dim3(256), lds_req, c.stream, (const float *)c.in, (const float4 *)wp, c.bias,
-                       (const float *)c.residual, c.relu, PLAN ? c.plan : c.nbr, PLAN ? c.plan_stride : c.nbr_stride, c.K, c.n_out, c.n_out_dev,
+                       (const float *)c.residual, sk::kernel_flags(c.relu, c.layout), PLAN ? c.plan : c.nbr, PLAN ? c.plan_stride : c.nbr_stride, c.K, c.n_out, c.n_out_dev,
                        (float *)c.out, in_bytes, c.ranges, rows_per);
     return 1;
 }
diff --git a/futuredet_amd/hip_ops.py b/futuredet_amd/hip_ops.py
--- a/futuredet_amd/hip_ops.py
+++ b/futuredet_amd/hip_ops.py
@@ -187,6 +187,23 @@
 def index_plan_wanted(src, dst, ksize, cin, cout):
     return (tuple(int(k) for k in ksize) == (3, 3, 3) and bool(dst.n) and bool(src.n) and src.n < (1 << 23) and src.n * cin * 4 < (1 << 31)
             and bool(_lib.load().fd_spconv_index_plan_wanted(int(cin), int(cout), 0)))
+
+
+def swizzle_rows(t):
+    n, c = t.shape
+    if c < 32 or n == 0:
+        return t.clone()
+    assert t.dtype == torch.float32 and c % 32 == 0
+    r = torch.arange(n, device=t.device) & 7
+    idx = torch.arange(8, device=t.device)[None, :] ^ r[:, None]
+    return torch.gather(t.reshape(n, c // 32, 8, 4), 2, idx[:, None, :, None].expand(n, c // 32, 8, 4)).reshape(n, c)
+
+
+def level_layout(cin, cout, n_in, n_out):
+    L = _lib.load()
+    fits = lambda n, c: 0 < n < (1 << 23) and n * c * 4 < (1 << 31)
+    return bool(fits(n_in, cin) and fits(n_out, cout) and L.fd_spconv_layout_wanted(int(cout), int(cout), 0) == 7
+                and L.fd_spconv_layout_wanted(int(cin), int(cout), 0) & 4)
 
 
 class IndexRulebook(object):
@@ -490,7 +507,7 @@
     return feats
 
 
-def spconv_apply(feats, wpacked, bias, nbr, n_out, cout, residual=None, relu=False, out=None, balanced=None, plan=None):
+def spconv_apply(feats, wpacked, bias, nbr, n_out, cout, residual=None, relu=False, out=None, balanced=None, plan=None, layout=0):
     L = _lib.load()
     feats = _dev(feats, "feats")
     dt = _DT[feats.dtype]
@@ -508,6 +525,13 @@
     ranges, n_ranges = row_split(nbr, n_out, cin, cout, balanced) if dt == 0 and n_out > 0 else (None, 0)
     if plan is None:
         plan = from_index or (dt == 0 and n_out > 0 and K == 27 and cin == cout and bool(L.fd_spconv_plan_wanted(cin, cout, 0)))
+    if layout:
+        plan_t, pstride = plan_for(nbr if from_index else _dev(nbr, "nbr", torch.int32), n_out, ranges, n_ranges) if plan else (None, 0)
+        check(L.fd_spconv_apply_layout(_p(feats), feats.shape[0], _p(_dev(wpacked, "wpacked")), _p(bias), _p(residual), int(bool(relu)),
+                                       None if from_index else _p(_dev(nbr, "nbr", torch.int32)), nstride, _p(ranges), n_ranges, K, n_out,
+                                       _p(n_dev), int(n_expected or 0), cin, cout, dt, _p(out), _p(plan_t), pstride, int(layout), _stream()),
+              "fd_spconv_apply_layout")
+        return out
     if plan:
         plan_t, pstride = plan_for(nbr if from_index else _dev(nbr, "nbr", torch.int32), n_out, ranges, n_ranges)
         check(L.fd_spconv_apply_plan(_p(feats), feats.shape[0], _p(_dev(wpacked, "wpacked")), _p(bias), _p(residual), int(bool(relu)),
diff --git a/futuredet_amd/lib.py b/futuredet_amd/lib.py
--- a/futuredet_amd/lib.py
+++ b/futuredet_amd/lib.py
@@ -117,6 +117,9 @@
     "fd_spconv_apply_plan": (c_int, [c_void_p, c_i64, c_void_p, c_void_p, c_void_p, c_int, c_void_p, c_i64, c_void_p, c_int, c_int, c_i64,
                                      c_void_p, c_i64, c_int, c_int, c_int, c_void_p, c_void_p, c_i64, c_void_p]),
     "fd_spconv_index_plan_wanted": (c_int, [c_int, c_int, c_int]),
+    "fd_spconv_layout_wanted": (c_int, [c_int, c_int, c_int]),
+    "fd_spconv_apply_layout": (c_int, [c_void_p, c_i64, c_void_p, c_void_p, c_void_p, c_int, c_void_p, c_i64, c_void_p, c_int, c_int, c_i64,
+                                       c_void_p, c_i64, c_int, c_int, c_int, c_void_p, c_void_p, c_i64, c_int, c_void_p]),
     "fd_spconv_plan_from_index": (c_int, [c_int, c_int, ctypes.POINTER(PlanSource), c_void_p]),
     "fd_spconv_ranges_from_index": (c_int, [c_void_p, c_int, c_int, c_int, c_int, c_void_p, c_i64, c_void_p, c_int, c_void_p, c_void_p, c_size_t,
                                             c_void_p]),
diff --git a/include/futuredet_hip.h b/include/futuredet_hip.h
--- a/include/futuredet_hip.h
+++ b/include/futuredet_hip.h
@@ -78,6 +78,11 @@
     int32_t stride[3], pad[3];
 } fd_plan_source;
 int fd_spconv_index_plan_wanted(int cin, int cout, int dtype);
+int fd_spconv_layout_wanted(int cin, int cout, int dtype);
+int fd_spconv_apply_layout(const void *in_feats, int64_t n_in, const void *wpacked, const float *bias, const void *residual, int relu,
+                           const int32_t *nbr, int64_t nbr_stride, const int32_t *ranges, int n_ranges, int K, int64_t n_out,
+                           const int32_t *n_out_dev, int64_t n_expected, int cin, int cout, int dtype, void *out_feats,
+                           const int32_t *plan, int64_t plan_stride, int layout, fd_stream_t stream);
 int fd_spconv_plan_from_index(int B, int n_sources, const fd_plan_source *sources_host, fd_stream_t stream);
 int fd_spconv_ranges_from_index(const uint64_t *words, int B, int D, int H, int W, const int32_t *coords, int64_t n_out,
                                 const int32_t *n_out_dev, int n_ranges, int32_t *ranges , void *workspace,
```
